# vearch/gamma

Hardware: AMD Instinct MI355X
Metric: queries/sec @ recall@10>=0.95, IVFPQ nlist=4096 nprobe=32 (higher is better)
Workload: dtype f32

## Files before the change

gamma_amd/_lib.py:

```python
import ctypes as C
import os

HERE = os.path.dirname(os.path.abspath(__file__))
LIB_PATH = os.path.join(HERE, "libgamma_hip.so")

f32p = C.POINTER(C.c_float)
i64p = C.POINTER(C.c_int64)
i32p = C.POINTER(C.c_int32)
u8p = C.POINTER(C.c_uint8)

NUM_STAGES = 6
STAGE_NAMES = ["coarse", "tables", "scan", "select", "rerank", "flat"]


class RangeFilter(C.Structure):
    _fields_ = [("bitmap", u8p), ("bitmap_bytes", C.c_int64), ("min_doc", C.c_int32),
                ("max_doc", C.c_int32), ("min_aligned", C.c_int32), ("b_not_in", C.c_int32)]


class FieldFilter(C.Structure):
    _fields_ = [("field_id", C.c_int32), ("include_lower", C.c_int32), ("include_upper", C.c_int32),
                ("reserved", C.c_int32), ("lower_i", C.c_int64), ("upper_i", C.c_int64),
                ("lower_f", C.c_double), ("upper_f", C.c_double)]


class TermFilter(C.Structure):
    _fields_ = [("field_id", C.c_int32), ("op", C.c_int32), ("n_items", C.c_int32), ("items", C.c_int32 * 16)]


class SearchParams(C.Structure):
    _fields_ = [("metric", C.c_int32), ("nprobe", C.c_int32), ("recall_num", C.c_int32),
                ("has_rank", C.c_int32), ("min_score", C.c_float), ("max_score", C.c_float),
                ("coarse_mode", C.c_int32), ("has_range", C.c_int32), ("n_range", C.c_int32),
                ("range", C.POINTER(RangeFilter)), ("n_field", C.c_int32), ("n_term", C.c_int32),
                ("field", C.POINTER(FieldFilter)), ("term", C.POINTER(TermFilter)), ("exact_ties", C.c_int32)]


SYMBOLS = {
    "gamma_hip_create": (C.c_int, [C.c_int, C.POINTER(C.c_void_p)]),
    "gamma_hip_destroy": (C.c_int, [C.c_void_p]),
    "gamma_hip_strerror": (C.c_char_p, [C.c_int]),
    "gamma_hip_last_error": (C.c_char_p, [C.c_void_p]),
    "gamma_hip_stream": (C.c_void_p, [C.c_void_p]),
    "gamma_hip_synchronize": (C.c_int, [C.c_void_p]),
    "gamma_hip_set_workspace_budget": (C.c_int, [C.c_void_p, C.c_int64]),
    "gamma_hip_debug_heap_stream": (C.c_int, [C.c_void_p, C.c_int, C.c_int, C.c_int, f32p, f32p, i32p, f32p, i32p]),
    "gamma_hip_set_scan_bound_feedback": (C.c_int, [C.c_void_p, C.c_int]),
    "gamma_hip_scan_bound_stats": (C.c_int, [C.c_void_p, i64p]),
    "gamma_hip_set_exact_ties": (C.c_int, [C.c_void_p, C.c_int]),
    "gamma_hip_field_append": (C.c_int, [C.c_void_p, C.c_int, C.c_int, C.c_int64, C.c_void_p]),
    "gamma_hip_field_update": (C.c_int, [C.c_void_p, C.c_int, C.c_int64, C.c_void_p]),
    "gamma_hip_field_count": (C.c_int64, [C.c_void_p, C.c_int]),
    "gamma_hip_term_append": (C.c_int, [C.c_void_p, C.c_int, C.c_int64, C.POINTER(C.c_int32), C.POINTER(C.c_int32)]),
    "gamma_hip_term_count": (C.c_int64, [C.c_void_p, C.c_int]),
    "gamma_hip_term_update": (C.c_int, [C.c_void_p, C.c_int, C.c_int64, C.c_int32, C.POINTER(C.c_int32)]),
    "gamma_hip_raw_init": (C.c_int, [C.c_void_p, C.c_int]),
    "gamma_hip_raw_append": (C.c_int, [C.c_void_p, C.c_int64, f32p]),
    "gamma_hip_raw_update": (C.c_int, [C.c_void_p, C.c_int64, f32p]),
    "gamma_hip_ivfpq_arena_stats": (C.c_int, [C.c_void_p, i64p]),
    "gamma_hip_ivfpq_arena_growth": (C.c_int, [C.c_void_p, i64p]),
    "gamma_hip_ivfpq_set_repack_threshold": (C.c_int, [C.c_void_p, C.c_int64]),
    "gamma_hip_set_small_path": (C.c_int, [C.c_void_p, C.c_int]),
    "gamma_hip_set_coarse_fused": (C.c_int, [C.c_void_p, C.c_int, C.c_int]),
    "gamma_hip_tie_stats": (C.c_int, [C.c_void_p, i64p, C.c_int]),
    "gamma_hip_ties_not_honoured": (C.c_int, [C.c_void_p, i64p, C.c_int]),
    "gamma_hip_blas_form_not_restated": (C.c_int, [C.c_void_p, i64p, C.c_int]),
    "gamma_hip_raw_write": (C.c_int, [C.c_void_p, C.c_int64, C.c_int64, f32p]),
    "gamma_hip_raw_gets": (C.c_int, [C.c_void_p, C.c_int64, i64p, f32p]),
    "gamma_hip_ivfpq_repack_verify_stats": (C.c_int, [C.c_void_p, i64p]),
    "gamma_hip_raw_count": (C.c_int64, [C.c_void_p]),
    "gamma_hip_raw_stats": (C.c_int, [C.c_void_p, i64p]),
    "gamma_hip_bitmap_upload": (C.c_int, [C.c_void_p, u8p, C.c_int64]),
    "gamma_hip_bitmap_set": (C.c_int, [C.c_void_p, i64p, C.c_int64, C.c_int]),
    "gamma_hip_ivfpq_init": (C.c_int, [C.c_void_p] + [C.c_int] * 7),
    "gamma_hip_ivfpq4_init": (C.c_int, [C.c_void_p] + [C.c_int] * 6),
    "gamma_hip_ivfpq_set_trained": (C.c_int, [C.c_void_p, f32p, f32p, f32p]),
    "gamma_hip_ivfpq_get_precomputed_table": (C.c_int, [C.c_void_p, f32p]),
    "gamma_hip_set_precomputed_table_max_bytes": (C.c_int, [C.c_int64]),
    "gamma_hip_get_precomputed_table_max_bytes": (C.c_int64, []),
    "gamma_hip_ivfpq_use_precomputed_table": (C.c_int, [C.c_void_p]),
    "gamma_hip_ivfpq_add_keys": (C.c_int, [C.c_void_p, C.c_int, C.c_int, i64p, u8p]),
    "gamma_hip_ivfpq_add_keys_batch": (C.c_int, [C.c_void_p, C.c_int, i32p, i32p, i64p, u8p]),
    "gamma_hip_ivfpq_update": (C.c_int, [C.c_void_p, C.c_int, C.c_int64, u8p]),
    "gamma_hip_vid2docid_append": (C.c_int, [C.c_void_p, C.c_int64, C.POINTER(C.c_int32)]),
    "gamma_hip_vid2docid_count": (C.c_int64, [C.c_void_p]),
    "gamma_hip_binivf_init": (C.c_int, [C.c_void_p, C.c_int, C.c_int, C.c_int, C.c_int]),
    "gamma_hip_binivf_train": (C.c_int, [C.c_void_p, C.c_int, C.c_int64, u8p, C.c_int, u8p]),
    "gamma_hip_binivf_set_trained": (C.c_int, [C.c_void_p, u8p]),
    "gamma_hip_binivf_assign": (C.c_int, [C.c_void_p, C.c_int64, u8p, C.c_int, i32p, i64p]),
    "gamma_hip_binivf_add": (C.c_int, [C.c_void_p, C.c_int64, u8p, C.c_int64]),
    "gamma_hip_binivf_search": (C.c_int, [C.c_void_p, C.POINTER(SearchParams), C.c_int, u8p, C.c_int, f32p, i64p]),
    "gamma_hip_binivf_search_device": (C.c_int, [C.c_void_p, C.POINTER(SearchParams), C.c_int, C.c_void_p, C.c_int,
                                                 C.c_void_p, C.c_void_p]),
    "gamma_hip_binivf_stats": (C.c_int, [C.c_void_p, i64p, C.c_int]),
    "gamma_hip_ivfflat_init": (C.c_int, [C.c_void_p, C.c_int, C.c_int, C.c_int, C.c_int, C.c_int]),
    "gamma_hip_ivfflat_set_trained": (C.c_int, [C.c_void_p, f32p]),
    "gamma_hip_ivfflat_search": (C.c_int, [C.c_void_p, C.POINTER(SearchParams), C.c_int, f32p, C.c_int, f32p, i64p]),
    "gamma_hip_ivfflat_search_device": (C.c_int, [C.c_void_p, C.POINTER(SearchParams), C.c_int, C.c_void_p, C.c_int,
                                                  C.c_void_p, C.c_void_p]),
    "gamma_hip_ivfpq_has_vid": (C.c_int, [C.c_void_p, i64p, C.c_int, u8p]),
    "gamma_hip_ivfpq_remove": (C.c_int, [C.c_void_p, C.c_int64]),
    "gamma_hip_ivfpq_delete": (C.c_int, [C.c_void_p, i64p, C.c_int]),
    "gamma_hip_ivfpq_compact_if_need": (C.c_int, [C.c_void_p]),
    "gamma_hip_ivfpq_list_size": (C.c_int64, [C.c_void_p, C.c_int]),
    "gamma_hip_ivfpq_list_capacity": (C.c_int64, [C.c_void_p, C.c_int]),
    "gamma_hip_ivfpq_get_list": (C.c_int, [C.c_void_p, C.c_int, i64p, u8p]),
    "gamma_hip_ivfpq_set_list_mask": (C.c_int, [C.c_void_p, u8p]),
    "gamma_hip_ivfpq_add": (C.c_int, [C.c_void_p, C.c_int64, f32p, C.c_int64]),
    "gamma_hip_ivfpq_encode": (C.c_int, [C.c_void_p, C.c_int64, f32p, i64p, u8p]),
    "gamma_hip_assign": (C.c_int, [C.c_void_p, C.c_int, C.c_int64, f32p, C.c_int, f32p, i32p, f32p]),
    "gamma_hip_kmeans": (C.c_int, [C.c_void_p, C.c_int, C.c_int64, f32p, C.c_int, C.c_int, C.c_int64, C.c_int, f32p,
                                   C.POINTER(C.c_float)]),
    "gamma_hip_rand_perm": (None, [i32p, C.c_int64, C.c_int64]),
    "gamma_hip_ivfpq_train": (C.c_int, [C.c_void_p, C.c_int, C.c_int64, f32p, C.c_int, C.c_int, f32p, f32p]),
    "gamma_hip_ivfpq_search": (C.c_int, [C.c_void_p, C.POINTER(SearchParams), C.c_int, f32p, C.c_int,
                                         f32p, i64p]),
    "gamma_hip_ivfpq_search_device": (C.c_int, [C.c_void_p, C.POINTER(SearchParams), C.c_int,
                                                C.c_void_p, C.c_int, C.c_void_p, C.c_void_p]),
    "gamma_hip_ivfpq_search_device_wait": (C.c_int, [C.c_void_p, C.POINTER(SearchParams), C.c_int,
                                                     C.c_void_p, C.c_int, C.c_void_p, C.c_void_p]),
    "gamma_hip_flat_search_device_wait": (C.c_int, [C.c_void_p, C.POINTER(SearchParams), C.c_int,
                                                    C.c_void_p, C.c_int, C.c_void_p, C.c_void_p]),
    "gamma_hip_ivfpq_last_stages": (C.c_int, [C.c_void_p, f32p, i64p, f32p, i64p]),
    "gamma_hip_ivfpq_search_shard": (C.c_int, [C.c_void_p, C.POINTER(SearchParams), C.c_int,
                                               C.c_void_p, C.c_int, C.c_void_p, C.c_void_p]),
    "gamma_hip_ivfpq_coarse_device": (C.c_int, [C.c_void_p, C.POINTER(SearchParams), C.c_int, C.c_void_p,
                                                C.c_void_p, C.c_void_p]),
    "gamma_hip_ivfpq_search_shard_preassigned": (C.c_int, [C.c_void_p, C.POINTER(SearchParams), C.c_int,
                                                           C.c_void_p, C.c_void_p, C.c_void_p, C.c_int,
                                                           C.c_void_p, C.c_void_p]),
    "gamma_hip_ivfpq_search_shard_bounded": (C.c_int, [C.c_void_p, C.POINTER(SearchParams), C.c_int,
                                                       C.c_void_p, C.c_void_p, C.c_void_p, C.c_int,
                                                       C.c_void_p, C.c_void_p, C.c_void_p, C.c_void_p, C.c_void_p]),
    "gamma_hip_raw_put": (C.c_int, [C.c_void_p, C.c_int64, i64p, f32p]),
    "gamma_hip_raw_drop": (C.c_int, [C.c_void_p, C.c_int64, i64p]),
    "gamma_hip_raw_clear": (C.c_int, [C.c_void_p]),
    "gamma_hip_raw_sparse_stats": (C.c_int, [C.c_void_p, i64p]),
    "gamma_hip_ivfpq_shard_exact": (C.c_int, [C.c_void_p, C.POINTER(SearchParams), C.c_int, C.c_void_p, C.c_void_p, C.c_int, C.c_void_p]),
    "gamma_hip_ivfpq_merge_rerank_exact": (C.c_int, [C.c_void_p, C.POINTER(SearchParams), C.c_int, C.c_int, C.c_void_p, C.c_int,
                                                     C.c_void_p, C.c_void_p, C.c_void_p, C.c_int, C.c_int, C.c_void_p, C.c_void_p]),
    "gamma_hip_ivfpq_shard_export_exact": (C.c_int, [C.c_void_p, C.POINTER(SearchParams), C.c_int, C.c_void_p, C.c_void_p, C.c_void_p,
                                                     C.c_void_p, C.c_int64, C.c_void_p, C.c_void_p]),
    "gamma_hip_ivfpq_merge_replay_exact": (C.c_int, [C.c_void_p, C.POINTER(SearchParams), C.c_int, C.c_int, C.c_void_p, C.c_int64,
                                                     C.c_void_p, C.c_void_p, C.c_void_p, C.c_void_p, C.c_int, C.c_void_p, C.c_void_p,
                                                     C.c_void_p]),
    "gamma_hip_bound_combine": (C.c_int, [C.c_void_p, C.c_void_p, C.c_void_p, C.c_int, C.c_int]),
    "gamma_hip_ivfpq_merge_rerank": (C.c_int, [C.c_void_p, C.POINTER(SearchParams), C.c_int, C.c_int,
                                               C.c_void_p, C.c_int, C.c_void_p, C.c_void_p, C.c_int,
                                               C.c_int, C.c_void_p, C.c_void_p]),
    "gamma_hip_flat_search": (C.c_int, [C.c_void_p, C.POINTER(SearchParams), C.c_int, f32p, C.c_int,
                                        f32p, i64p]),
    "gamma_hip_flat_search_device": (C.c_int, [C.c_void_p, C.POINTER(SearchParams), C.c_int,
                                               C.c_void_p, C.c_int, C.c_void_p, C.c_void_p]),
    "gamma_hip_raw_update_batch": (C.c_int, [C.c_void_p, C.c_int64, i64p, f32p]),
    "gamma_hip_ivfpq_dim": (C.c_int, [C.c_void_p]),
    "gamma_hip_ivfpq_nlist": (C.c_int, [C.c_void_p]),
    "gamma_hip_ivfpq_code_size": (C.c_int, [C.c_void_p]),
    "gamma_hip_ivfpq_update_batch": (C.c_int, [C.c_void_p, C.c_int, i64p, f32p]),
    "gamma_hip_ivfpq_encode_each": (C.c_int, [C.c_void_p, C.c_int64, f32p, i64p, u8p]),
    "gamma_hip_ivfpq_apply_updates": (C.c_int, [C.c_void_p, C.c_int, i32p, i64p, u8p, u8p]),
    "gamma_hip_group_create": (C.c_int, [C.POINTER(C.c_int), C.c_int, C.POINTER(C.c_void_p)]),
    "gamma_hip_group_destroy": (C.c_int, [C.c_void_p]),
    "gamma_hip_group_size": (C.c_int, [C.c_void_p]),
    "gamma_hip_group_member": (C.c_void_p, [C.c_void_p, C.c_int]),
    "gamma_hip_group_last_error": (C.c_char_p, [C.c_void_p]),
    "gamma_hip_group_set_owners": (C.c_int, [C.c_void_p, i64p]),
    "gamma_hip_group_owner": (C.c_int, [C.c_void_p, C.c_int]),
    "gamma_hip_ivfpq_shard_cut_flags": (C.c_int, [C.c_void_p, C.c_int, C.c_void_p]),
    "gamma_hip_ivfpq_merge_set_shard_flags": (C.c_int, [C.c_void_p, C.c_void_p]),
    "gamma_hip_ivfpq_merge_flagged": (C.c_int, [C.c_void_p, C.POINTER(C.c_int), C.POINTER(C.c_void_p)]),
    "gamma_hip_gather_rows": (C.c_int, [C.c_void_p, C.c_void_p, C.c_int, C.c_void_p, C.c_int, C.c_void_p]),
    "gamma_hip_ivfpq_max_list_len": (C.c_int, [C.c_void_p]),
    "gamma_hip_ivfpq_shard_export_rows": (C.c_int, [C.c_void_p, C.c_void_p, C.c_int, C.c_void_p, i64p]),
    "gamma_hip_ivfpq_shard_export": (C.c_int, [C.c_void_p, C.c_void_p, C.c_int, C.c_void_p, C.c_void_p, C.c_void_p, C.c_int64,
                                               C.c_void_p, C.c_void_p, C.c_void_p]),
    "gamma_hip_ivfpq_merge_replay": (C.c_int, [C.c_void_p, C.c_void_p, C.c_int, C.c_int, C.c_void_p, C.c_int64, C.c_void_p,
                                               C.c_void_p, C.c_void_p, C.c_int, C.c_void_p, C.c_void_p, C.c_void_p]),
    "gamma_hip_set_deferred_replay": (C.c_int, [C.c_void_p, C.c_int]),
    "gamma_hip_join": (C.c_int, [C.c_void_p]),
    "gamma_hip_group_set_placement": (C.c_int, [C.c_void_p, C.c_int]),
    "gamma_hip_group_placement": (C.c_int, [C.c_void_p]),
    "gamma_hip_group_ivfpq_add": (C.c_int, [C.c_void_p, C.c_int64, f32p, C.c_int64]),
    "gamma_hip_group_ivfpq_add_keys": (C.c_int, [C.c_void_p, C.c_int, C.c_int, i64p, u8p]),
    "gamma_hip_group_ivfpq_list_size": (C.c_int64, [C.c_void_p, C.c_int]),
    "gamma_hip_group_set_transport": (C.c_int, [C.c_void_p, C.c_int]),
    "gamma_hip_group_transport": (C.c_int, [C.c_void_p, i64p]),
    "gamma_hip_group_transport_note": (C.c_char_p, [C.c_void_p]),
    "gamma_hip_group_ivfpq_get_list": (C.c_int, [C.c_void_p, C.c_int, i64p, u8p]),
    "gamma_hip_group_ivfpq_update": (C.c_int, [C.c_void_p, C.c_int, i64p, f32p]),
    "gamma_hip_group_ivfpq_delete": (C.c_int, [C.c_void_p, i64p, C.c_int]),
    "gamma_hip_group_ivfpq_compact_if_need": (C.c_int, [C.c_void_p]),
    "gamma_hip_group_ivfpq_search": (C.c_int, [C.c_void_p, C.POINTER(SearchParams), C.c_int, f32p, C.c_int, f32p, i64p]),
    "gamma_hip_group_ivfpq_search_device": (C.c_int, [C.c_void_p, C.POINTER(SearchParams), C.c_int, C.c_void_p, C.c_int,
                                                      C.c_void_p, C.c_void_p]),
    "gamma_hip_group_total_mem_bytes": (C.c_int64, [C.c_void_p]),
    "gamma_hip_group_set_raw_placement": (C.c_int, [C.c_void_p, C.c_int]),
    "gamma_hip_group_raw_placement": (C.c_int, [C.c_void_p]),
    "gamma_hip_group_raw_put": (C.c_int, [C.c_void_p, C.c_int64, i64p, f32p, i64p]),
    "gamma_hip_total_mem_bytes": (C.c_int64, [C.c_void_p]),
    "gamma_hip_profile_enable": (C.c_int, [C.c_void_p, C.c_int]),
    "gamma_hip_profile_reset": (C.c_int, [C.c_void_p]),
    "gamma_hip_profile_get": (C.c_int, [C.c_void_p, C.c_int, C.POINTER(C.c_double),
                                        C.POINTER(C.c_int64)]),
    "gamma_hip_profile_scan_bytes": (C.c_int, [C.c_void_p, C.POINTER(C.c_int64),
                                               C.POINTER(C.c_int64)]),
}

_lib = None


BOUND_REDUCE_FN = C.CFUNCTYPE(C.c_int, C.c_void_p, C.c_void_p, C.c_int, C.c_int, C.c_void_p)


class GammaHipError(RuntimeError):
    pass

# ... 21 lines not shown
```

gamma_amd/api.py:

```python
import ctypes as C

import numpy as np

from . import _lib
from ._lib import GammaHipError, RangeFilter, SearchParams

METRIC_IP = 0
METRIC_L2 = 1

FLT_TINY = float(np.finfo(np.float32).tiny)
FLT_MAX = float(np.finfo(np.float32).max)


def _f32(a):
    return np.ascontiguousarray(a, dtype=np.float32)


def _p(a, t):
    return a.ctypes.data_as(t) if a is not None else None


def make_range_filter(docids, b_not_in=False):
    docids = np.asarray(sorted(set(int(x) for x in docids)), dtype=np.int64)
    mn, mx = (int(docids[0]), int(docids[-1])) if len(docids) else (0, 0)
# ... 361 lines not shown

    def binivf_search(self, x, k, args):
        x = np.ascontiguousarray(x, dtype=np.uint8)
        nq = x.shape[0]
        D = np.empty((nq, max(k, 0)), dtype=np.float32)
        I = np.empty((nq, max(k, 0)), dtype=np.int64)
        self._ck(self.L.gamma_hip_binivf_search(self.h, args.ref(), nq, _p(x, _lib.u8p), k, _p(D, _lib.f32p),
                                                _p(I, _lib.i64p)), "binivf_search")
        return D, I

    def binivf_search_device(self, d_x, nq, k, args, d_D, d_I):
        self._ck(self.L.gamma_hip_binivf_search_device(self.h, args.ref(), nq, d_x, k, d_D, d_I), "binivf_search_device")

    def binivf_stats(self, reset=False):
        out = np.zeros(2, dtype=np.int64)
        self._ck(self.L.gamma_hip_binivf_stats(self.h, _p(out, _lib.i64p), 1 if reset else 0), "binivf_stats")
        return int(out[0]), int(out[1])

    def last_stages(self, nq, nprobe, R):
        cd = np.empty((nq, nprobe), dtype=np.float32)
        ci = np.empty((nq, nprobe), dtype=np.int64)
        rd = np.empty((nq, R), dtype=np.float32)
        ri = np.empty((nq, R), dtype=np.int64)
        self._ck(self.L.gamma_hip_ivfpq_last_stages(self.h, _p(cd, _lib.f32p), _p(ci, _lib.i64p),
                                                    _p(rd, _lib.f32p), _p(ri, _lib.i64p)), "last_stages")
        return dict(coarse_dis=cd, coarse_idx=ci, recall_dis=rd, recall_ids=ri)

    def flat_search(self, x, k, args):
        x = _f32(x)
        nq = x.shape[0]
        D = np.empty((nq, max(k, 0)), dtype=np.float32)
        I = np.empty((nq, max(k, 0)), dtype=np.int64)
        self._ck(self.L.gamma_hip_flat_search(self.h, args.ref(), nq, _p(x, _lib.f32p), k,
                                              _p(D, _lib.f32p), _p(I, _lib.i64p)), "flat_search")
        return D, I

    def ivfpq_search_device(self, d_x, nq, k, args, d_D, d_I):
        self._ck(self.L.gamma_hip_ivfpq_search_device(self.h, args.ref(), nq, d_x, k, d_D, d_I),
                 "ivfpq_search_device")

    def ivfpq_search_device_wait(self, d_x, nq, k, args, d_D, d_I):
        self._ck(self.L.gamma_hip_ivfpq_search_device_wait(self.h, args.ref(), nq, d_x, k, d_D, d_I),
                 "ivfpq_search_device_wait")

    def flat_search_device_wait(self, d_x, nq, k, args, d_D, d_I):
        self._ck(self.L.gamma_hip_flat_search_device_wait(self.h, args.ref(), nq, d_x, k, d_D, d_I), "flat_search_device_wait")

    def flat_search_device(self, d_x, nq, k, args, d_D, d_I):
        self._ck(self.L.gamma_hip_flat_search_device(self.h, args.ref(), nq, d_x, k, d_D, d_I),
                 "flat_search_device")

    def ivfpq_search_shard(self, d_x, nq, k, args, d_rdis, d_rids):
        self._ck(self.L.gamma_hip_ivfpq_search_shard(self.h, args.ref(), nq, d_x, k, d_rdis, d_rids),
                 "ivfpq_search_shard")

    def ivfpq_coarse_device(self, d_x, nq, args, d_cdis, d_probe):
        self._ck(self.L.gamma_hip_ivfpq_coarse_device(self.h, args.ref(), nq, d_x, d_cdis, d_probe),
                 "ivfpq_coarse_device")

    def ivfpq_search_shard_preassigned(self, d_x, nq, d_cdis, d_probe, k, args, d_rdis, d_rids):
        self._ck(self.L.gamma_hip_ivfpq_search_shard_preassigned(self.h, args.ref(), nq, d_x, d_cdis,
                                                                  d_probe, k, d_rdis, d_rids),
                 "ivfpq_search_shard_preassigned")

    def ivfpq_search_shard_bounded(self, d_x, nq, d_cdis, d_probe, k, args, d_rdis, d_rids, d_bound, reduce=None):
        err = []

        def _cb(user, ptr, n, take_max, stream):
            try:
                reduce(n, bool(take_max))
                return 0
            except BaseException as e:
                err.append(e)
                return 1
        cb = _lib.BOUND_REDUCE_FN(_cb) if reduce is not None else None
        rc = self.L.gamma_hip_ivfpq_search_shard_bounded(self.h, args.ref(), nq, d_x, d_cdis, d_probe, k, d_rdis, d_rids,
                                                         d_bound, C.cast(cb, C.c_void_p) if cb is not None else None, None)
        if err:
            raise err[0]
        self._ck(rc, "ivfpq_search_shard_bounded")

    def ivfpq_merge_rerank(self, nshards, nq, d_x, k, args, d_all_dis, d_all_ids, q0, nq_local, d_D, d_I):
        self._ck(self.L.gamma_hip_ivfpq_merge_rerank(self.h, args.ref(), nshards, nq, d_x, k, d_all_dis,
                                                     d_all_ids, q0, nq_local, d_D, d_I), "merge_rerank")

    def ivfpq_shard_cut_flags(self, nq, d_flags):
        self._ck(self.L.gamma_hip_ivfpq_shard_cut_flags(self.h, nq, d_flags), "shard_cut_flags")

    def ivfpq_merge_set_shard_flags(self, d_flags):
        self._ck(self.L.gamma_hip_ivfpq_merge_set_shard_flags(self.h, d_flags), "merge_set_shard_flags")

    def ivfpq_merge_flagged(self):
        import ctypes as C
        n = C.c_int(0)
        ptr = C.c_void_p(0)
        self._ck(self.L.gamma_hip_ivfpq_merge_flagged(self.h, C.byref(n), C.byref(ptr)), "merge_flagged")
        return int(n.value), (ptr.value or 0)

    def gather_rows(self, d_src, row_words, d_list, n, d_dst):
        self._ck(self.L.gamma_hip_gather_rows(self.h, d_src, row_words, d_list, n, d_dst), "gather_rows")

    def max_list_len(self):
        return self.L.gamma_hip_ivfpq_max_list_len(self.h)

    def ivfpq_shard_export_rows(self, nf, d_probe_f, args):
        out = np.zeros(1, dtype=np.int64)
        self._ck(self.L.gamma_hip_ivfpq_shard_export_rows(self.h, args.ref(), nf, d_probe_f, _p(out, _lib.i64p)), "shard_export_rows")
        return int(out[0])

    def ivfpq_shard_export(self, nf, d_xf, d_cdis_f, d_probe_f, stride, args, d_vals, d_ids, d_off):
        self._ck(self.L.gamma_hip_ivfpq_shard_export(self.h, args.ref(), nf, d_xf, d_cdis_f, d_probe_f, stride, d_vals, d_ids,
                                                     d_off), "shard_export")

    def ivfpq_shard_exact(self, d_x, nq, d_ids, R, args, d_exact):
        self._ck(self.L.gamma_hip_ivfpq_shard_exact(self.h, args.ref(), nq, d_x, d_ids, R, d_exact), "shard_exact")

    def ivfpq_merge_rerank_exact(self, nshards, nq, d_x, k, args, d_all_dis, d_all_ids, d_all_exact, q0, nq_local, d_D, d_I):
        self._ck(self.L.gamma_hip_ivfpq_merge_rerank_exact(self.h, args.ref(), nshards, nq, d_x, k, d_all_dis, d_all_ids, d_all_exact,
                                                           q0, nq_local, d_D, d_I), "merge_rerank_exact")

    def ivfpq_shard_export_exact(self, nf, d_xf, d_vals, d_ids, d_off, stride, d_bound_f, args, d_ex):
        self._ck(self.L.gamma_hip_ivfpq_shard_export_exact(self.h, args.ref(), nf, d_xf, d_vals, d_ids, d_off, stride, d_bound_f, d_ex),
                 "shard_export_exact")

    def ivfpq_merge_replay_exact(self, nshards, nf, d_x_slice, stride, d_vals_all, d_ids_all, d_off_all, d_ex_all, k, args, d_list,
                                 d_D, d_I):
        self._ck(self.L.gamma_hip_ivfpq_merge_replay_exact(self.h, args.ref(), nshards, nf, d_x_slice, stride, d_vals_all, d_ids_all,
                                                           d_off_all, d_ex_all, k, d_list, d_D, d_I), "merge_replay_exact")

    def ivfpq_merge_replay(self, nshards, nf, d_x_slice, stride, d_vals_all, d_ids_all, d_off_all, k, args, d_list, d_D, d_I):
        self._ck(self.L.gamma_hip_ivfpq_merge_replay(self.h, args.ref(), nshards, nf, d_x_slice, stride, d_vals_all, d_ids_all,
                                                     d_off_all, k, d_list, d_D, d_I), "merge_replay")

    def debug_heap_stream(self, op, k, vals):
        vals = _f32(vals).ravel()
        av, ai = np.empty(k, np.float32), np.empty(k, np.int32)
        sv, si = np.empty(k, np.float32), np.empty(k, np.int32)
        self._ck(self.L.gamma_hip_debug_heap_stream(self.h, op, k, len(vals), _p(vals, _lib.f32p), _p(av, _lib.f32p),
                                                    _p(ai, _lib.i32p), _p(sv, _lib.f32p), _p(si, _lib.i32p)), "debug_heap_stream")
        return av, ai, sv, si

    def set_scan_bound_feedback(self, on):
        self._ck(self.L.gamma_hip_set_scan_bound_feedback(self.h, 1 if on else 0), "set_scan_bound_feedback")

    def scan_bound_stats(self):
        out = np.zeros(4, np.int64)
        self._ck(self.L.gamma_hip_scan_bound_stats(self.h, _p(out, _lib.i64p)), "scan_bound_stats")
        return dict(zip(["fell_through", "queries", "backoffs", "gave_up_waiting"], [int(v) for v in out]))

    def set_dist_budget(self, nbytes):
        self._ck(self.L.gamma_hip_set_workspace_budget(self.h, int(nbytes)), "set_workspace_budget")

    def set_coarse_fused(self, on=True, list_cap=128):
        self._ck(self.L.gamma_hip_set_coarse_fused(self.h, 1 if on else 0, list_cap), "set_coarse_fused")

    def set_small_path(self, on=True):
        self._ck(self.L.gamma_hip_set_small_path(self.h, int(on)), "set_small_path")

    def tie_stats(self, reset=False):
        out = np.zeros(3, np.int64)
        self._ck(self.L.gamma_hip_tie_stats(self.h, _p(out, _lib.i64p), 1 if reset else 0), "tie_stats")
        return dict(coarse_rows=int(out[0]), cut_ties=int(out[1]), replayed=int(out[2]))

    def ties_not_honoured(self, reset=False):
        out = np.zeros(1, dtype=np.int64)
        self._ck(self.L.gamma_hip_ties_not_honoured(self.h, _p(out, _lib.i64p), 1 if reset else 0), "ties_not_honoured")
        return int(out[0])

    def blas_form_not_restated(self, reset=False):
        out = np.zeros(1, dtype=np.int64)
        self._ck(self.L.gamma_hip_blas_form_not_restated(self.h, _p(out, _lib.i64p), 1 if reset else 0), "blas_form_not_restated")
        return int(out[0])

    def set_exact_ties(self, on=True):
        self._ck(self.L.gamma_hip_set_exact_ties(self.h, 1 if on else 0), "set_exact_ties")

    _FIELD_DTYPES = {np.dtype(np.int32): 0, np.dtype(np.int64): 1, np.dtype(np.float32): 2,
                     np.dtype(np.float64): 3}

    def field_append(self, field_id, values):
        values = np.ascontiguousarray(values)
        dt = self._FIELD_DTYPES[values.dtype]
        self._ck(self.L.gamma_hip_field_append(self.h, field_id, dt, values.size, values.ctypes.data),
                 "field_append")

    def field_update(self, field_id, docid, value):
        value = np.ascontiguousarray(value)
        self._ck(self.L.gamma_hip_field_update(self.h, field_id, docid, value.ctypes.data), "field_update")

    def term_append(self, field_id, docs_items):
        counts = np.ascontiguousarray([len(d) for d in docs_items], dtype=np.int32)
        flat = np.ascontiguousarray([t for d in docs_items for t in d], dtype=np.int32)
        self._ck(self.L.gamma_hip_term_append(self.h, field_id, len(counts), counts.ctypes.data_as(C.POINTER(C.c_int32)),
                                              flat.ctypes.data_as(C.POINTER(C.c_int32))), "term_append")

    def term_update(self, field_id, docid, items):
        it = np.ascontiguousarray(items, dtype=np.int32)
        self._ck(self.L.gamma_hip_term_update(self.h, field_id, docid, len(it), it.ctypes.data_as(C.POINTER(C.c_int32))),
                 "term_update")

    def term_count(self, field_id):
        return self.L.gamma_hip_term_count(self.h, field_id)

    def field_count(self, field_id):
        return self.L.gamma_hip_field_count(self.h, field_id)

    def stream(self):
        return self.L.gamma_hip_stream(self.h)

    def synchronize(self):
        self._ck(self.L.gamma_hip_synchronize(self.h), "synchronize")

    def total_mem_bytes(self):
        return self.L.gamma_hip_total_mem_bytes(self.h)

    def profile_enable(self, on=True):
        self._ck(self.L.gamma_hip_profile_enable(self.h, int(on)), "profile_enable")

    def profile_reset(self):
        self._ck(self.L.gamma_hip_profile_reset(self.h), "profile_reset")

    def profile(self):
        out = {}
        for i, name in enumerate(_lib.STAGE_NAMES):
            ms, n = C.c_double(), C.c_int64()
            self._ck(self.L.gamma_hip_profile_get(self.h, i, C.byref(ms), C.byref(n)), "profile_get")
            out[name] = (ms.value, n.value)
        b, pr = C.c_int64(), C.c_int64()
        self._ck(self.L.gamma_hip_profile_scan_bytes(self.h, C.byref(b), C.byref(pr)), "scan_bytes")
        out["scan_bytes"] = b.value
        out["scan_pairs"] = pr.value
        return out


class GammaHipGroup:

    def __init__(self, devices):
        self.L = _lib.load()
        devs = (C.c_int * len(devices))(*devices)
        g = C.c_void_p()
        rc = self.L.gamma_hip_group_create(devs, len(devices), C.byref(g))
        if rc != 0:
            raise GammaHipError("gamma_hip_group_create(%s): %s" % (list(devices), self.L.gamma_hip_strerror(rc).decode()))
        self.g = g
        self.members = []
        for i in range(len(devices)):
            m = GammaHip.__new__(GammaHip)
            m.L = self.L
            m.h = C.c_void_p(self.L.gamma_hip_group_member(g, i))
            m.d = m.M = None
            m.close = lambda: None
            self.members.append(m)

    def close(self):
        if getattr(self, "g", None):
            for m in self.members:
                m.h = None
            self.L.gamma_hip_group_destroy(self.g)
            self.g = None

    def __del__(self):
        try:
            self.close()
        except Exception:
            pass

    def _ck(self, rc, what):
        if rc != 0:
            raise GammaHipError("%s: %s (%s)" % (what, self.L.gamma_hip_strerror(rc).decode(),
                                                 self.L.gamma_hip_group_last_error(self.g).decode()))

    def each(self, fn):
        return [fn(m) for m in self.members]

    def set_owners(self, weights=None):
        w = None if weights is None else np.ascontiguousarray(weights, dtype=np.int64)
        self._ck(self.L.gamma_hip_group_set_owners(self.g, None if w is None else _p(w, _lib.i64p)), "group_set_owners")

    def owner(self, l):
        return self.L.gamma_hip_group_owner(self.g, l)

    def set_placement(self, replicate):
        self._ck(self.L.gamma_hip_group_set_placement(self.g, 1 if replicate else 0), "group_set_placement")

    def set_raw_placement(self, sharded):
        self._ck(self.L.gamma_hip_group_set_raw_placement(self.g, 1 if sharded else 0), "group_set_raw_placement")

    def raw_placement(self):
        return bool(self.L.gamma_hip_group_raw_placement(self.g))

    def raw_put(self, vids, vecs):
        vids = np.ascontiguousarray(vids, dtype=np.int64)
        vecs = _f32(vecs)
        skipped = np.zeros(1, dtype=np.int64)
        self._ck(self.L.gamma_hip_group_raw_put(self.g, len(vids), _p(vids, _lib.i64p), _p(vecs, _lib.f32p), _p(skipped, _lib.i64p)),
                 "group_raw_put")
        return int(skipped[0])

    def add(self, vecs, first_vid):
        vecs = _f32(vecs)
        self._ck(self.L.gamma_hip_group_ivfpq_add(self.g, vecs.shape[0], _p(vecs, _lib.f32p), first_vid), "group_add")

    def add_keys(self, l, vids, codes):
        vids = np.ascontiguousarray(vids, dtype=np.int64)
        codes = np.ascontiguousarray(codes, dtype=np.uint8)
        self._ck(self.L.gamma_hip_group_ivfpq_add_keys(self.g, l, len(vids), _p(vids, _lib.i64p), _p(codes, _lib.u8p)),
                 "group_add_keys")
# ... 68 lines not shown
```

gamma_amd/csrc/coarse.hip:

```cpp
#include <hip/hip_runtime.h>
#include <stdint.h>
#include <math.h>
#include <stdlib.h>

#include <algorithm>
#include <type_traits>

#include "device_math.h"
#include "heap_dev.h"
#include "kernels.h"

namespace gh {

namespace {
typedef float f32x16 __attribute__((ext_vector_type(16)));
typedef unsigned int u32x2 __attribute__((ext_vector_type(2)));

__device__ __forceinline__ int wave_incl_scan_i(int v) {
    const int lane = threadIdx.x & 63;
#pragma unroll
    for (int o = 1; o < 64; o <<= 1) {
        const int t = __shfl_up(v, o, 64);
        if (lane >= o) v += t;
    }
    return v;
}
}

template <int NCH, bool STORE = false>
__global__ __launch_bounds__(256, 2) void k_coarse_fused(const float* __restrict__ x, int nq,
                                                         const float* __restrict__ y, int ny, int col0,
                                                         const float* __restrict__ yn,
                                                         const float* __restrict__ tau,
                                                         int tiles_per_strip, int cap, int cap_stride,
                                                         unsigned long long* __restrict__ cand,
                                                         int* __restrict__ cand_cnt, int nseg,
                                                         const int* __restrict__ rowmap) {
    constexpr int D = 16 * NCH, LD = D + 1, SEGS = D / 32;
    extern __shared__ float s_co[];
    __shared__ float s_xn[128];
    __shared__ float2 s_xt[128];
    const int tid = threadIdx.x, lane = tid & 63, w = tid >> 6;
    const int seg = blockIdx.x, q_base = blockIdx.y * 128;
    int nrows = nq;
    if constexpr (STORE) {
        if (rowmap) {
            nrows = min(rowmap[0], nq);
            if (q_base >= nrows) return;
        }
    }
    const int ntiles = (ny - col0 + 63) >> 6;
    const int t0 = seg * tiles_per_strip, t1 = min(ntiles, t0 + tiles_per_strip);
    auto slot_r = [&](int it) { return (((w * NCH + it) / SEGS) << 3) + (lane >> 3); };
    auto slot_c = [&](int it) { return (((w * NCH + it) % SEGS) << 5) + ((lane & 7) << 2); };
    float4 vb[NCH];
    auto put = [&](float* base, int it) {
        float* p = base + slot_r(it) * LD + slot_c(it);
        p[0] = vb[it].x; p[1] = vb[it].y; p[2] = vb[it].z; p[3] = vb[it].w;
    };
#pragma unroll
    for (int half = 0; half < 2; half++) {
#pragma unroll
        for (int it = 0; it < NCH; it++) {
            int row = min(q_base + half * 64 + slot_r(it), nrows - 1);
            if constexpr (STORE) {
                if (rowmap) row = rowmap[1 + row];
            }
            vb[it] = *reinterpret_cast<const float4*>(x + (int64_t)row * D + slot_c(it));
        }
#pragma unroll
        for (int it = 0; it < NCH; it++) put(s_co + half * 64 * LD, it);
    }
    __syncthreads();
#pragma unroll
    for (int half = 0; half < 2; half++) {
        const float* row = s_co + (half * 64 + (tid >> 2)) * LD;
        const int l4 = tid & 3;
        float nacc = 0.f;
        for (int i = 0; i < D; i += 4) {
            const float xv = row[i + l4];
            nacc = __builtin_fmaf(xv, xv, nacc);
        }
        const float t01 = nacc + __shfl_down(nacc, 1, 4);
        const float nn = t01 + __shfl_down(t01, 2, 4);
        if (l4 == 0) s_xn[half * 64 + (tid >> 2)] = nn;
    }
    float a[8 * NCH];
    {
        const float* fa = s_co + (w * 32 + (lane & 31)) * LD + (lane >> 5);
#pragma unroll
        for (int u = 0; u < 8 * NCH; u++) a[u] = fa[2 * u];
    }
    __syncthreads();
    if (tid < 128) s_xt[tid] = make_float2(s_xn[tid], (!STORE && q_base + tid < nq) ? tau[q_base + tid] : -INFINITY);
    auto gload = [&](int t) {
#pragma unroll
        for (int it = 0; it < NCH; it++)
            vb[it] = *reinterpret_cast<const float4*>(y + (int64_t)min(col0 + t * 64 + slot_r(it), ny - 1) * D + slot_c(it));
    };
    if (t0 < t1) {
        gload(t0);
#pragma unroll
        for (int it = 0; it < NCH; it++) put(s_co, it);
    }
    __syncthreads();
    int cnt[16];
#pragma unroll
    for (int r = 0; r < 16; r++) cnt[r] = 0;
    const uint32_t lt_mask = (1u << (lane & 31)) - 1u;
    const unsigned row_stride = STORE ? (unsigned)cap_stride : (unsigned)nseg * (unsigned)cap_stride;
    const unsigned lane_row = STORE ? (unsigned)(q_base + w * 32 + 4 * (lane >> 5)) * (unsigned)cap_stride
                                    : ((unsigned)((q_base + w * 32 + 4 * (lane >> 5)) * nseg + seg)) * (unsigned)cap_stride;
    const __amdgpu_buffer_rsrc_t rsrc = __builtin_amdgcn_make_buffer_rsrc(
        cand, 0,
        (int)min(STORE ? (int64_t)nq * cap_stride * 4 : (int64_t)nq * nseg * cap_stride * 8, (int64_t)0x7fffffff),
        0x00020000);
    constexpr unsigned OOB = 0x80000000u;
    const int sh = lane & 32;
    int rs[16];
#pragma unroll
    for (int r = 0; r < 16; r++) rs[r] = ((r & 3) + 8 * (r >> 2)) * (int)row_stride * (STORE ? 4 : 8);
    const float2* xt_row = s_xt + w * 32 + 4 * (lane >> 5);
    auto epi = [&](const f32x16& o, int r, unsigned colv, float ync, int rsoff) {
        const float2 xt = xt_row[(r & 3) + 8 * (r >> 2)];
        if constexpr (STORE) {
            float dis = __builtin_fmaf(-2.f, o[r], xt.x + ync);
            if (dis < 0.f) dis = 0.f;
            __builtin_amdgcn_raw_buffer_store_b32(__float_as_uint(dis), rsrc,
                                                  (int)colv < ny ? (lane_row + (colv - (unsigned)col0)) * 4u : OOB, rsoff, 0);
            return;
        }
        const float dis = __builtin_fmaf(-2.f, o[r], xt.x + ync);
        const bool pass = dis <= xt.y;
        const unsigned long long mask = __ballot(pass);
        const uint32_t mh = (uint32_t)(mask >> sh);
        const unsigned slot = min((unsigned)cnt[r] + (unsigned)__popc(mh & lt_mask), (unsigned)cap);
        u32x2 item;
        item.x = colv;
        item.y = (uint32_t)max((int)__float_as_uint(dis), 0) | 0x80000000u;
        __builtin_amdgcn_raw_buffer_store_b64(item, rsrc, pass ? (lane_row + slot) * 8u : OOB, rsoff, 0);
        cnt[r] += __popc(mh);
    };
    auto step = [&](auto do_mfma, auto do_epi, f32x16& n, const float* fb, const f32x16& o, int colo) {
        constexpr bool MF = decltype(do_mfma)::value, EP = decltype(do_epi)::value;
        float ync = 0.f;
        const unsigned colv = (unsigned)(colo + (lane & 31));
        if constexpr (EP) ync = (int)colv < ny ? yn[min((int)colv, ny - 1)] : INFINITY;
        if constexpr (MF) {
#pragma unroll
            for (int i = 0; i < 16; i++) n[i] = 0.f;
            float f[4];
#pragma unroll
            for (int u = 0; u < 3; u++) f[u] = fb[2 * u];
            constexpr int KP = 8 * NCH, EVERY = KP / 16;
#pragma unroll
            for (int u = 0; u < KP; u++) {
                if (u + 3 < KP) f[(u + 3) & 3] = fb[2 * (u + 3)];
                n = __builtin_amdgcn_mfma_f32_32x32x2f32(a[u], f[u & 3], n, 0, 0, 0);
                if constexpr (EP) {
                    if (u % EVERY == 0) epi(o, u / EVERY, colv, ync, rs[u / EVERY]);
                }
                __builtin_amdgcn_sched_barrier(0);
            }
        } else if constexpr (EP) {
#pragma unroll
            for (int r = 0; r < 16; r++) epi(o, r, colv, ync, rs[r]);
        }
    };
    const std::true_type yes;
    const std::false_type no;
    f32x16 acc0, acc1;
    auto stage = [&](int t) {
#pragma unroll
        for (int it = 0; it < NCH; it++) put(s_co + ((t - t0) & 1) * 64 * LD, it);
    };
    for (int t = t0; t < t1; t++) {
        const float* fb0 = s_co + ((t - t0) & 1) * 64 * LD + (lane & 31) * LD + (lane >> 5);
        const int colb = col0 + t * 64;
        if (t > t0) step(yes, yes, acc0, fb0, acc1, colb - 32);
        else step(yes, no, acc0, fb0, acc1, 0);
        const bool more = t + 1 < t1;
        if (more) gload(t + 1);
        step(yes, yes, acc1, fb0 + 32 * LD, acc0, colb);
        if (more) stage(t + 1);
        __syncthreads();
    }
    if (t0 < t1) step(no, yes, acc0, s_co, acc1, col0 + (t1 - 1) * 64 + 32);
    if (!STORE && (lane & 31) == 0) {
#pragma unroll
        for (int r = 0; r < 16; r++) {
            const int row = q_base + w * 32 + (r & 3) + 8 * (r >> 2) + 4 * (lane >> 5);
            if (row < nq) cand_cnt[row * nseg + seg] = cnt[r];
        }
    }
}


__device__ __forceinline__ uint32_t wave_kth_smallest(uint32_t m, int K) {
    int lt = 0, le = 0;
#pragma unroll
    for (int l = 0; l < 64; l++) {
        const uint32_t o = (uint32_t)__builtin_amdgcn_readlane((int)m, l);
        lt += o < m ? 1 : 0;
        le += o <= m ? 1 : 0;
    }
    const unsigned long long who = __ballot(lt < K && K <= le);
    return (uint32_t)__shfl((int)m, (int)__ffsll((long long)who) - 1, 64);
}

__device__ __forceinline__ uint32_t wave_kth_smallest2(uint32_t m0, uint32_t m1, int K) {
    int lt0 = 0, le0 = 0, lt1 = 0, le1 = 0;
#pragma unroll
    for (int l = 0; l < 64; l++) {
        const uint32_t o0 = (uint32_t)__builtin_amdgcn_readlane((int)m0, l);
        const uint32_t o1 = (uint32_t)__builtin_amdgcn_readlane((int)m1, l);
        lt0 += (o0 < m0 ? 1 : 0) + (o1 < m0 ? 1 : 0);
        le0 += (o0 <= m0 ? 1 : 0) + (o1 <= m0 ? 1 : 0);
        lt1 += (o0 < m1 ? 1 : 0) + (o1 < m1 ? 1 : 0);
        le1 += (o0 <= m1 ? 1 : 0) + (o1 <= m1 ? 1 : 0);
    }
    const unsigned long long who0 = __ballot(lt0 < K && K <= le0), who1 = __ballot(lt1 < K && K <= le1);
    return who0 ? (uint32_t)__shfl((int)m0, (int)__ffsll((long long)who0) - 1, 64)
                : (uint32_t)__shfl((int)m1, (int)__ffsll((long long)who1) - 1, 64);
}

template <int NPL>
__global__ __launch_bounds__(256) void k_coarse_bound(const float* __restrict__ mat, int nq, int P, float* __restrict__ tau,
                                                      int* __restrict__ ovf) {
    if (blockIdx.x == 0 && threadIdx.x == 0) ovf[0] = 0;
    const int lane = threadIdx.x & 63, q = blockIdx.x * 4 + (threadIdx.x >> 6);
    if (q >= nq) return;
    const float* v = mat + (int64_t)q * (64 * NPL) + lane;
    uint32_t m0 = 0xffffffffu, m1 = 0xffffffffu;
#pragma unroll
    for (int j = 0; j < NPL; j++) {
        const uint32_t k = f2key(v[64 * j]);
        if (j & 1) m1 = k < m1 ? k : m1;
        else m0 = k < m0 ? k : m0;
    }
    const uint32_t kb = P <= 32 ? wave_kth_smallest(m0 < m1 ? m0 : m1, P) : wave_kth_smallest2(m0, m1, P);
    if (lane == 0) tau[q] = key2f(kb);
}

constexpr int CF_BUF = 256;
template <int SNPL, int MAXSEG>
__global__ __launch_bounds__(256) void k_coarse_final(const float* __restrict__ mat, const float* __restrict__ tau,
                                                      const unsigned long long* __restrict__ cand,
                                                      const int* __restrict__ cand_cnt, int nseg, int cap,
                                                      int cap_stride, int nq, int P, float* __restrict__ out_dis,
                                                      int* __restrict__ out_idx, int* __restrict__ ovf, int flag_ties) {
    constexpr int NPL = SNPL + 2 * MAXSEG;
    __shared__ unsigned long long s_buf[4][CF_BUF];
    const int lane = threadIdx.x & 63, w = threadIdx.x >> 6;
    const int q = blockIdx.x * 4 + w;
    if (q >= nq) return;
    unsigned long long* buf = s_buf[w];
    const int cnt = lane < nseg ? cand_cnt[q * nseg + lane] : 0;
    if (__ballot(cnt > cap)) {
        if (lane == 0) ovf[1 + atomicAdd(ovf, 1)] = q;
        return;
    }
    unsigned long long it[NPL];
    {
        const float t = tau[q];
        const float* v = mat + (int64_t)q * (64 * SNPL) + lane;
#pragma unroll
        for (int j = 0; j < SNPL; j++) {
            const float x = v[64 * j];
            it[j] = x <= t ? (((unsigned long long)f2key(x) << 32) | (unsigned)(64 * j + lane)) : ~0ull;
        }
    }
#pragma unroll
    for (int sg = 0; sg < MAXSEG; sg++) {
        const int c = __shfl(cnt, sg, 64);
        const unsigned long long* p = cand + ((int64_t)q * nseg + min(sg, nseg - 1)) * cap_stride;
        const int e0 = (lane - 4 * sg) & 63;
        it[SNPL + 2 * sg] = e0 < c ? p[e0] : ~0ull;
        it[SNPL + 2 * sg + 1] = e0 + 64 < c ? p[e0 + 64] : ~0ull;
    }
    uint32_t m0 = 0xffffffffu, m1 = 0xffffffffu;
#pragma unroll
    for (int j = 0; j < NPL; j++) {
        const uint32_t k = (uint32_t)(it[j] >> 32);
        const bool g1 = j < SNPL ? (j & 1) != 0 : ((j >> 1) & 1) != 0;
        if (g1) m1 = k < m1 ? k : m1;
        else m0 = k < m0 ? k : m0;
    }
    const uint32_t kb = P <= 32 ? wave_kth_smallest(m0 < m1 ? m0 : m1, P) : wave_kth_smallest2(m0, m1, P);
    int c = 0;
#pragma unroll
    for (int j = 0; j < NPL; j++) c += ((uint32_t)(it[j] >> 32) <= kb && it[j] != ~0ull) ? 1 : 0;
    const int incl = wave_incl_scan_i(c);
    const int tot = __shfl(incl, 63, 64);
    if (tot > CF_BUF) {
        if (lane == 0) ovf[1 + atomicAdd(ovf, 1)] = q;
        return;
    }
    int off = incl - c;
#pragma unroll
    for (int j = 0; j < NPL; j++)
        if ((uint32_t)(it[j] >> 32) <= kb && it[j] != ~0ull) buf[off++] = it[j];
    __builtin_amdgcn_wave_barrier();
    unsigned long long mine[CF_BUF / 64];
    int rr[CF_BUF / 64];
#pragma unroll
    for (int u = 0; u < CF_BUF / 64; u++) {
        mine[u] = lane + 64 * u < tot ? buf[lane + 64 * u] : ~0ull;
        rr[u] = 0;
    }
    if (tot <= 64) {
        for (int j = 0; j < tot; j++) rr[0] += buf[j] < mine[0] ? 1 : 0;
    } else {
        for (int j = 0; j < tot; j++) {
            const unsigned long long xj = buf[j];
#pragma unroll
            for (int u = 0; u < CF_BUF / 64; u++) rr[u] += xj < mine[u] ? 1 : 0;
        }
    }
#pragma unroll
    for (int u = 0; u < CF_BUF / 64; u++) {
        if (lane + 64 * u < tot && rr[u] < P) {
            out_dis[(int64_t)q * P + rr[u]] = key2f((uint32_t)(mine[u] >> 32));
            out_idx[(int64_t)q * P + rr[u]] = (int)(uint32_t)mine[u];
        }
    }
    for (int r = tot + lane; r < P; r += 64) {
        out_dis[(int64_t)q * P + r] = INFINITY;
        out_idx[(int64_t)q * P + r] = -1;
    }
    if (flag_ties) {
        __builtin_amdgcn_wave_barrier();
#pragma unroll
        for (int u = 0; u < CF_BUF / 64; u++)
            if (lane + 64 * u < tot) buf[rr[u]] = mine[u];
        __builtin_amdgcn_wave_barrier();
        const int have = min(tot, P + 1);
        bool eq = false;
        for (int i = lane; i + 1 < have; i += 64) eq |= (uint32_t)(buf[i] >> 32) == (uint32_t)(buf[i + 1] >> 32);
        if (__ballot(eq) && lane == 0) ovf[1 + atomicAdd(ovf, 1)] = q;
    }
}

__global__ __launch_bounds__(256) void k_coarse_repair(const float* __restrict__ x, int d, const float* __restrict__ y, int ny,
                                                       const float* __restrict__ yn, const int* __restrict__ ovf,
                                                       uint32_t* __restrict__ scratch, int P,
                                                       float* __restrict__ out_dis, int* __restrict__ out_idx) {
    extern __shared__ float s_x[];
    __shared__ float s_n;
    __shared__ unsigned long long s_red[4];
    const int tid = threadIdx.x, lane = tid & 63, w = tid >> 6;
    const int n = ovf[0];
    uint32_t* keys = scratch + (int64_t)blockIdx.x * ny;
    for (int i = blockIdx.x; i < n; i += gridDim.x) {
        const int q = ovf[1 + i];
        __syncthreads();
        for (int t = tid; t < d; t += 256) s_x[t] = x[(int64_t)q * d + t];
        __syncthreads();
        if (tid == 0) {
            float a4[4] = {0.f, 0.f, 0.f, 0.f};
            int t = 0;
            for (; t + 4 <= d; t += 4)
                for (int l = 0; l < 4; l++) a4[l] = __builtin_fmaf(s_x[t + l], s_x[t + l], a4[l]);
            for (int l = 0; t + l < d; l++) a4[l] = a4[l] + s_x[t + l] * s_x[t + l];
            s_n = (a4[0] + a4[1]) + (a4[2] + a4[3]);
        }
        __syncthreads();
        const float xn = s_n;
        for (int c = tid; c < ny; c += 256) {
            const float* yr = y + (int64_t)c * d;
            float ip = 0.f;
            for (int t = 0; t < d; t++) ip = __builtin_fmaf(s_x[t], yr[t], ip);
            float dis = (xn + yn[c]) - 2.f * ip;
            if (dis < 0.f) dis = 0.f;
            keys[c] = f2key(dis);
        }
        __syncthreads();
        unsigned long long last = 0;
        bool first = true;
        for (int r = 0; r < P; r++) {
            unsigned long long best = ~0ull;
            for (int c = tid; c < ny; c += 256) {
                const unsigned long long item = ((unsigned long long)keys[c] << 32) | (unsigned)c;
                if ((first || item > last) && item < best) best = item;
            }
#pragma unroll
            for (int o = 32; o > 0; o >>= 1) {
                const unsigned long long t = __shfl_xor(best, o, 64);
                best = t < best ? t : best;
            }
            if (lane == 0) s_red[w] = best;
            __syncthreads();
            best = s_red[0];
            for (int k = 1; k < 4; k++) best = s_red[k] < best ? s_red[k] : best;
            __syncthreads();
            if (tid == 0) {
                out_dis[(int64_t)q * P + r] = best == ~0ull ? INFINITY : key2f((uint32_t)(best >> 32));
                out_idx[(int64_t)q * P + r] = best == ~0ull ? -1 : (int)(uint32_t)best;
            }
            last = best;
            first = false;
            if (best == ~0ull) {
                for (int r2 = r + 1 + tid; r2 < P; r2 += 256) {
                    out_dis[(int64_t)q * P + r2] = INFINITY;
                    out_idx[(int64_t)q * P + r2] = -1;
                }
                break;
            }
        }
    }
}

static bool coarse_fused_shape(int nlist, int P, int* sample, int* nseg) {
    if (P < 1 || P > 64) return false;
    for (int sm = P <= 32 ? 512 : 1024; sm <= 2048; sm *= 2) {
        if (nlist < 4 * sm) break;
        const double F = P <= 32 ? 1.0 - pow(1.0 - P / 64.0, 64.0 / sm) : 1.0 - pow(1.0 - P / 128.0, 128.0 / sm);
        for (int sg = 8; sg <= 16; sg *= 2) {
            if (F * (nlist - sm) / sg <= 48.0) {
                *sample = sm;
                *nseg = sg;
                return true;
            }
        }
    }
    return false;
}

bool coarse_fused_supported(int nq, int d, int nlist, int P, bool exact_ties) {
    int sm, sg;
    if (!(nq >= 4096 && (d == 32 || d == 64 || d == 96 || d == 128) && coarse_fused_shape(nlist, P, &sm, &sg))) return false;
    if (exact_ties && (int64_t)nq * nlist * 4 >= 0x7fffffffLL) return false;
    return (int64_t)nq * sg * kCoarseCap * 8 < 0x7fffffffLL && (int64_t)nq * sm * 4 < 0x7fffffffLL;
}

CoarseFusedPlan coarse_fused_plan(int nq, int nlist, int P, int cap, bool exact_ties) {
    CoarseFusedPlan pl;
    if (!coarse_fused_shape(nlist, P, &pl.sample, &pl.nseg)) {
        launch_refused("coarse_fused_plan: shape outside the matrix-free coarse path (coarse_fused_supported)");
        pl.sample = 512;
        pl.nseg = 1;
    }
    const int ntiles = (nlist - pl.sample + 63) / 64;
    pl.tiles_per_strip = (ntiles + pl.nseg - 1) / pl.nseg;
    pl.nseg = (ntiles + pl.tiles_per_strip - 1) / pl.tiles_per_strip;
    pl.cap_stride = kCoarseCap;
    pl.cap = std::max(1, std::min(kCoarseCap - 1, cap));
    size_t o = 0;
    auto take = [&](size_t bytes) {
        const size_t at = o;
        o += (bytes + 255) & ~(size_t)255;
        return at;
    };
    pl.off_mat = take((size_t)nq * pl.sample * sizeof(float));
    pl.off_tau = take((size_t)nq * sizeof(float));
    pl.off_cand = take((size_t)nq * pl.nseg * pl.cap_stride * sizeof(unsigned long long));
    pl.off_cnt = take((size_t)nq * pl.nseg * sizeof(int));
    pl.off_ovf = take((size_t)(nq + 1) * sizeof(int));
    pl.off_scratch = take((size_t)kCoarseRepairGrid * nlist * sizeof(uint32_t));
    pl.off_full = exact_ties ? take((size_t)nq * nlist * sizeof(float)) : 0;
    pl.bytes = o;
    return pl;
}

void launch_coarse_fused(hipStream_t s, const CoarseFusedPlan& pl, void* ws, const float* x, int nq, int d,
                         const float* y, int nlist, const float* yn, int P, float* out_dis, int* out_idx, bool exact_ties,
                         unsigned long long* tie_stats, hipStream_t side, hipEvent_t fork, hipEvent_t join) {
    char* b = static_cast<char*>(ws);
    float* mat = reinterpret_cast<float*>(b + pl.off_mat);
    float* tau = reinterpret_cast<float*>(b + pl.off_tau);
    unsigned long long* cand = reinterpret_cast<unsigned long long*>(b + pl.off_cand);
    int* cnt = reinterpret_cast<int*>(b + pl.off_cnt);
    int* ovf = reinterpret_cast<int*>(b + pl.off_ovf);
    uint32_t* scratch = reinterpret_cast<uint32_t*>(b + pl.off_scratch);
    const size_t lds = (size_t)2 * 64 * (d + 1) * sizeof(float);
    {
        const int stiles = pl.sample / 64, sstrips = 4, tps = (stiles + sstrips - 1) / sstrips;
        dim3 sgrid((unsigned)sstrips, (unsigned)((nq + 127) / 128));
#define GH_CS(NCH)                                                                                                      \
    do {                                                                                                                \
        static std::atomic<uint64_t> attr{0};                                                           \
        if (first_call_on_device(attr)) {                                                                               \
            (void)hipFuncSetAttribute(reinterpret_cast<const void*>(k_coarse_fused<NCH, true>),                         \
                                      hipFuncAttributeMaxDynamicSharedMemorySize, 2 * 64 * (16 * NCH + 1) * 4);         \
        }                                                                                                               \
        hipLaunchKernelGGL((k_coarse_fused<NCH, true>), sgrid, dim3(256), lds, s, x, nq, y, pl.sample, 0, yn, nullptr, \
                           tps, 0, pl.sample, reinterpret_cast<unsigned long long*>(mat), nullptr, sstrips, nullptr);  \
    } while (0)
        switch (d) {
            case 32: GH_CS(2); break;
            case 64: GH_CS(4); break;
            case 96: GH_CS(6); break;
            default: GH_CS(8); break;
        }
#undef GH_CS
    }
    if (pl.sample == 512) hipLaunchKernelGGL(k_coarse_bound<8>, dim3((nq + 3) / 4), dim3(256), 0, s, mat, nq, P, tau, ovf);
    else if (pl.sample == 1024) hipLaunchKernelGGL(k_coarse_bound<16>, dim3((nq + 3) / 4), dim3(256), 0, s, mat, nq, P, tau, ovf);
    else hipLaunchKernelGGL(k_coarse_bound<32>, dim3((nq + 3) / 4), dim3(256), 0, s, mat, nq, P, tau, ovf);
    dim3 grid((unsigned)pl.nseg, (unsigned)((nq + 127) / 128));
#define GH_CF(NCH)                                                                                                      \
    do {                                                                                                                \
        static std::atomic<uint64_t> attr{0};                                                           \
        if (first_call_on_device(attr)) {                                                                               \
            (void)hipFuncSetAttribute(reinterpret_cast<const void*>(k_coarse_fused<NCH>),                               \
                                      hipFuncAttributeMaxDynamicSharedMemorySize, 2 * 64 * (16 * NCH + 1) * 4);         \
        }                                                                                                               \
        hipLaunchKernelGGL((k_coarse_fused<NCH>), grid, dim3(256), lds, s, x, nq, y, nlist, pl.sample, yn, tau,         \
                           pl.tiles_per_strip, pl.cap, pl.cap_stride, cand, cnt, pl.nseg, nullptr);                          \
    } while (0)
    switch (d) {
        case 32: GH_CF(2); break;
        case 64: GH_CF(4); break;
        case 96: GH_CF(6); break;
        default: GH_CF(8); break;
    }
#undef GH_CF
#define GH_FIN(SN, MS)                                                                                                  \
    hipLaunchKernelGGL((k_coarse_final<SN, MS>), dim3((nq + 3) / 4), dim3(256), 0, s, mat, tau, cand, cnt, pl.nseg, pl.cap, \
                       pl.cap_stride, nq, P, out_dis, out_idx, ovf, exact_ties ? 1 : 0)
    if (pl.sample == 512) {
        if (pl.nseg <= 4) GH_FIN(8, 4);
        else if (pl.nseg <= 8) GH_FIN(8, 8);
        else GH_FIN(8, 16);
    } else if (pl.sample == 1024) {
        if (pl.nseg <= 8) GH_FIN(16, 8);
        else GH_FIN(16, 16);
    } else {
        if (pl.nseg <= 8) GH_FIN(32, 8);
        else GH_FIN(32, 16);
    }
#undef GH_FIN
    if (!exact_ties) {
        hipLaunchKernelGGL(k_coarse_repair, dim3(kCoarseRepairGrid), dim3(256), (size_t)d * sizeof(float), s, x, d, y, nlist, yn,
                           ovf, scratch, P, out_dis, out_idx);
        return;
    }
    hipStream_t rs = s;
    const bool forked = side && fork && join;
    float* full = reinterpret_cast<float*>(b + pl.off_full);
    {
        const int ntiles = (nlist + 63) / 64, fstrips = std::min(ntiles, 64), tps = (ntiles + fstrips - 1) / fstrips;
        dim3 fgrid((unsigned)fstrips, (unsigned)((nq + 127) / 128));
#define GH_CR(NCH)                                                                                                      \
    hipLaunchKernelGGL((k_coarse_fused<NCH, true>), fgrid, dim3(256), lds, rs, x, nq, y, nlist, 0, yn, nullptr, tps, 0,  \
                       nlist, reinterpret_cast<unsigned long long*>(full), nullptr, fstrips, ovf)
        switch (d) {
            case 32: GH_CR(2); break;
            case 64: GH_CR(4); break;
            case 96: GH_CR(6); break;
            default: GH_CR(8); break;
        }
#undef GH_CR
    }
    if (forked) {
        (void)hipEventRecord(fork, s);
        (void)hipStreamWaitEvent(side, fork, 0);
        rs = side;
    }
    launch_coarse_heap_rows(rs, full, nlist, nq, P, ovf, out_dis, out_idx, tie_stats);
    if (rs != s) (void)hipEventRecord(join, rs);
}

}
```

gamma_amd/csrc/flat_mfma.hip:

```cpp
#include <hip/hip_runtime.h>
#include <stdint.h>

#include <algorithm>
#include <atomic>
#include <cstdlib>

#include "device_math.h"
#include "filter_dev.h"
#include "block_utils.h"
#include "kernels.h"
#include "rerank_dev.h"

namespace gh {

typedef __attribute__((__vector_size__(8 * sizeof(__bf16)))) __bf16 bf16x8;
typedef float ff32x16 __attribute__((ext_vector_type(16)));

constexpr float FM_C = 1.220703125e-4f;
constexpr int FM_QT = 64;
constexpr int FM_ROWS = 128;
constexpr int FM_NT = 256;

__device__ __forceinline__ uint32_t cvt_pk_bf16(float lo, float hi) {
    uint32_t r;
    asm("v_cvt_pk_bf16_f32 %0, %1, %2" : "=v"(r) : "v"(lo), "v"(hi));
    return r;
}
__device__ __forceinline__ void split_bf16x8(const float* f, uint4& hi, uint4& lo) {
    uint32_t h[4], l[4];
#pragma unroll
    for (int i = 0; i < 4; i++) {
        h[i] = cvt_pk_bf16(f[2 * i], f[2 * i + 1]);
        const float h0 = __uint_as_float(h[i] << 16), h1 = __uint_as_float(h[i] & 0xffff0000u);
        l[i] = cvt_pk_bf16(f[2 * i] - h0, f[2 * i + 1] - h1);
    }
    hi = make_uint4(h[0], h[1], h[2], h[3]);
    lo = make_uint4(l[0], l[1], l[2], l[3]);
}

__host__ __device__ constexpr int fm_mt_bytes(int D) { return 2 * (D / 16) * 2 * 32 * 16; }

template <int D>
__global__ __launch_bounds__(256) void k_flat_prep_queries(const float* __restrict__ x, int nq, int nq_pad,
                                                           char* __restrict__ out) {
    constexpr int KK = D / 16;
    const int idx = blockIdx.x * 256 + threadIdx.x;
    if (idx >= nq_pad * (D / 8)) return;
    const int q = idx / (D / 8), kg = idx % (D / 8);
    float f[8];
#pragma unroll
    for (int t = 0; t < 8; t++) f[t] = q < nq ? x[(int64_t)q * D + kg * 8 + t] : 0.f;
    uint4 hi, lo;
    split_bf16x8(f, hi, lo);
    const int mt = q >> 5, i = q & 31, kh = kg / KK, kk = kg % KK;
    char* base = out + (int64_t)mt * fm_mt_bytes(D);
    *reinterpret_cast<uint4*>(base + ((((0 * KK + kk) * 2 + kh) * 32 + i) * 16)) = hi;
    *reinterpret_cast<uint4*>(base + ((((1 * KK + kk) * 2 + kh) * 32 + i) * 16)) = lo;
}

template <bool L2>
__global__ __launch_bounds__(256) void k_flat_bounds(const float* __restrict__ xn, const uint32_t* __restrict__ tau, int nq,
                                                     int nq_pad, float* __restrict__ bnd, float cm) {
    const int q = blockIdx.x * 256 + threadIdx.x;
    if (q >= nq_pad) return;
    float av = INFINITY, gv = 0.f;
    if (q < nq) {
        const uint32_t t = tau[q];
        const float tq = t >= 0xff800000u ? (L2 ? 3.402823466e+38f : -3.402823466e+38f) : key2f(L2 ? t : ~t);
        const float x2 = xn[q];
        if (L2) {
            av = 0.5f * ((1.f - cm) * x2 - tq);
        } else {
            av = tq;
            gv = -cm * __builtin_sqrtf(x2);
        }
    }
    bnd[q] = av;
    bnd[nq_pad + q] = gv;
}

struct FlatFilterArgs {
    const char* qimg;
    const float* bnd;
    int nq, nq_pad;
    const float* y;
    int64_t ny;
    int64_t row_base;
    uint2* pairs;
    int* npairs;
    int cap;
};
constexpr int FM_WLIST = 256;
constexpr int FM_NSUB = 32;
constexpr int FM_CTR_STRIDE = 32;

template <bool L2, int D>
__global__ __launch_bounds__(FM_NT) void k_flat_filter(FlatFilterArgs a) {
    constexpr int KK = D / 16;
    constexpr int TILE = 2 * fm_mt_bytes(D);
    constexpr int LPT = TILE / (FM_NT * 16);
    static_assert(TILE % (FM_NT * 16) == 0, "tile staged by whole rounds of the workgroup");
    extern __shared__ __attribute__((aligned(16))) char s_fm[];
    char* s_tile = s_fm;
    float* s_a = reinterpret_cast<float*>(s_fm + 2 * TILE);
    float* s_g = s_a + 2 * FM_QT;
    uint2* s_list = reinterpret_cast<uint2*>(s_g + 2 * FM_QT);
    const int tid = threadIdx.x, lane = tid & 63, w = tid >> 6;
    const int rg = w >> 1, mh = w & 1, kh = lane >> 5, j = lane & 31;
    const int64_t r0 = (int64_t)blockIdx.x * FM_ROWS + rg * 64;
    bf16x8 bh[2][KK], bl[2][KK];
    float hrow[2];
#pragma unroll
    for (int nt = 0; nt < 2; nt++) {
        const int64_t r = r0 + nt * 32 + j;
        const bool live = r < a.ny;
        const float* yp = a.y + (live ? r : 0) * D + (D / 2) * kh;
        float ss = 0.f;
#pragma unroll
        for (int kk = 0; kk < KK; kk++) {
            const float4 v0 = *reinterpret_cast<const float4*>(yp + 8 * kk);
            const float4 v1 = *reinterpret_cast<const float4*>(yp + 8 * kk + 4);
            const float f[8] = {v0.x, v0.y, v0.z, v0.w, v1.x, v1.y, v1.z, v1.w};
#pragma unroll
            for (int t = 0; t < 8; t++) ss = __builtin_fmaf(f[t], f[t], ss);
            uint4 hi, lo;
            split_bf16x8(f, hi, lo);
            bh[nt][kk] = __builtin_bit_cast(bf16x8, hi);
            bl[nt][kk] = __builtin_bit_cast(bf16x8, lo);
        }
        const float yn = ss + __shfl_xor(ss, 32, 64);
        hrow[nt] = !live ? (L2 ? INFINITY : -INFINITY) : (L2 ? 0.5f * (1.f - FM_C) * yn : __builtin_sqrtf(yn));
    }
    const int nit = a.nq_pad / FM_QT;
    auto stage = [&](int it, int b) {
        const char* src = a.qimg + (int64_t)it * TILE + (w * LPT) * 1024 + lane * 16;
        char* dst = s_tile + b * TILE + (w * LPT) * 1024;
#pragma unroll
        for (int u = 0; u < LPT; u++)
            __builtin_amdgcn_global_load_lds((const __attribute__((address_space(1))) void*)(src + u * 1024),
                                             (__attribute__((address_space(3))) void*)(dst + u * 1024), 16, 0, 0);
        if (w == 0) {
            __builtin_amdgcn_global_load_lds((const __attribute__((address_space(1))) void*)(a.bnd + it * FM_QT + lane),
                                             (__attribute__((address_space(3))) void*)(s_a + b * FM_QT), 4, 0, 0);
            if (!L2)
                __builtin_amdgcn_global_load_lds((const __attribute__((address_space(1))) void*)(a.bnd + a.nq_pad + it * FM_QT + lane),
                                                 (__attribute__((address_space(3))) void*)(s_g + b * FM_QT), 4, 0, 0);
        }
    };
    uint2* wl = s_list + w * FM_WLIST;
    int wcnt = 0;
    const int sub = (int)(blockIdx.x & (FM_NSUB - 1));
    int* seg_ctr = a.npairs + sub * FM_CTR_STRIDE;
    uint2* seg = a.pairs + (int64_t)sub * a.cap;
    auto flush = [&]() {
        int base = 0;
        if (lane == 0) base = atomicAdd(seg_ctr, wcnt);
        base = __builtin_amdgcn_readfirstlane(base);
        __builtin_amdgcn_wave_barrier();
        for (int i = lane; i < wcnt; i += 64)
            if (base + i < a.cap) seg[base + i] = wl[i];
        __builtin_amdgcn_wave_barrier();
        wcnt = 0;
    };
    stage(0, 0);
    __syncthreads();
    for (int it = 0; it < nit; it++) {
        const int b = it & 1;
        const float* pa = s_a + b * FM_QT + mh * 32 + 4 * kh;
        const float* pg = s_g + b * FM_QT + mh * 32 + 4 * kh;
        float4 av4[4], gv4[4];
#pragma unroll
        for (int g4 = 0; g4 < 4; g4++) {
            av4[g4] = *reinterpret_cast<const float4*>(pa + 8 * g4);
            gv4[g4] = L2 ? make_float4(1.f, 1.f, 1.f, 1.f) : *reinterpret_cast<const float4*>(pg + 8 * g4);
        }
        if (it + 1 < nit) stage(it + 1, b ^ 1);
        ff32x16 acc[2];
#pragma unroll
        for (int nt = 0; nt < 2; nt++)
#pragma unroll
            for (int r = 0; r < 16; r++) acc[nt][r] = 0.f;
        const char* tb = s_tile + b * TILE + mh * fm_mt_bytes(D) + (kh * 32 + j) * 16;
#pragma unroll
        for (int kk = 0; kk < KK; kk++) {
            const bf16x8 ah = *reinterpret_cast<const bf16x8*>(tb + ((0 * KK + kk) * 2) * 512);
            const bf16x8 al = *reinterpret_cast<const bf16x8*>(tb + ((1 * KK + kk) * 2) * 512);
#pragma unroll
            for (int nt = 0; nt < 2; nt++) {
                acc[nt] = __builtin_amdgcn_mfma_f32_32x32x16_bf16(al, bh[nt][kk], acc[nt], 0, 0, 0);
                acc[nt] = __builtin_amdgcn_mfma_f32_32x32x16_bf16(ah, bl[nt][kk], acc[nt], 0, 0, 0);
                acc[nt] = __builtin_amdgcn_mfma_f32_32x32x16_bf16(ah, bh[nt][kk], acc[nt], 0, 0, 0);
// ... 365 lines not shown
```

gamma_amd/csrc/gamma_hip.cpp:

```cpp
#include "gamma_hip_internal.h"

using namespace ghi;

extern "C" {

const char* gamma_hip_strerror(int code) {
    switch (code) {
        case GAMMA_HIP_OK: return "ok";
        case GAMMA_HIP_EINVAL: return "invalid argument";
        case GAMMA_HIP_ENOTTRAINED: return "index not trained";
        case GAMMA_HIP_EDEVICE: return "HIP runtime error";
        case GAMMA_HIP_ENOMEM: return "out of memory";
        case GAMMA_HIP_EFULL: return "inverted list full";
        case GAMMA_HIP_EUNSUPPORTED: return "exact ties requested beyond the replay's range";
        default: return "unknown error";
    }
}

int gamma_hip_create(int device, gamma_hip_index** out) {
    if (!out) return GAMMA_HIP_EINVAL;
    *out = nullptr;
    int ndev = 0;
    if (hipGetDeviceCount(&ndev) != hipSuccess || ndev <= 0) return GAMMA_HIP_EDEVICE;
    if (device < 0 || device >= ndev) return GAMMA_HIP_EINVAL;
    if (hipSetDevice(device) != hipSuccess) return GAMMA_HIP_EDEVICE;
    H* h = new (std::nothrow) H();
    if (!h) return GAMMA_HIP_ENOMEM;
    h->device = device;
    if (hipStreamCreateWithFlags(&h->stream, hipStreamNonBlocking) != hipSuccess ||
        hipStreamCreateWithFlags(&h->wstream, hipStreamNonBlocking) != hipSuccess ||
        hipStreamCreateWithFlags(&h->side, hipStreamNonBlocking) != hipSuccess ||
        hipStreamCreateWithFlags(&h->side2, hipStreamNonBlocking) != hipSuccess ||
        hipEventCreateWithFlags(&h->ev_fork, hipEventDisableTiming) != hipSuccess ||
        hipEventCreateWithFlags(&h->ev_join, hipEventDisableTiming) != hipSuccess ||
        hipEventCreateWithFlags(&h->ev_rfork, hipEventDisableTiming) != hipSuccess ||
        hipEventCreateWithFlags(&h->ev_rdone, hipEventDisableTiming) != hipSuccess) {
        delete h;
        return GAMMA_HIP_EDEVICE;
    }
    for (int v = 0; v < H::NVER; v++)
        if (hipEventCreateWithFlags(&h->ver_ev[v], hipEventDisableTiming) != hipSuccess ||
            hipEventCreateWithFlags(&h->rd_ev[v], hipEventDisableTiming) != hipSuccess) {
            delete h;
            return GAMMA_HIP_EDEVICE;
        }
    if (hipMalloc((void**)&h->d_scan_codes, sizeof(unsigned long long)) != hipSuccess ||
        hipMemset(h->d_scan_codes, 0, sizeof(unsigned long long)) != hipSuccess ||
        hipMalloc((void**)&h->d_tie_stats, 3 * sizeof(unsigned long long)) != hipSuccess ||
        hipMemset(h->d_tie_stats, 0, 3 * sizeof(unsigned long long)) != hipSuccess ||
        hipMalloc((void**)&h->d_bound_stat, 5 * sizeof(unsigned long long)) != hipSuccess ||
        hipMemset(h->d_bound_stat, 0, 5 * sizeof(unsigned long long)) != hipSuccess ||
        hipHostMalloc((void**)&h->pin_bound_stat, 4 * sizeof(unsigned long long), hipHostMallocDefault) != hipSuccess) {
        (void)hipStreamDestroy(h->stream);
        delete h;
        return GAMMA_HIP_EDEVICE;
    }
    memset(h->pin_bound_stat, 0, 4 * sizeof(unsigned long long));
    size_t free_b = 0, total_b = 0;
    if (hipMemGetInfo(&free_b, &total_b) == hipSuccess && total_b > 0)
        h->dist_budget_bytes = std::min<size_t>((size_t)32 << 30, std::max<size_t>((size_t)1 << 30, total_b / 8));
    *out = h;
    return GAMMA_HIP_OK;
}

int gamma_hip_destroy(gamma_hip_index* h) {
    if (!h) return GAMMA_HIP_OK;
    {
        std::unique_lock<std::mutex> lk(h->comb_mu);
        h->comb_stop = true;
        h->comb_wcv.notify_all();
    }
    if (h->comb_thread.joinable()) h->comb_thread.join();
    (void)hipSetDevice(h->device);
    (void)hipStreamSynchronize(h->stream);
    (void)hipStreamSynchronize(h->wstream);
    if (h->side) (void)hipStreamSynchronize(h->side);
    if (h->ev_fork) (void)hipEventDestroy(h->ev_fork);
    if (h->ev_join) (void)hipEventDestroy(h->ev_join);
    for (hipEvent_t& e : h->ev_call)
        if (e) (void)hipEventDestroy(e);
    for (auto& sl : h->hslot) {
        sl.x.release();
        sl.D.release();
        sl.I.release();
        if (sl.pin) (void)hipHostFree(sl.pin);
        if (sl.ev_up) (void)hipEventDestroy(sl.ev_up);
        if (sl.ev_done) (void)hipEventDestroy(sl.ev_done);
    }
    if (h->up_stream) (void)hipStreamDestroy(h->up_stream);
    for (auto& b : h->fbank) b.release();
    for (hipEvent_t& e : h->ev_bank)
        if (e) (void)hipEventDestroy(e);
    if (h->ev_rfork) (void)hipEventDestroy(h->ev_rfork);
    if (h->ev_rdone) (void)hipEventDestroy(h->ev_rdone);
    for (int v = 0; v < H::NVER; v++) {
        if (h->ver_ev[v]) (void)hipEventDestroy(h->ver_ev[v]);
        if (h->rd_ev[v]) (void)hipEventDestroy(h->rd_ev[v]);
        if (h->d_ver_off[v]) (void)hipFree(h->d_ver_off[v]);
        if (h->d_ver_len[v]) (void)hipFree(h->d_ver_len[v]);
        if (h->pin_ver[v]) (void)hipHostFree(h->pin_ver[v]);
    }
    for (auto& e : h->events) {
        (void)hipEventDestroy(e.a);
        (void)hipEventDestroy(e.b);
    }
    if (h->raw_vmm) {
        h->raw_vm.release();
        h->d_raw = nullptr;
    }
    h->vm_codes.release();
    h->vm_ids.release();
    h->vm_sums.release();
    h->alt_codes.release();
    h->alt_ids.release();
    h->alt_sums.release();
    for (auto& r : h->vm_retired) r.release();
    if (h->arena_vmm) {
        h->d_codes = nullptr;
        h->d_ids = nullptr;
        h->d_sums = nullptr;
    }
    if (h->d_raw_slot) (void)hipFree(h->d_raw_slot);
    void* ptrs[] = {h->d_list_rank, h->d_raw, h->d_bitmap, h->d_cc, h->d_cc_norms, h->d_pqc, h->d_T2, h->d_codes,
                    h->d_ids, h->d_list_mask, h->d_scan_codes, h->d_tie_stats, h->d_v2d, h->d_sums, h->d_t2max, h->d_bound_stat,
                    h->d_bin_cc, h->d_bin_stats};
    for (void* p : ptrs)
        if (p) (void)hipFree(p);
    for (auto& kv : h->fields)
        if (kv.second.d) (void)hipFree(kv.second.d);
    for (auto& kv : h->terms) {
        if (kv.second.d_off) (void)hipFree(kv.second.d_off);
        if (kv.second.d_tok) (void)hipFree(kv.second.d_tok);
    }
    for (hipEvent_t e : h->event_pool) (void)hipEventDestroy(e);
    for (void* pp : h->comb_pin)
        if (pp) (void)hipHostFree(pp);
    if (h->dir_pin) (void)hipHostFree(h->dir_pin);
    if (h->bound_copy_ev) (void)hipEventDestroy(h->bound_copy_ev);
    if (h->pin_bound_stat) (void)hipHostFree(h->pin_bound_stat);
    if (h->pin_flat_over) (void)hipHostFree(h->pin_flat_over);
    DevBuf* bufs[] = {&h->w_mat, &h->w_coarse_dis, &h->w_probe, &h->w_xn, &h->w_st2, &h->w_pair_off,
                      &h->w_qtotal, &h->w_dist, &h->w_cand_dis, &h->w_cand_pos, &h->w_cand_ids,
                      &h->w_exact, &h->w_selv, &h->w_selp, &h->w_x, &h->w_outd, &h->w_outl, &h->w_stage, &h->w_shard_cut,
                      &h->w_filter, &h->w_m_dis, &h->w_m_ids, &h->w_part_v, &h->w_part_i, &h->w_assign,
                      &h->w_codes_tmp, &h->w_qperm, &h->w_qbins, &h->w_scnt, &h->w_sflag, &h->w_surv, &h->w_pair_base,
                      &h->w_pair_ip, &h->w_flat_cand, &h->w_flat_meta, &h->w_full_cdis,
                      &h->w_full_probe, &h->w_ftab, &h->w_qfil, &h->w_tieflag, &h->w_tcut, &h->w_tlist, &h->w_lm_units, &h->w_lm_cnt, &h->w_fbits, &h->w_cmp_codes, &h->w_cmp_ids, &h->w_cmp_len, &h->w_cmp_sums, &h->w_fD, &h->w_fI, &h->w_fx, &h->w_fslab, &h->w_flog, &h->w_mr_vals, &h->w_mr_ids, &h->w_mr_meta,
                      &h->we_mat, &h->we_cdis, &h->we_x, &h->we_assign, &h->we_codes, &h->we_stage};
    for (DevBuf* b : bufs) b->release();
    (void)hipStreamDestroy(h->stream);
    (void)hipStreamDestroy(h->wstream);
    if (h->side) (void)hipStreamDestroy(h->side);
    if (h->side2) (void)hipStreamDestroy(h->side2);
    delete h;
    return GAMMA_HIP_OK;
}

const char* gamma_hip_last_error(gamma_hip_index* h) { return h ? h->err.c_str() : "null handle"; }
void* gamma_hip_stream(gamma_hip_index* h) { return h ? (void*)h->stream : nullptr; }

int gamma_hip_synchronize(gamma_hip_index* h) {
    if (!h) return GAMMA_HIP_EINVAL;
    SearchLock lk(h);
    GH_CHECK(h, hipSetDevice(h->device));
    GH_CHECK(h, hipStreamSynchronize(h->stream));
    GH_CHECK(h, hipStreamSynchronize(h->wstream));
    if (h->side) GH_CHECK(h, hipStreamSynchronize(h->side));
    if (h->side2) GH_CHECK(h, hipStreamSynchronize(h->side2));
    h->replay_pending = false;
    return GAMMA_HIP_OK;
}

int gamma_hip_set_deferred_replay(gamma_hip_index* h, int on) {
    if (!h) return GAMMA_HIP_EINVAL;
    SearchLock lk(h);
    if (!on && h->replay_pending) {
        GH_CHECK(h, hipSetDevice(h->device));
        GH_CHECK(h, hipStreamWaitEvent(h->stream, h->ev_rdone, 0));
        h->replay_pending = false;
    }
    h->defer_replay = on != 0;
    return GAMMA_HIP_OK;
}

int gamma_hip_join(gamma_hip_index* h) {
    if (!h) return GAMMA_HIP_EINVAL;
    SearchLock lk(h);
    if (h->replay_pending) {
        GH_CHECK(h, hipSetDevice(h->device));
        GH_CHECK(h, hipStreamWaitEvent(h->stream, h->ev_rdone, 0));
        h->replay_pending = false;
    }
    return GAMMA_HIP_OK;
}

int gamma_hip_ivfpq_dim(gamma_hip_index* h) { return (h && h->ivf_init) ? h->d : 0; }
int gamma_hip_ivfpq_nlist(gamma_hip_index* h) { return (h && h->ivf_init) ? h->nlist : 0; }
int gamma_hip_ivfpq_code_size(gamma_hip_index* h) { return (h && h->ivf_init) ? h->code_size : 0; }

int gamma_hip_set_exact_ties(gamma_hip_index* h, int on) {
    if (!h) return GAMMA_HIP_EINVAL;
    SearchLock lk(h);
    h->exact_ties = on != 0;
    return GAMMA_HIP_OK;
}

int gamma_hip_set_coarse_fused(gamma_hip_index* h, int on, int list_cap) {
    if (!h || list_cap < 1 || list_cap > gh::kCoarseCap) return GAMMA_HIP_EINVAL;
    SearchLock lk(h);
    h->coarse_fused = on != 0;
    h->coarse_cap = list_cap;
    return GAMMA_HIP_OK;
}

int gamma_hip_set_small_path(gamma_hip_index* h, int on) {
    if (!h) return GAMMA_HIP_EINVAL;
    SearchLock lk(h);
    h->small_path = on != 0;
    h->small_presel = on >= 2 ? on : 0;
    return GAMMA_HIP_OK;
}

int gamma_hip_tie_stats(gamma_hip_index* h, int64_t* out3, int reset) {
    if (!h || !out3) return GAMMA_HIP_EINVAL;
    SearchLock lk(h);
    GH_CHECK(h, hipSetDevice(h->device));
    if (h->side) GH_CHECK(h, hipStreamSynchronize(h->side));
    if (h->side2) GH_CHECK(h, hipStreamSynchronize(h->side2));
    unsigned long long v[3];
    GH_CHECK(h, hipMemcpyAsync(v, h->d_tie_stats, sizeof(v), hipMemcpyDeviceToHost, h->stream));
    if (reset) GH_CHECK(h, hipMemsetAsync(h->d_tie_stats, 0, sizeof(v), h->stream));
    GH_CHECK(h, hipStreamSynchronize(h->stream));
    for (int i = 0; i < 3; i++) out3[i] = (int64_t)v[i];
    return GAMMA_HIP_OK;
}

int gamma_hip_ties_not_honoured(gamma_hip_index* h, int64_t* out_calls, int reset) {
    if (!h || !out_calls) return GAMMA_HIP_EINVAL;
    *out_calls = reset ? h->ties_unhonoured.exchange(0) : h->ties_unhonoured.load();
    return GAMMA_HIP_OK;
}

int gamma_hip_blas_form_not_restated(gamma_hip_index* h, int64_t* out_calls, int reset) {
    if (!h || !out_calls) return GAMMA_HIP_EINVAL;
    *out_calls = reset ? h->blas_unrestated.exchange(0) : h->blas_unrestated.load();
    return GAMMA_HIP_OK;
}

int gamma_hip_set_scan_bound_feedback(gamma_hip_index* h, int on) {
    if (!h) return GAMMA_HIP_EINVAL;
    SearchLock lk(h);
    h->bound_feedback_off = on == 0;
    h->bound_off_calls = 0;
    return GAMMA_HIP_OK;
}

int gamma_hip_scan_bound_stats(gamma_hip_index* h, int64_t* out4) {
    if (!h || !out4) return GAMMA_HIP_EINVAL;
    SearchLock lk(h);
    GH_CHECK(h, hipSetDevice(h->device));
    GH_CHECK(h, hipStreamSynchronize(h->stream));
    unsigned long long v[5] = {0, 0, 0, 0, 0};
    GH_CHECK(h, hipMemcpy(v, h->d_bound_stat, sizeof(v), hipMemcpyDeviceToHost));
    const int slot = h->bound_epoch & 1;
    out4[0] = (int64_t)v[2 * slot];
    out4[1] = (int64_t)v[2 * slot + 1];
    out4[2] = h->bound_backoffs;
    out4[3] = (int64_t)v[4];
    return GAMMA_HIP_OK;
}

int gamma_hip_set_workspace_budget(gamma_hip_index* h, int64_t bytes) {
    if (!h || bytes <= 0) return GAMMA_HIP_EINVAL;
    SearchLock lk(h);
    h->dist_budget_bytes = (size_t)bytes;
    return GAMMA_HIP_OK;
}

int64_t gamma_hip_total_mem_bytes(gamma_hip_index* h) {
    if (!h) return -1;
    std::lock_guard<std::mutex> g(h->mu);
    int64_t b = 0;
    b += h->raw_cap * h->raw_d * (int64_t)sizeof(float) + h->raw_slot_cap * (int64_t)sizeof(int32_t);
    b += (int64_t)h->bitmap_cap_bytes;
    for (auto& kv : h->fields) b += kv.second.cap * (int64_t)field_elem_size(kv.second.dtype);
    for (auto& kv : h->terms) b += kv.second.cap_docs * 8 + kv.second.cap_tok * 4;
    if (h->ivf_init) {
        b += (int64_t)h->nlist * h->d * 4 + (int64_t)h->nlist * 4 + (int64_t)h->M * 256 * h->dsub * 4;
        if (h->d_T2) b += h->ivfflat ? 256 : (int64_t)h->nlist * h->M * 256 * 4;
        b += h->arena_cap * (h->code_size + (int64_t)sizeof(int64_t));
        if (h->d_sums) b += h->arena_cap * (int64_t)sizeof(float) + (int64_t)h->nlist * 4;
        b += (int64_t)h->nlist * 12;
        b += (int64_t)(h->w_cmp_codes.cap + h->w_cmp_ids.cap + h->w_cmp_len.cap);
    }
    return b;
}

int gamma_hip_profile_enable(gamma_hip_index* h, int on) {
    if (!h) return GAMMA_HIP_EINVAL;
    SearchLock lk(h);
    h->profile = on == 2 ? 2 : (on != 0 ? 1 : 0);
    return GAMMA_HIP_OK;
}

int gamma_hip_profile_reset(gamma_hip_index* h) {
    if (!h) return GAMMA_HIP_EINVAL;
    SearchLock lk(h);
    GH_CHECK(h, hipSetDevice(h->device));
    GH_TRY(drain_events(h));
    for (int i = 0; i < GAMMA_HIP_NUM_STAGES; i++) {
        h->stage_ms[i] = 0;
        h->stage_n[i] = 0;
    }
    h->scan_pairs = 0;
    GH_CHECK(h, hipMemsetAsync(h->d_scan_codes, 0, sizeof(unsigned long long), h->stream));
    GH_CHECK(h, hipStreamSynchronize(h->stream));
    return GAMMA_HIP_OK;
}

int gamma_hip_profile_get(gamma_hip_index* h, int stage, double* total_ms, int64_t* launches) {
    if (!h || stage < 0 || stage >= GAMMA_HIP_NUM_STAGES) return GAMMA_HIP_EINVAL;
    SearchLock lk(h);
    GH_CHECK(h, hipSetDevice(h->device));
    GH_TRY(drain_events(h));
    if (total_ms) *total_ms = h->stage_ms[stage];
    if (launches) *launches = h->stage_n[stage];
    return GAMMA_HIP_OK;
}

int gamma_hip_profile_scan_bytes(gamma_hip_index* h, int64_t* bytes, int64_t* pairs) {
    if (!h) return GAMMA_HIP_EINVAL;
    SearchLock lk(h);
    GH_CHECK(h, hipSetDevice(h->device));
    GH_CHECK(h, hipStreamSynchronize(h->stream));
    unsigned long long codes = 0;
    GH_CHECK(h, hipMemcpy(&codes, h->d_scan_codes, sizeof(codes), hipMemcpyDeviceToHost));
    if (bytes) *bytes = (int64_t)codes * h->code_size;
    if (pairs) *pairs = h->scan_pairs;
    return GAMMA_HIP_OK;
}

}
```

gamma_amd/csrc/gamma_hip_internal.h:

```cpp
#pragma once
#include "../../include/gamma_hip.h"

#include <hip/hip_runtime.h>
#include <math.h>
#include <stdlib.h>
#include <string.h>

#include <algorithm>
#include <atomic>
#include <map>
#include <chrono>
#include <condition_variable>
#include <cstring>
#include <deque>
#include <functional>
#include <mutex>
#include <string>
#include <thread>
#include <unordered_map>
#include <vector>

#include "kernels.h"

namespace ghi {
// ... 63 lines not shown
    const int64_t rx = nx % 4096, ry = ny % 1024;
    if ((rx >= 1 && rx <= 7) || (ry >= 1 && ry <= 7)) return true;
    return d == 384 && ry >= 9 && ry <= 512;
}

struct gamma_hip_index {
    int device = 0;
    hipStream_t stream = nullptr, wstream = nullptr;
    hipStream_t side = nullptr;
    hipStream_t side2 = nullptr;
    hipEvent_t ev_fork = nullptr, ev_join = nullptr;
    bool coarse_join_pending = false;
    hipEvent_t ev_rfork = nullptr, ev_rdone = nullptr;
    bool defer_replay = false, defer_now = false, replay_pending = false;
    hipEvent_t ev_call[4] = {nullptr, nullptr, nullptr, nullptr};
    unsigned call_seq = 0;
    struct HostSlot {
        DevBuf x, D, I;
        void* pin = nullptr;
        size_t pin_bytes = 0;
        hipEvent_t ev_up = nullptr, ev_done = nullptr;
        bool busy = false;
    };
    HostSlot hslot[2];
    std::mutex hs_mu;
    std::condition_variable hs_cv;
    hipStream_t up_stream = nullptr;
    DevBuf fbank[5];
    int flat_bank = 0;
    hipEvent_t ev_bank[2] = {nullptr, nullptr};
    bool bank_used[2] = {false, false};
    bool replay_is_flat = false;
    int* pin_flat_over = nullptr;
    int* flat_over_dst = nullptr;
    bool flat_no_bound = false;
    std::atomic<int> big_calls_in_flight{0};
    std::atomic<int64_t> big_calls_overlap_seen_ns{INT64_MIN / 2};
    uint64_t write_gen = 1, cmp_gen = 0;
    bool cmp_has_sums = false, cmp_sums_built = false;
    bool cmp_by_clause = false;
    bool merge_flags = false;
    int shard_cut_nq = 0;
    bool shard_cut_chunked = false;
    const uint8_t* merge_shard_flags = nullptr;
    int merge_nql = 0;
    std::mutex mu, search_mu, writer_mu;
    WriteLock* wl = nullptr;
    static constexpr int NVER = 4;
    int64_t* d_ver_off[NVER] = {nullptr, nullptr, nullptr, nullptr};
    int* d_ver_len[NVER] = {nullptr, nullptr, nullptr, nullptr};
    void* pin_ver[NVER] = {nullptr, nullptr, nullptr, nullptr};
    hipEvent_t ver_ev[NVER] = {nullptr, nullptr, nullptr, nullptr};
    hipEvent_t rd_ev[NVER] = {nullptr, nullptr, nullptr, nullptr};
    bool rd_set[NVER] = {false, false, false, false};
    int cur_ver = 0;
    std::string err;

    int raw_d = 0;
    float* d_raw = nullptr;
    int64_t nraw = 0, raw_cap = 0;
    bool raw_sparse = false;
    std::vector<int32_t> h_raw_slot;
    int32_t* d_raw_slot = nullptr;
    int64_t raw_slot_cap = 0;
    int64_t raw_live = 0;
    std::vector<int32_t> raw_free;
    bool raw_vmm = false;
    VmRange raw_vm;
    int64_t raw_regrows = 0;

    struct Column {
        int dtype = 0;
        uint8_t* d = nullptr;
        int64_t n = 0, cap = 0;
    };
    std::map<int, Column> fields;
    struct TermColumn {
        int64_t* d_off = nullptr;
        int32_t* d_tok = nullptr;
        int64_t ndocs = 0, cap_docs = 0, ntok = 0, cap_tok = 0;
        std::vector<int64_t> h_rows;
    };
    std::map<int, TermColumn> terms;

    uint8_t* d_bitmap = nullptr;
    int64_t bitmap_bits = 0;
    size_t bitmap_cap_bytes = 0;
    std::vector<uint8_t> h_bitmap;
    bool bitmap_any = false;
    int64_t n_moved = 0;

    bool ivf_init = false, trained = false;
    int d = 0, nlist = 0, M = 0, ksub = 256, dsub = 0, code_size = 0, metric = GAMMA_HIP_METRIC_L2;
    int bucket_init = 1000, bucket_max = 1280000;
    float *d_cc = nullptr, *d_cc_norms = nullptr, *d_pqc = nullptr, *d_T2 = nullptr;
    int* d_list_rank = nullptr;
    bool sort_queries = getenv("GAMMA_HIP_NO_QUERY_SORT") == nullptr;
    bool scan_bound = getenv("GAMMA_HIP_NO_SCAN_BOUND") == nullptr;
    unsigned long long* d_bound_stat = nullptr;
    unsigned long long* pin_bound_stat = nullptr;
    unsigned long long bound_seen[2] = {0, 0};
    hipEvent_t bound_copy_ev = nullptr;
    bool bound_copy_pending = false;
    uint64_t bound_sig = 0;
    int bound_epoch = 0;
    bool bound_feedback_off = false;
    int bound_calls = 0, bound_off_calls = 0;
    int64_t bound_backoffs = 0;

    uint8_t* d_codes = nullptr;
    int64_t* d_ids = nullptr;
    float* d_sums = nullptr;
    float* d_t2max = nullptr;
    float t2max_all = 0.f;
    int table_mode = 1;
    const float* scan_st2(bool l2) const { return (l2 && table_mode == 0) ? d_pqc : w_st2.as<float>(); }
    bool keep_sums = false;
    int64_t q_stride_cap = 0;
    int64_t arena_cap = 0, arena_used = 0, arena_waste = 0;
    bool arena_vmm = false;
    VmRange vm_codes, vm_ids, vm_sums;
    VmRange alt_codes, alt_ids, alt_sums;
    std::vector<VmRange> vm_retired;
    int64_t arena_regrows = 0;
    int64_t repack_min_entries = 1 << 16;
    int64_t n_repacks = 0;
    int64_t repack_verified = 0, repack_verify_failures = 0;
    std::vector<int64_t> h_list_off;
    std::vector<int> h_list_len, h_list_cap, h_deleted;
    std::vector<uint8_t> h_extend_time;
    int64_t* d_list_off = nullptr;
    int* d_list_len = nullptr;
    uint8_t* d_list_mask = nullptr;
    std::vector<uint8_t> h_list_mask;
    std::vector<int64_t> vid_pos;
    int max_list_len = 0;
    int64_t ntotal = 0;

    DevBuf w_mat, w_coarse_dis, w_probe, w_xn, w_st2, w_pair_off, w_qtotal, w_dist, w_cand_dis,
            w_cand_pos, w_cand_ids, w_exact, w_selv, w_selp, w_x, w_outd, w_outl, w_stage, w_shard_cut, w_filter,
            w_m_dis, w_m_ids, w_part_v, w_part_i, w_assign, w_codes_tmp, w_qperm, w_qbins, w_scnt, w_sflag, w_surv, w_pair_base, w_q8, w_q8meta, w_q8cand, w_q8int,
            w_pair_ip, w_flat_cand, w_flat_meta, w_full_cdis, w_full_probe, w_ftab, w_qfil, w_tieflag, w_tcut, w_tlist, w_textra, w_fq, w_fraw, w_frcnt, w_lm_units, w_lm_cnt, w_fbits, w_cmp_codes, w_cmp_ids, w_cmp_len, w_cmp_sums, w_fD, w_fI, w_fx, w_fslab, w_flog, w_mr_vals, w_mr_ids, w_mr_meta,
            we_mat, we_cdis, we_x, we_assign, we_codes, we_stage, we_chk;
    unsigned long long* d_scan_codes = nullptr;
    size_t dist_budget_bytes = (size_t)8 << 30;

    gh::FilterDesc ftab_shadow;
    bool ftab_valid = false;

    bool exact_ties = true;
    std::atomic<int64_t> ties_unhonoured{0};
    int scan_dbg_now = 0;
    std::atomic<int64_t> blas_unrestated{0};
    bool coarse_fused = true;
    bool small_path = true;
    int small_presel = 0;
    std::vector<int32_t> h_v2d;
    int32_t* d_v2d = nullptr;
    int64_t v2d_cap = 0;
    int64_t doc_of(int64_t v) const { return (v >= 0 && (size_t)v < h_v2d.size()) ? (int64_t)h_v2d[v] : v; }
    bool doc_deleted(int64_t v) const {
        const int64_t dd = doc_of(v);
        return dd >= 0 && dd < bitmap_bits && !h_bitmap.empty() && ((h_bitmap[dd >> 3] >> (dd & 7)) & 1);
    }
    bool ivfflat = false;
    bool binivf = false;
    uint8_t* d_bin_cc = nullptr;
    unsigned long long* d_bin_stats = nullptr;
    int coarse_cap = gh::kCoarseCap;
    unsigned long long* d_tie_stats = nullptr;
    struct TieCtx {
        bool on = false, bounded = false;
        int G = 0, nsl = 0, cap = 0;
        int64_t q_stride = 0;
    } tie;

    int last_nq = 0, last_P = 0, last_R = 0;
    const int* last_qperm = nullptr;

    struct Waiter {
        const gamma_hip_search_params* p;
        int nq, k, mode;
        int kind = 0;
        const float* x;
        float* D;
        int64_t* I;
        int rc = 0;
        static constexpr int FAN = 4;
        bool done = false;
        std::mutex wm;
        std::condition_variable cv;
        Waiter* child[FAN] = {nullptr, nullptr, nullptr, nullptr};
    };
    std::mutex comb_mu;
    std::condition_variable comb_wcv;
    std::deque<Waiter*> comb_q;
    bool prefiltered = false;
    bool comb_busy = false;
    bool comb_stop = false;
    std::thread comb_thread;
    bool combine = getenv("GAMMA_HIP_NO_COMBINE") == nullptr;
    static constexpr int NSET = 4;
    void* comb_pin[NSET] = {nullptr, nullptr, nullptr, nullptr};
    void* comb_pin_dev[NSET] = {nullptr, nullptr, nullptr, nullptr};
    size_t comb_pin_bytes[NSET] = {0, 0, 0, 0};
    void* dir_pin = nullptr;
    void* dir_pin_dev = nullptr;
    size_t dir_pin_bytes = 0;

    int profile = 0;
    std::vector<StageEvent> events;
    std::vector<hipEvent_t> event_pool;
    double stage_ms[GAMMA_HIP_NUM_STAGES] = {0};
    int64_t stage_n[GAMMA_HIP_NUM_STAGES] = {0};
    int64_t scan_pairs = 0;
};

struct WriteLock {
    gamma_hip_index* h;
    std::unique_lock<std::mutex> w, s, m;
    explicit WriteLock(gamma_hip_index* h_) : h(h_), w(h_->writer_mu), s(h_->search_mu, std::defer_lock), m(h_->mu) {
        h->wl = this;
        h->write_gen++;
    }
    ~WriteLock() { h->wl = nullptr; }
    hipError_t exclusive() {
        if (!s.owns_lock()) {
            m.unlock();
            s.lock();
            m.lock();
        }
        hipError_t e = hipStreamSynchronize(h->stream);
        if (e == hipSuccess) e = hipStreamSynchronize(h->wstream);
        if (e == hipSuccess && h->side) e = hipStreamSynchronize(h->side);
        if (e == hipSuccess && h->side2) e = hipStreamSynchronize(h->side2);
        return e;
    }
    void shared() {
        if (s.owns_lock()) s.unlock();
    }
};

namespace ghi {

using H = gamma_hip_index;

struct SearchLock {
    std::unique_lock<std::mutex> s, m;
    explicit SearchLock(H* h) : s(h->search_mu), m(h->mu) {}
    void enqueued() {
        if (m.owns_lock()) m.unlock();
    }
};

#define GH_CHECK(h, expr)                                                                  \
    do {                                                                                   \
        hipError_t e_ = (expr);                                                            \
        if (e_ != hipSuccess) {                                                            \
            (h)->err = std::string(#expr) + ": " + hipGetErrorString(e_);                  \
            return e_ == hipErrorOutOfMemory ? GAMMA_HIP_ENOMEM : GAMMA_HIP_EDEVICE;       \
        }                                                                                  \
        if (const char* r_ = gh::launch_refused_take()) {    \
            (h)->err = std::string("internal: ") + r_;                                     \
            return GAMMA_HIP_EDEVICE;                                                      \
        }                                                                                  \
    } while (0)

#define GH_TRY(expr)                   \
    do {                               \
        int rc_ = (expr);              \
        if (rc_ != GAMMA_HIP_OK) return rc_; \
    } while (0)

inline int fail(H* h, int code, const char* msg) {
    h->err = msg;
    return code;
}

struct StageScope {
    H* h;
    int stage;
    bool count;
    hipEvent_t a = nullptr, b = nullptr;
    StageScope(H* h_, int st, bool count_ = true) : h(h_), stage(st), count(count_) {
        if (h->profile == 1 || (h->profile == 2 && st == GAMMA_HIP_STAGE_SCAN && count_)) {
            auto take = [&]() -> hipEvent_t {
                if (!h->event_pool.empty()) {
                    hipEvent_t e = h->event_pool.back();
                    h->event_pool.pop_back();
                    return e;
                }
                hipEvent_t e = nullptr;
                return hipEventCreate(&e) == hipSuccess ? e : nullptr;
            };
            a = take();
            b = take();
            if (!a || !b) {
                a = b = nullptr;
                return;
            }
            (void)hipEventRecord(a, h->stream);
        }
    }
    ~StageScope() {
        if (a && b) {
            (void)hipEventRecord(b, h->stream);
            h->events.push_back({stage, a, b, count});
// ... 47 lines not shown
```

gamma_amd/csrc/gamma_hip_search.cpp:

```cpp
#include "gamma_hip_internal.h"
#include "gamma_hip_search.h"
#include "pq4.h"

namespace ghi {


int build_filter(H* h, const gamma_hip_search_params* p, gh::FilterDesc* f, size_t* off_io, int64_t est_codes) {
    memset(f, 0, sizeof(*f));
    f->del_bitmap = h->d_bitmap;
    f->del_bits = h->d_bitmap ? h->bitmap_bits : 0;
    f->vid2doc = h->h_v2d.empty() ? nullptr : h->d_v2d;
    f->n_vid2doc = (int64_t)h->h_v2d.size();
    f->has_range = p->has_range ? 1 : 0;
    f->n_range = p->has_range ? p->n_range : 0;
    if (f->n_range > gh::kMaxRange) return fail(h, GAMMA_HIP_EINVAL, "too many range filters");
    if (f->n_range > 0) {
        size_t tot = 0;
        for (int i = 0; i < f->n_range; i++) tot += ((size_t)p->range[i].bitmap_bytes + 15) & ~(size_t)15;
        if (!off_io) GH_CHECK(h, h->w_filter.ensure(tot));
        size_t off = off_io ? *off_io : 0;
        for (int i = 0; i < f->n_range; i++) {
            const gamma_hip_range_filter& r = p->range[i];
            uint8_t* dst = h->w_filter.as<uint8_t>() + off;
            GH_CHECK(h, hipMemcpyAsync(dst, r.bitmap, (size_t)r.bitmap_bytes, hipMemcpyHostToDevice,
                                       h->stream));
            f->range[i].bitmap = dst;
            f->range[i].min_doc = r.min_doc;
            f->range[i].max_doc = r.max_doc;
            f->range[i].min_aligned = r.min_aligned;
            f->range[i].b_not_in = r.b_not_in;
            off += ((size_t)r.bitmap_bytes + 15) & ~(size_t)15;
        }
        if (off_io) *off_io = off;
    }
    f->n_field = p->n_field;
    if (p->n_field < 0 || p->n_field > gh::kMaxField || (p->n_field > 0 && !p->field))
        return fail(h, GAMMA_HIP_EINVAL, "bad field filters");
    for (int i = 0; i < p->n_field; i++) {
        const gamma_hip_field_filter& ff = p->field[i];
        auto it = h->fields.find(ff.field_id);
        if (it == h->fields.end()) return fail(h, GAMMA_HIP_EINVAL, "field filter on an unknown column");
        gh::FieldDesc& fd = f->field[i];
        fd.col = it->second.d;
        fd.n = it->second.n;
        fd.dtype = it->second.dtype;
        fd.incl = (ff.include_lower ? 1 : 0) | (ff.include_upper ? 2 : 0);
        fd.lo_i = ff.lower_i;
        fd.hi_i = ff.upper_i;
        fd.lo_f = ff.lower_f;
        fd.hi_f = ff.upper_f;
    }
    f->n_term = p->n_term;
    if (p->n_term < 0 || p->n_term > gh::kMaxTerm || (p->n_term > 0 && !p->term))
        return fail(h, GAMMA_HIP_EINVAL, "bad term filters");
    for (int i = 0; i < p->n_term; i++) {
        const gamma_hip_term_filter& tf = p->term[i];
        auto it = h->terms.find(tf.field_id);
        if (it == h->terms.end()) return fail(h, GAMMA_HIP_EINVAL, "term filter on an unknown column");
        if (tf.n_items < 0 || tf.n_items > gh::kMaxTermItems || tf.op < 0 || tf.op > 2)
            return fail(h, GAMMA_HIP_EINVAL, "bad term filter");
        gh::TermDesc& td = f->term[i];
        td.off = it->second.d_off;
        td.tok = it->second.d_tok;
        td.n = it->second.ndocs;
        td.op = tf.op;
        td.n_items = tf.n_items;
        for (int k = 0; k < tf.n_items; k++) td.items[k] = tf.items[k];
    }
    if (!off_io && est_codes > 0 && f->n_field + f->n_term > 0 && f->n_range < gh::kMaxRange) {
        int64_t nbits = 0;
        for (int i = 0; i < f->n_field; i++) nbits = std::max<int64_t>(nbits, f->field[i].n);
        for (int i = 0; i < f->n_term; i++) nbits = std::max<int64_t>(nbits, f->term[i].n);
        const char* env = getenv("GAMMA_HIP_FILTER_BITMAP");
        const bool want = env ? atoi(env) != 0 : est_codes >= 4 * nbits;
        if (want && nbits > 0 && nbits < ((int64_t)1 << 31)) {
            gh::FilterDesc g = *f;
            g.has_range = 0;
            g.n_range = 0;
            g.del_bitmap = nullptr;
            g.del_bits = 0;
            g.vid2doc = nullptr;
            g.n_vid2doc = 0;
            GH_CHECK(h, h->w_fbits.ensure((size_t)((nbits + 63) / 64) * 8));
            gh::launch_filter_bitmap(h->stream, g, nbits, h->w_fbits.as<uint8_t>());
            gh::RangeDesc& r = f->range[f->n_range++];
            r.bitmap = h->w_fbits.as<uint8_t>();
            r.min_doc = 0;
            r.max_doc = (int32_t)(nbits - 1);
            r.min_aligned = 0;
            r.b_not_in = 0;
            f->has_range = 1;
            f->n_field = 0;
            f->n_term = 0;
        }
    }
    return GAMMA_HIP_OK;
}

int filt_ctx_single(H* h, const gh::FilterDesc& f, FiltCtx* c) {
    GH_CHECK(h, h->w_ftab.ensure(sizeof(gh::FilterDesc)));
    if (!h->ftab_valid || memcmp(&h->ftab_shadow, &f, sizeof(f)) != 0) {
        h->ftab_shadow = f;
        h->ftab_valid = true;
        GH_CHECK(h, hipMemcpyAsync(h->w_ftab.p, &h->ftab_shadow, sizeof(f), hipMemcpyHostToDevice, h->stream));
    }
    c->d_tab = h->w_ftab.as<gh::FilterDesc>();
    c->d_qf = nullptr;
    c->any_clause = f.has_range || f.n_field > 0 || f.n_term > 0;
    return GAMMA_HIP_OK;
}

int check_params(H* h, const gamma_hip_search_params* p, int nq, int k) {
    if (!p) return fail(h, GAMMA_HIP_EINVAL, "null params");
    if (nq < 0) return fail(h, GAMMA_HIP_EINVAL, "nq < 0");
    if (p->metric != GAMMA_HIP_METRIC_IP && p->metric != GAMMA_HIP_METRIC_L2)
        return fail(h, GAMMA_HIP_EINVAL, "bad metric");
    if (k > 4096) return fail(h, GAMMA_HIP_EINVAL, "k > 4096 unsupported");
    return GAMMA_HIP_OK;
}

static inline bool tie_on(const gamma_hip_search_params* p) { return p->exact_ties > 0; }
int resolve_ties(H* h, const gamma_hip_search_params* p, gamma_hip_search_params* pp, bool in_range, const char* what) {
    *pp = *p;
    bool want = p->exact_ties != 0 ? p->exact_ties > 0 : h->exact_ties;
    if (want && !in_range) {
        if (p->exact_ties > 0) return fail(h, GAMMA_HIP_EUNSUPPORTED, what);
        h->ties_unhonoured.fetch_add(1, std::memory_order_relaxed);
        want = false;
    }
    pp->exact_ties = want ? 1 : -1;
    return GAMMA_HIP_OK;
}

int coarse_join(H* h) {
    if (h->coarse_join_pending) {
        GH_CHECK(h, hipStreamWaitEvent(h->stream, h->ev_join, 0));
        h->coarse_join_pending = false;
    }
    return GAMMA_HIP_OK;
}

int ivfpq_coarse(H* h, const gamma_hip_search_params* p, int nq, const float* d_x, float* out_dis = nullptr,
                 int* out_probe = nullptr, bool defer_join = false) {
    const int P = p->nprobe, d = h->d, nlist = h->nlist;
    hipStream_t s = h->stream;
    int mode = p->coarse_mode;
    if (mode < 0) mode = nq < 20 ? 0 : 1;
    const bool fused = mode == 1 && h->coarse_fused && gh::coarse_fused_supported(nq, d, nlist, P, tie_on(p));
    gh::CoarseFusedPlan plan;
    if (fused) {
        plan = gh::coarse_fused_plan(nq, nlist, P, h->coarse_cap, tie_on(p));
        GH_CHECK(h, h->w_mat.ensure(plan.bytes));
    } else {
        GH_CHECK(h, h->w_mat.ensure((size_t)nq * nlist * sizeof(float)));
    }
    if (!out_dis || !out_probe) {
        GH_CHECK(h, h->w_coarse_dis.ensure((size_t)nq * P * sizeof(float)));
        GH_CHECK(h, h->w_probe.ensure((size_t)nq * P * sizeof(int)));
        out_dis = h->w_coarse_dis.as<float>();
        out_probe = h->w_probe.as<int>();
    }
    StageScope t(h, GAMMA_HIP_STAGE_COARSE);
    if (fused) {
        static const bool no_side = getenv("GAMMA_HIP_NO_SIDE_STREAM") != nullptr;
        const bool side = tie_on(p) && defer_join && !no_side;
        gh::launch_coarse_fused(s, plan, h->w_mat.p, d_x, nq, d, h->d_cc, nlist, h->d_cc_norms, P, out_dis, out_probe,
                                tie_on(p), h->d_tie_stats, side ? h->side : nullptr, h->ev_fork, h->ev_join);
        h->coarse_join_pending = side;
        static const bool dbg = getenv("GAMMA_HIP_COARSE_DBG") != nullptr;
        if (dbg) {
            int n_ovf = 0;
            GH_CHECK(h, hipStreamSynchronize(s));
            GH_CHECK(h, hipMemcpy(&n_ovf, static_cast<char*>(h->w_mat.p) + plan.off_ovf, sizeof(int), hipMemcpyDeviceToHost));
            fprintf(stderr, "coarse fused: nlist %d nprobe %d sample %d strips %d: %d of %d queries repaired\n", nlist, P,
                    plan.sample, plan.nseg, n_ovf, nq);
        }
        return GAMMA_HIP_OK;
    }
    if (mode == 0) {
        gh::launch_pairwise(s, true, d_x, nq, d, h->d_cc, nlist, h->w_mat.as<float>(), nlist);
    } else {
        const float* xn = nullptr;
        if (d > 128) {
            GH_CHECK(h, h->w_xn.ensure((size_t)nq * sizeof(float)));
            gh::launch_row_norms(s, d_x, nq, d, h->w_xn.as<float>());
            xn = h->w_xn.as<float>();
        }
        gh::launch_l2_gemmform(s, d_x, nq, d, h->d_cc, nlist, xn, h->d_cc_norms,
                               h->w_mat.as<float>(), nlist, true);
    }
    if (tie_on(p)) GH_CHECK(h, h->w_tieflag.ensure((size_t)nq));
    static const bool no_side = getenv("GAMMA_HIP_NO_SIDE_STREAM") != nullptr;
    const bool side = tie_on(p) && defer_join && !no_side;
    h->coarse_join_pending = gh::launch_coarse_select(s, h->w_mat.as<float>(), nlist, nq, P, out_dis, out_probe,
                                                      tie_on(p) ? h->w_tieflag.as<uint8_t>() : nullptr, h->d_tie_stats,
                                                      side ? h->side : nullptr, h->ev_fork, h->ev_join);
    return GAMMA_HIP_OK;
}

struct BoundXchg {
    float* d_bound = nullptr;
    gamma_hip_bound_reduce_fn fn = nullptr;
    void* user = nullptr;
    bool called = false;
    bool two_phase = false;
    int P_in = 0;
    int G1 = 2;
    int reduce(H* h, int nq, bool l2) {
        called = true;
        const int rc = fn ? fn(user, d_bound, nq, l2 ? 0 : 1, (void*)h->stream) : 0;
        return rc ? fail(h, GAMMA_HIP_EDEVICE, "bound reduction callback failed") : GAMMA_HIP_OK;
    }
};

static int pq4_refuse(H* h, const char* what) {
    h->err = std::string("4-bit handle: ") + what + " is 8-bit only";
    return GAMMA_HIP_EUNSUPPORTED;
}
#define GH_NO_PQ4(h, what)                                                \
    do {                                                                  \
        if ((h)->ksub == gh::kPq4Ksub) return pq4_refuse((h), (what));    \
    } while (0)

int ivfpq_stage_a(H* h, const gamma_hip_search_params* p, const FiltCtx& fc, int nq,
                  const float* d_x, int R, const float* pre_dis = nullptr, const int* pre_probe = nullptr,
                  bool shard = false, float* out_dis = nullptr, int64_t* out_ids = nullptr, BoundXchg* bx = nullptr) {
    const int P = p->nprobe, d = h->d, M = h->M, nlist = h->nlist;
    const bool two = bx && bx->two_phase;
    const bool l2 = p->metric == GAMMA_HIP_METRIC_L2;
    const bool pq4 = h->ksub == gh::kPq4Ksub;
    if (pq4 && (shard || bx)) return pq4_refuse(h, "a list-shard search");
    hipStream_t s = h->stream;
    const int ver = h->cur_ver;
    GH_CHECK(h, hipStreamWaitEvent(s, h->ver_ev[ver], 0));
    GH_CHECK(h, h->w_coarse_dis.ensure((size_t)nq * P * sizeof(float)));
    GH_CHECK(h, h->w_probe.ensure((size_t)nq * P * sizeof(int)));
    GH_CHECK(h, h->w_pair_off.ensure((size_t)nq * (P + 1) * sizeof(int)));
    GH_CHECK(h, h->w_pair_base.ensure((size_t)nq * P * sizeof(int64_t)));
    GH_CHECK(h, h->w_qtotal.ensure((size_t)nq * sizeof(int)));
    GH_CHECK(h, h->w_cand_pos.ensure((size_t)nq * R * sizeof(int)));
    if (!out_dis) {
        GH_CHECK(h, h->w_cand_dis.ensure((size_t)nq * R * sizeof(float)));
        out_dis = h->w_cand_dis.as<float>();
    }
    if (!out_ids) {
        GH_CHECK(h, h->w_cand_ids.ensure((size_t)nq * R * sizeof(int64_t)));
        out_ids = h->w_cand_ids.as<int64_t>();
    }
    if (pre_dis && pre_probe) {
        if (shard) {
            gh::launch_compact_probes(s, pre_probe, pre_dis, nq, two ? bx->P_in : P, h->d_list_len, h->d_list_mask, nlist,
                                      h->w_probe.as<int>(), h->w_coarse_dis.as<float>(), P);
        } else {
            GH_CHECK(h, hipMemcpyAsync(h->w_coarse_dis.p, pre_dis, (size_t)nq * P * sizeof(float),
                                       hipMemcpyDeviceToDevice, s));
            GH_CHECK(h, hipMemcpyAsync(h->w_probe.p, pre_probe, (size_t)nq * P * sizeof(int),
                                       hipMemcpyDeviceToDevice, s));
        }
    } else {
        GH_TRY(ivfpq_coarse(h, p, nq, d_x, nullptr, nullptr, true));
    }
    h->scan_pairs += (int64_t)nq * P;
    const int need_ids =
            (!h->prefiltered && (fc.any_clause || (h->d_bitmap && h->bitmap_any) || h->n_moved > 0)) ? 1 : 0;
    const int* qperm = nullptr;
    double mean_len = (double)h->ntotal / std::max(1, nlist);
    int64_t owned = nlist;
    if (shard && !h->h_list_mask.empty()) {
        int64_t tot = 0;
        owned = 0;
        for (int l = 0; l < nlist; l++)
            if (h->h_list_len[l] > 0 && h->h_list_mask[l]) {
                owned++;
                tot += h->h_list_len[l];
            }
        mean_len = owned ? (double)tot / (double)owned : 0.0;
    }
    int G0 = (mean_len <= 700.0 && P <= 64) ? 8 : 4;
    static const bool no_c8 = getenv("GAMMA_HIP_NO_C8") != nullptr;
    constexpr int cf_maxr = 512;
    const bool c8_shape = !pq4 && !no_c8 && l2 && M == 16 && R <= cf_maxr && h->d_sums && h->d_t2max;
    if (G0 == 8 && c8_shape && P > 8) G0 = 5;
    int64_t t2_bytes = (int64_t)nlist * M * h->ksub * sizeof(float);
    const bool compacted = shard && pre_dis && pre_probe;
    if (two) {
        G0 = std::max(1, std::min(bx->G1, P));
        t2_bytes = owned * M * 256 * (int64_t)sizeof(float);
    } else if (compacted && h->scan_bound && R <= 256) {
        if (h->h_list_mask.empty()) {
            owned = 0;
            for (int l = 0; l < nlist; l++) owned += h->h_list_len[l] > 0;
        }
        t2_bytes = owned * M * 256 * (int64_t)sizeof(float);
        const double exp_probes = (double)P * (double)owned / std::max(1, nlist);
        const double exp_cand = exp_probes * mean_len;
        if (exp_cand <= 16384.0) {
            G0 = 1;
            while (G0 < P) G0 <<= 1;
        }
    }
    const int G = gh::scan_group_size(nq, P, G0), PGN = (P + G - 1) / G;
    h->tie = H::TieCtx();
    h->tie.on = tie_on(p);
    h->shard_cut_nq = (shard && h->tie.on) ? nq : 0;
    h->shard_cut_chunked = false;
    constexpr int scan_gmin = 4, bound_maxr = 1024;
    bool bounded = !pq4 && (!shard || compacted) && h->scan_bound && R <= bound_maxr && P <= 128 && G >= (two ? 1 : scan_gmin);
    if (bounded) {
        static const bool no_fb = getenv("GAMMA_HIP_NO_BOUND_FEEDBACK") != nullptr;
        const uint64_t sig = ((uint64_t)P << 40) ^ ((uint64_t)R << 20) ^ ((uint64_t)(l2 ? 1 : 0) << 1) ^ (fc.any_clause ? 1u : 0u) ^
                             ((uint64_t)(shard ? 1 : 0) << 2) ^ (1ull << 63);
        if (sig != h->bound_sig) {
            h->bound_sig = sig;
            h->bound_epoch++;
            h->bound_off_calls = 0;
            h->bound_calls = 0;
            h->bound_seen[0] = h->bound_seen[1] = 0;
            const int slot = h->bound_epoch & 1;
            if (h->bound_copy_pending) {
                (void)hipEventSynchronize(h->bound_copy_ev);
                h->bound_copy_pending = false;
// ... 1966 lines not shown
```

gamma_amd/csrc/gamma_hip_store.cpp:

```cpp
#include "binivf.h"
#include "gamma_hip_internal.h"
#include "pq4.h"

namespace ghi {


}
bool VmRange::reserve(int device_, size_t chunk_min) {
    hipMemAllocationProp prop = {};
    prop.type = hipMemAllocationTypePinned;
    prop.location.type = hipMemLocationTypeDevice;
    prop.location.id = device_;
    size_t g = 0, free_b = 0, total_b = 0;
    void* va = nullptr;
    if (hipMemGetAllocationGranularity(&g, &prop, hipMemAllocationGranularityRecommended) != hipSuccess || g == 0 ||
        hipMemGetInfo(&free_b, &total_b) != hipSuccess || total_b == 0) {
        (void)hipGetLastError();
        return false;
    }
    const size_t chunk = std::max<size_t>(std::max<size_t>(g, chunk_min), (size_t)2 << 20) / g * g;
    const size_t want = (total_b + chunk - 1) / chunk * chunk;
    if (hipMemAddressReserve(&va, want, 0, nullptr, 0) != hipSuccess || !va) {
        (void)hipGetLastError();
        return false;
// ... 940 lines not shown
    GH_CHECK(h, hipMalloc((void**)&np, ncap));
    GH_CHECK(h, hipMemsetAsync(np, 0, ncap, h->wstream));
    if (h->d_bitmap)
        GH_CHECK(h, hipMemcpyAsync(np, h->d_bitmap, h->bitmap_cap_bytes, hipMemcpyDeviceToDevice, h->wstream));
    GH_CHECK(h, hipStreamSynchronize(h->wstream));
    if (h->d_bitmap) GH_CHECK(h, hipFree(h->d_bitmap));
    h->d_bitmap = np;
    h->bitmap_cap_bytes = ncap;
    h->h_bitmap.resize(ncap, 0);
    return GAMMA_HIP_OK;
}

int gamma_hip_bitmap_upload(gamma_hip_index* h, const uint8_t* bitmap, int64_t nbits) {
    if (!h || nbits < 0 || (nbits > 0 && !bitmap)) return GAMMA_HIP_EINVAL;
    WriteLock lk(h);
    GH_CHECK(h, hipSetDevice(h->device));
    GH_TRY(bitmap_reserve(h, nbits));
    size_t bytes = ((size_t)nbits >> 3) + 1;
    GH_CHECK(h, hipMemsetAsync(h->d_bitmap, 0, h->bitmap_cap_bytes, h->wstream));
    GH_CHECK(h, hipMemcpyAsync(h->d_bitmap, bitmap, bytes, hipMemcpyHostToDevice, h->wstream));
    GH_CHECK(h, hipStreamSynchronize(h->wstream));
    std::fill(h->h_bitmap.begin(), h->h_bitmap.end(), 0);
    memcpy(h->h_bitmap.data(), bitmap, bytes);
    h->bitmap_bits = nbits;
    h->bitmap_any = false;
    for (size_t i = 0; i < bytes && !h->bitmap_any; i++) h->bitmap_any = bitmap[i] != 0;
    return GAMMA_HIP_OK;
}

int gamma_hip_bitmap_set(gamma_hip_index* h, const int64_t* docids, int64_t n, int value) {
    if (!h || n < 0 || (n > 0 && !docids)) return GAMMA_HIP_EINVAL;
    WriteLock lk(h);
    if (n == 0) return GAMMA_HIP_OK;
    GH_CHECK(h, hipSetDevice(h->device));
    int64_t mx = 0;
    for (int64_t i = 0; i < n; i++) mx = std::max(mx, docids[i]);
    if (mx >= h->bitmap_bits) {
        GH_TRY(bitmap_reserve(h, mx + 1));
        h->bitmap_bits = std::max<int64_t>(h->bitmap_bits, mx + 1);
    }
    GH_CHECK(h, h->we_stage.ensure((size_t)n * sizeof(int64_t)));
    GH_CHECK(h, hipMemcpyAsync(h->we_stage.p, docids, (size_t)n * sizeof(int64_t), hipMemcpyHostToDevice, h->wstream));
    gh::launch_bitmap_set(h->wstream, h->d_bitmap, h->we_stage.as<int64_t>(), n, h->bitmap_bits, value);
    GH_CHECK(h, hipStreamSynchronize(h->wstream));
    for (int64_t i = 0; i < n; i++) {
        int64_t id = docids[i];
        if (id < 0) continue;
        if (value) h->bitmap_any = true;
        if (value) h->h_bitmap[id >> 3] |= (uint8_t)(1u << (id & 7));
        else h->h_bitmap[id >> 3] &= (uint8_t)~(1u << (id & 7));
    }
    return GAMMA_HIP_OK;
}

static int ivf_init_locked(gamma_hip_index* h, int d, int nlist, int M, int metric, int bucket_init_size,
                           int bucket_max_size, bool flat, bool binary = false);
int gamma_hip_ivfpq_init(gamma_hip_index* h, int d, int nlist, int M, int nbits, int metric,
                         int bucket_init_size, int bucket_max_size) {
    if (!h) return GAMMA_HIP_EINVAL;
    WriteLock lk(h);
    if (h->ivf_init) return fail(h, GAMMA_HIP_EINVAL, "already initialised");
    if (d <= 0 || nlist <= 0 || M <= 0) return fail(h, GAMMA_HIP_EINVAL, "bad d/nlist/M");
    if (nbits != 8) return fail(h, GAMMA_HIP_EINVAL, "only nbits_per_idx == 8 is supported on device");
    if (d % M != 0) return fail(h, GAMMA_HIP_EINVAL, "d must be divisible by nsubvector");
    if (d / M > 64) return fail(h, GAMMA_HIP_EINVAL, "dsub > 64 unsupported");
    if (M > 64) return fail(h, GAMMA_HIP_EINVAL, "nsubvector > 64 unsupported (LUT must fit 64 KiB LDS)");
    return ivf_init_locked(h, d, nlist, M, metric, bucket_init_size, bucket_max_size, false);
}

static std::atomic<int64_t> g_table_max_bytes{(int64_t)1 << 31};
int gamma_hip_set_precomputed_table_max_bytes(int64_t bytes) {
    if (bytes < 0) return GAMMA_HIP_EINVAL;
    g_table_max_bytes.store(bytes);
    return GAMMA_HIP_OK;
}
int64_t gamma_hip_get_precomputed_table_max_bytes(void) { return g_table_max_bytes.load(); }
int gamma_hip_ivfpq_use_precomputed_table(gamma_hip_index* h) {
    if (!h || !h->ivf_init || h->ivfflat) return GAMMA_HIP_EINVAL;
    return h->table_mode;
}

int gamma_hip_ivfpq4_init(gamma_hip_index* h, int d, int nlist, int M, int metric, int bucket_init_size,
                          int bucket_max_size) {
    if (!h) return GAMMA_HIP_EINVAL;
    WriteLock lk(h);
    if (h->ivf_init) return fail(h, GAMMA_HIP_EINVAL, "already initialised");
    if (d <= 0 || nlist <= 0 || M <= 0) return fail(h, GAMMA_HIP_EINVAL, "bad d/nlist/M");
    if (d % M != 0) return fail(h, GAMMA_HIP_EINVAL, "d must be divisible by nsubvector");
    if (d / M > 64) return fail(h, GAMMA_HIP_EINVAL, "dsub > 64 unsupported");
    if (gh::pq4_code_size(M) > gh::kPq4MaxCodeSize)
        return fail(h, GAMMA_HIP_EINVAL, "4-bit codes: code_size = (4 * nsubvector + 7) / 8 > 64 unsupported");
    if ((int64_t)nlist * M * gh::kPq4Ksub * (int64_t)sizeof(float) > g_table_max_bytes.load())
        return fail(h, GAMMA_HIP_EUNSUPPORTED, "4-bit codes: the precomputed table would exceed precomputed_table_max_bytes (table mode 0 is 8-bit only)");
    h->ksub = gh::kPq4Ksub;
    const int rc = ivf_init_locked(h, d, nlist, M, metric, bucket_init_size, bucket_max_size, false);
    if (rc != GAMMA_HIP_OK) h->ksub = 256;
    return rc;
}

static int ivf_init_locked(gamma_hip_index* h, int d, int nlist, int M, int metric, int bucket_init_size,
                           int bucket_max_size, bool flat, bool binary) {
    if (metric != GAMMA_HIP_METRIC_IP && metric != GAMMA_HIP_METRIC_L2) return fail(h, GAMMA_HIP_EINVAL, "bad metric");
    GH_CHECK(h, hipSetDevice(h->device));
    h->ivfflat = flat;
    const int ksub = h->ksub;
    h->table_mode = (!flat && (int64_t)nlist * M * ksub * (int64_t)sizeof(float) > g_table_max_bytes.load()) ? 0 : 1;
    h->keep_sums = !flat && ksub == 256 && h->table_mode == 1 && getenv("GAMMA_HIP_NO_CODE_SUMS") == nullptr;
    h->d = d;
    h->nlist = nlist;
    h->M = M;
    h->dsub = d / M;
    h->code_size = ksub == gh::kPq4Ksub ? gh::pq4_code_size(M) : M;
    h->metric = metric;
    h->bucket_init = bucket_init_size > 0 ? bucket_init_size : 1000;
    h->bucket_max = bucket_max_size > 0 ? bucket_max_size : 1280000;
    if (!binary) {
        GH_CHECK(h, hipMalloc((void**)&h->d_cc, (size_t)nlist * d * sizeof(float)));
        GH_CHECK(h, hipMalloc((void**)&h->d_cc_norms, (size_t)nlist * sizeof(float)));
        GH_CHECK(h, hipMalloc((void**)&h->d_pqc, flat ? 256 : (size_t)M * ksub * h->dsub * sizeof(float)));
        if (flat || h->table_mode == 1)
            GH_CHECK(h, hipMalloc((void**)&h->d_T2, flat ? 256 : (size_t)nlist * M * ksub * sizeof(float)));
    }
    for (int v = 0; v < H::NVER; v++) {
        GH_CHECK(h, hipMalloc((void**)&h->d_ver_off[v], (size_t)nlist * sizeof(int64_t)));
        GH_CHECK(h, hipMalloc((void**)&h->d_ver_len[v], (size_t)nlist * sizeof(int)));
        GH_CHECK(h, hipHostMalloc(&h->pin_ver[v], (size_t)nlist * (sizeof(int64_t) + sizeof(int)), hipHostMallocDefault));
    }
    h->d_list_off = h->d_ver_off[0];
    h->d_list_len = h->d_ver_len[0];
    h->h_list_off.resize(nlist);
    h->h_list_len.assign(nlist, 0);
    h->h_list_cap.assign(nlist, h->bucket_init);
    h->h_deleted.assign(nlist, 0);
    h->h_extend_time.assign(nlist, 0);
    for (int l = 0; l < nlist; l++) h->h_list_off[l] = (int64_t)l * h->bucket_init;
    h->arena_used = 0;
    GH_TRY(arena_reserve(h, (int64_t)nlist * h->bucket_init));
    h->arena_used = (int64_t)nlist * h->bucket_init;
    GH_TRY(publish_meta(h));
    GH_CHECK(h, hipStreamSynchronize(h->wstream));
    h->vid_pos.assign((size_t)nlist * h->bucket_init, -1);
    h->ivf_init = true;
    return GAMMA_HIP_OK;
}

int gamma_hip_ivfflat_init(gamma_hip_index* h, int d, int nlist, int metric, int bucket_init_size, int bucket_max_size) {
    if (!h) return GAMMA_HIP_EINVAL;
    WriteLock lk(h);
    if (h->ivf_init) return fail(h, GAMMA_HIP_EINVAL, "already initialised");
    if (d <= 0 || nlist <= 0) return fail(h, GAMMA_HIP_EINVAL, "bad d/nlist");
    return ivf_init_locked(h, d, nlist, 1, metric, bucket_init_size, bucket_max_size, true);
}

int gamma_hip_ivfflat_set_trained(gamma_hip_index* h, const float* cc) {
    if (!h || !cc) return GAMMA_HIP_EINVAL;
    WriteLock lk(h);
    if (!h->ivf_init || !h->ivfflat || h->binivf) return fail(h, GAMMA_HIP_EINVAL, "ivfflat not initialised");
    GH_CHECK(h, hipSetDevice(h->device));
    GH_CHECK(h, hipMemcpyAsync(h->d_cc, cc, (size_t)h->nlist * h->d * sizeof(float), hipMemcpyHostToDevice, h->wstream));
    gh::launch_row_norms(h->wstream, h->d_cc, h->nlist, h->d, h->d_cc_norms);
    GH_CHECK(h, hipGetLastError());
    GH_CHECK(h, hipStreamSynchronize(h->wstream));
    h->trained = true;
    return GAMMA_HIP_OK;
}

int gamma_hip_binivf_init(gamma_hip_index* h, int nbits, int nlist, int bucket_init_size, int bucket_max_size) {
    if (!h) return GAMMA_HIP_EINVAL;
    WriteLock lk(h);
    if (h->ivf_init) return fail(h, GAMMA_HIP_EINVAL, "already initialised");
    if (nbits <= 0 || nbits % 8 != 0 || nbits / 8 > gh::kBinMaxCodeSize || nlist <= 0)
        return fail(h, GAMMA_HIP_EINVAL, "bad nbits / nlist (nbits % 8 == 0, at most 2048 bits)");
    GH_TRY(ivf_init_locked(h, nbits, nlist, nbits / 8, GAMMA_HIP_METRIC_L2, bucket_init_size, bucket_max_size, true, true));
    h->binivf = true;
    GH_CHECK(h, hipMalloc((void**)&h->d_bin_cc, (size_t)nlist * h->code_size));
    GH_CHECK(h, hipMalloc((void**)&h->d_bin_stats, 2 * sizeof(unsigned long long)));
    GH_CHECK(h, hipMemset(h->d_bin_stats, 0, 2 * sizeof(unsigned long long)));
    return GAMMA_HIP_OK;
}

int gamma_hip_binivf_set_trained(gamma_hip_index* h, const uint8_t* centroid_codes) {
    if (!h || !centroid_codes) return GAMMA_HIP_EINVAL;
    WriteLock lk(h);
    if (!h->ivf_init || !h->binivf) return fail(h, GAMMA_HIP_EINVAL, "binivf not initialised");
    GH_CHECK(h, hipSetDevice(h->device));
    GH_CHECK(h, hipMemcpyAsync(h->d_bin_cc, centroid_codes, (size_t)h->nlist * h->code_size, hipMemcpyHostToDevice,
                               h->wstream));
    GH_CHECK(h, hipStreamSynchronize(h->wstream));
    h->trained = true;
    return GAMMA_HIP_OK;
}

int gamma_hip_ivfpq_set_trained(gamma_hip_index* h, const float* cc, const float* pqc, const float* table) {
    if (!h || !cc || !pqc) return GAMMA_HIP_EINVAL;
    WriteLock lk(h);
    if (!h->ivf_init || h->ivfflat) return fail(h, GAMMA_HIP_EINVAL, "ivfpq not initialised");
    GH_CHECK(h, hipSetDevice(h->device));
    const size_t ncc = (size_t)h->nlist * h->d, npq = (size_t)h->M * h->ksub * h->dsub;
    const size_t nt = (size_t)h->nlist * h->M * h->ksub;
    GH_CHECK(h, hipMemcpyAsync(h->d_cc, cc, ncc * sizeof(float), hipMemcpyHostToDevice, h->wstream));
    GH_CHECK(h, hipMemcpyAsync(h->d_pqc, pqc, npq * sizeof(float), hipMemcpyHostToDevice, h->wstream));
    gh::launch_row_norms(h->wstream, h->d_cc, h->nlist, h->d, h->d_cc_norms);
    if (h->table_mode == 0) {
    } else if (table)
        GH_CHECK(h, hipMemcpyAsync(h->d_T2, table, nt * sizeof(float), hipMemcpyHostToDevice, h->wstream));
    else if (h->ksub == gh::kPq4Ksub)
        gh::launch_pq4_precompute_table(h->wstream, h->d_cc, h->nlist, h->d, h->M, h->d_pqc, h->d_T2);
    else
        gh::launch_precompute_table(h->wstream, h->d_cc, h->nlist, h->d, h->M, h->d_pqc, h->d_T2);
    {
        std::vector<int> rank = centroid_rank(cc, h->nlist, h->d);
        if (!h->d_list_rank) GH_CHECK(h, hipMalloc((void**)&h->d_list_rank, (size_t)h->nlist * sizeof(int)));
        GH_CHECK(h, hipMemcpyAsync(h->d_list_rank, rank.data(), (size_t)h->nlist * sizeof(int),
                                   hipMemcpyHostToDevice, h->wstream));
        GH_CHECK(h, hipStreamSynchronize(h->wstream));
    }
    if (h->keep_sums) {
        if (!h->d_t2max) GH_CHECK(h, hipMalloc((void**)&h->d_t2max, (size_t)h->nlist * sizeof(float)));
        gh::launch_t2_rowmax(h->wstream, h->d_T2, h->nlist, h->M, h->d_t2max);
    }
    GH_CHECK(h, hipGetLastError());
    GH_CHECK(h, hipStreamSynchronize(h->wstream));
    h->t2max_all = 0.f;
    if (h->keep_sums && h->d_t2max) {
        std::vector<float> tm((size_t)h->nlist);
        GH_CHECK(h, hipMemcpy(tm.data(), h->d_t2max, tm.size() * sizeof(float), hipMemcpyDeviceToHost));
        for (float v : tm) h->t2max_all = std::max(h->t2max_all, v);
    }
    h->trained = true;
    if (h->ntotal > 0) {
        GH_TRY(sums_all_lists(h));
        GH_CHECK(h, hipStreamSynchronize(h->wstream));
    }
    return GAMMA_HIP_OK;
}

int gamma_hip_ivfpq_get_precomputed_table(gamma_hip_index* h, float* out) {
    if (!h || !out) return GAMMA_HIP_EINVAL;
    WriteLock lk(h);
    if (!h->trained) return fail(h, GAMMA_HIP_ENOTTRAINED, "not trained");
    if (h->table_mode == 0) return fail(h, GAMMA_HIP_EUNSUPPORTED, "table mode 0: no precomputed table (it would exceed precomputed_table_max_bytes)");
    GH_CHECK(h, hipSetDevice(h->device));
    GH_CHECK(h, hipMemcpyAsync(out, h->d_T2, (size_t)h->nlist * h->M * h->ksub * sizeof(float),
                               hipMemcpyDeviceToHost, h->wstream));
    GH_CHECK(h, hipStreamSynchronize(h->wstream));
    return GAMMA_HIP_OK;
}

int gamma_hip_ivfpq_add_keys(gamma_hip_index* h, int list_no, int n, const int64_t* vids, const uint8_t* codes) {
    if (!h || (n > 0 && (!vids || !codes))) return GAMMA_HIP_EINVAL;
    WriteLock lk(h);
    if (!h->ivf_init) return fail(h, GAMMA_HIP_EINVAL, "ivfpq not initialised");
    GH_CHECK(h, hipSetDevice(h->device));
    return add_keys_locked(h, list_no, n, vids, codes);
}

int gamma_hip_ivfpq_add_keys_batch(gamma_hip_index* h, int nlists, const int32_t* list_nos,
                                   const int32_t* counts, const int64_t* vids, const uint8_t* codes) {
    if (!h || nlists < 0 || (nlists > 0 && (!list_nos || !counts || !vids || !codes))) return GAMMA_HIP_EINVAL;
    WriteLock lk(h);
    if (!h->ivf_init) return fail(h, GAMMA_HIP_EINVAL, "ivfpq not initialised");
    GH_CHECK(h, hipSetDevice(h->device));
    int64_t off = 0;
    {
        std::map<int, int64_t> per_list;
        for (int i = 0; i < nlists; i++) {
            if (list_nos[i] < 0 || list_nos[i] >= h->nlist || counts[i] < 0) return fail(h, GAMMA_HIP_EINVAL, "bad list_no");
            per_list[list_nos[i]] += counts[i];
        }
        for (auto& kv : per_list) {
            if (kv.second > h->bucket_max) return fail(h, GAMMA_HIP_EFULL, "exceed the max bucket keys");
            GH_TRY(list_ensure(h, kv.first, (int)kv.second));
        }
    }
    std::vector<int> r_list, r_n;
    std::vector<int64_t> r_pos;
    int r_max = 0;
    for (int i = 0; i < nlists; i++) {
        const int l = list_nos[i], n = counts[i];
        if (n == 0) continue;
        const int64_t pos = h->h_list_off[l] + h->h_list_len[l];
        r_list.push_back(l);
        r_n.push_back(n);
        r_pos.push_back(pos);
        r_max = std::max(r_max, n);
        GH_CHECK(h, hipMemcpyAsync(h->d_ids + pos, vids + off, (size_t)n * sizeof(int64_t), hipMemcpyHostToDevice, h->wstream));
        GH_CHECK(h, hipMemcpyAsync(h->d_codes + pos * h->code_size, codes + off * h->code_size,
                                   (size_t)n * h->code_size, hipMemcpyHostToDevice, h->wstream));
        for (int j = 0; j < n; j++) {
            const int64_t v = vids[off + j];
            if (v < 0) {
                h->h_deleted[l]++;
                h->n_moved++;
                continue;
            }
            if ((size_t)v >= h->vid_pos.size()) h->vid_pos.resize(std::max<size_t>(h->vid_pos.size() * 2, v + 1), -1);
            h->vid_pos[v] = ((int64_t)l << 32) | (int64_t)(h->h_list_len[l] + j);
            if (h->doc_deleted(v)) h->h_deleted[l]++;
        }
        h->h_list_len[l] += n;
        h->ntotal += n;
        if (h->h_list_len[l] > h->max_list_len) h->max_list_len = h->h_list_len[l];
        off += n;
    }
    if (h->d_sums && h->trained && !r_list.empty()) {
        const size_t nr = r_list.size(), o_n = nr * sizeof(int), o_pos = (2 * nr * sizeof(int) + 7) & ~(size_t)7;
        GH_CHECK(h, h->we_stage.ensure(o_pos + nr * sizeof(int64_t)));
        char* b = h->we_stage.as<char>();
        GH_CHECK(h, hipMemcpyAsync(b, r_list.data(), nr * sizeof(int), hipMemcpyHostToDevice, h->wstream));
        GH_CHECK(h, hipMemcpyAsync(b + o_n, r_n.data(), nr * sizeof(int), hipMemcpyHostToDevice, h->wstream));
        GH_CHECK(h, hipMemcpyAsync(b + o_pos, r_pos.data(), nr * sizeof(int64_t), hipMemcpyHostToDevice, h->wstream));
        gh::launch_code_sums_ranges(h->wstream, h->d_T2, h->d_codes, h->code_size, reinterpret_cast<int*>(b),
                                    reinterpret_cast<int64_t*>(b + o_pos), reinterpret_cast<int*>(b + o_n), (int)nr, r_max,
                                    h->d_sums);
    }
    GH_TRY(publish_meta(h));
    GH_CHECK(h, hipStreamSynchronize(h->wstream));
    return arena_repack_if_need(h);
}

int gamma_hip_ivfpq_update(gamma_hip_index* h, int list_no, int64_t vid, const uint8_t* code) {
    if (!h || !code) return GAMMA_HIP_EINVAL;
    WriteLock lk(h);
    if (!h->ivf_init || list_no < 0 || list_no >= h->nlist) return fail(h, GAMMA_HIP_EINVAL, "bad list_no");
    if (vid < 0 || (size_t)vid >= h->vid_pos.size()) return GAMMA_HIP_OK;
    const int64_t bp = h->vid_pos[vid];
    if (bp == -1) return GAMMA_HIP_OK;
    GH_CHECK(h, hipSetDevice(h->device));
    const int ob = (int)(bp >> 32), op = (int)(bp & 0xffffffff);
    if (ob == list_no) {
        GH_CHECK(h, hipMemcpyAsync(h->d_codes + (h->h_list_off[ob] + op) * h->code_size, code, h->code_size,
                                   hipMemcpyHostToDevice, h->wstream));
        GH_TRY(sums_range(h, ob, h->h_list_off[ob] + op, 1));
        GH_CHECK(h, hipStreamSynchronize(h->wstream));
        return GAMMA_HIP_OK;
    }
    GH_TRY(list_ensure(h, list_no, 1));
    gh::launch_mark_moved(h->wstream, h->d_ids, h->h_list_off[ob] + op);
    h->h_deleted[ob]++;
    h->n_moved++;
    h->ntotal -= 1;
    return add_keys_locked(h, list_no, 1, &vid, code);
}

int gamma_hip_ivfpq_apply_updates(gamma_hip_index* h, int n, const int32_t* list_nos, const int64_t* vids,
                                  const uint8_t* codes, const uint8_t* ops) {
    if (!h || n < 0 || (n > 0 && (!list_nos || !vids || !codes))) return GAMMA_HIP_EINVAL;
    if (n == 0) return GAMMA_HIP_OK;
    WriteLock lk(h);
    if (!h->ivf_init) return fail(h, GAMMA_HIP_EINVAL, "ivfpq not initialised");
    GH_CHECK(h, hipSetDevice(h->device));
    const int cs = h->code_size;
    {
        std::map<int, int64_t> per_list;
        for (int i = 0; i < n; i++) {
// ... 377 lines not shown
```

gamma_amd/csrc/kernels.h:

```cpp
#pragma once
#include <atomic>
#include <hip/hip_runtime.h>
#include <stdint.h>

namespace gh {

void launch_refused(const char* what);
const char* launch_refused_take();


inline bool first_call_on_device(std::atomic<uint64_t>& done) {
    int dev = 0;
    (void)hipGetDevice(&dev);
    const uint64_t bit = 1ull << (dev & 63);
    return (done.fetch_or(bit) & bit) == 0;
}

constexpr int kMaxRange = 8;

struct RangeDesc {
    const uint8_t* bitmap;
    int32_t min_doc, max_doc, min_aligned, b_not_in;
};

// ... 36 lines not shown
void launch_pairwise_filtered(hipStream_t s, bool l2, const float* x, int nq, int d,
                              const float* y, int64_t ny, float* out, int64_t ld_out,
                              const FilterDesc& filt, float min_score, float max_score,
                              int64_t row_base);
struct FlatEmit {
    const uint32_t* tau;
    unsigned long long* cand;
    int* cnt;
    int cap;
    int cstride = 1;
};
bool pairwise_can_emit(int nq, int d, int64_t ny);
int flat_list_cap();
void launch_pairwise_emit(hipStream_t s, bool l2, const float* x, int nq, int d, const float* y, int64_t ny,
                          const FilterDesc& filt, float min_score, float max_score, int64_t row_base,
                          const FlatEmit& em);
void launch_flat_init(hipStream_t s, bool l2, const float* vals, const int* pos, int nq, int k, int64_t r0,
                      const FlatEmit& em, uint32_t* tau, int* kept = nullptr);
struct FlatLog {
    unsigned long long* items = nullptr;
    int* cnt = nullptr;
    int* kept = nullptr;
    int nsl = 0, pass = 0;
    unsigned long long* dbg = nullptr;
};
void launch_flat_compact(hipStream_t s, int nq, int k, const FlatEmit& em, uint32_t* tau, int* overflow,
                         const FlatLog* log = nullptr);
void launch_flat_final(hipStream_t s, bool l2, int nq, int k, const FlatEmit& em, float neutral, float* distances,
                       int64_t* labels);
void launch_row_norms(hipStream_t s, const float* y, int64_t n, int d, float* out);
bool flat_filter_supported(int nq, int d, int64_t ny);
int64_t flat_filter_pair_cap(int nq);
int flat_filter_counter_bytes();
size_t flat_filter_query_image_bytes(int nq, int d);
void launch_flat_prep_queries(hipStream_t s, const float* x, int nq, int d, void* image);
size_t flat_filter_bounds_bytes(int nq);
void launch_flat_filter(hipStream_t s, bool l2, int d, const void* qimage, const float* xn, const uint32_t* tau, float* bounds,
                        int nq, const float* y, int64_t ny, int64_t row_base, void* pairs, int* npairs, int64_t cap);
void launch_flat_exact(hipStream_t s, bool l2, const void* pairs, const int* npairs, int64_t cap, const float* x, int nq, int d,
                       const float* store, const FilterDesc& filt, float min_score, float max_score, const FlatEmit& em,
                       int* overflow);
inline int gemm_k_split(int d) { return (d > 384 && d <= 768 && d % 8 == 0) ? d / 2 : 0; }
void launch_l2_gemmform(hipStream_t s, const float* x, int nq, int d, const float* y, int64_t ny,
                        const float* xn, const float* yn, float* out, int64_t ld_out,
                        bool use_mfma);
void launch_pq_ip_table(hipStream_t s, const float* x, int nq, int d, int M, const float* pqc,
                        float* out);
void launch_precompute_table(hipStream_t s, const float* cc, int nlist, int d, int M,
                             const float* pqc, float* out);
struct PairZero {
    uint8_t* bytes = nullptr;
    unsigned long long* words = nullptr;
    int* count_a = nullptr;
    int* count_b = nullptr;
    const int* qo_rank = nullptr;
    int* qo_key = nullptr;
    int* qo_bins = nullptr;
};
void launch_pair_offsets(hipStream_t s, const int* probe_list, int nq, int P, const int* list_len,
                         const uint8_t* list_mask, int nlist, int* pair_off, int* q_total,
                         unsigned long long* scan_codes, const int64_t* list_off = nullptr,
                         int64_t* pair_base = nullptr, const PairZero* zero = nullptr);
void launch_compact_probes(hipStream_t s, const int* probe_in, const float* cdis_in, int nq, int P,
                           const int* list_len, const uint8_t* list_mask, int nlist, int* probe_out,
                           float* cdis_out, int P_out = 0);
void launch_bound_export(hipStream_t s, bool l2, const unsigned long long* ready, int nq, float* out);
void launch_bound_import(hipStream_t s, bool l2, const float* in, int nq, unsigned long long* ready);
void launch_fill_f32(hipStream_t s, float* p, int n, float v);
void launch_bound_combine(hipStream_t s, float* acc, const float* in, int n, int take_max);
void launch_pair_ip(hipStream_t s, const float* x, const float* cc, const int* probe_list, int nq, int P, int d,
                    int nlist, float* out);
struct ScanBound {
    unsigned long long* ready;
    unsigned long long* surv;
    int* gcnt;
    int K;
    int cnt_stride;
    int store_all;
    int* rq_list;
    int* rq_count;
    const float* sums;
    const float* t2max;
    int cf_span;
    unsigned long long* timeouts;
    int slice_cap;
    int part;
    int dbg_part;
    int c8;
    const int64_t* pair_base;
    float t2max_all;
};
struct Q8Args {
    int nq, P, G, M, nlist;
    double mean_len;
    const int* probe_list;
    const float* coarse_dis;
    const float* st2;
    const float* pqc = nullptr;
    int d = 0;
    const float* xd = nullptr;
    const float* T2;
    const float* t2max;
    const float* sums;
    const uint8_t* codes;
    const int64_t* ids;
    const int64_t* list_off;
    const int* list_len;
    const uint8_t* list_mask;
    const int* pair_off;
    const unsigned long long* ready;
    const FilterDesc* ftab;
    int need_ids;
    unsigned long long* surv;
    int* gcnt;
    int cnt_stride, slice_cap;
    int* rq_list;
    int* rq_count;
    uint8_t* q8;
    float4* meta;
    uint32_t* cand;
    int* iwork;
};
bool q8_supported(int M, int P, int G, int64_t q_stride);
int q8_cand_cap(int nq);
size_t q8_int_words(int nq, int P, int G, int nlist);
void launch_q8_consumers(hipStream_t s, const Q8Args& a);
int scan_slice_cap(int K);
bool scan_cf_applies(bool l2, int M, int P, int G, bool have_sums, bool store_all);
int scan_group_size(int nq, int P, int G0 = 8);
void launch_ivfpq_scan_pair(hipStream_t s, bool l2, const float* x, int nq, int d, int M, int P,
                            const int* probe_list, const float* coarse_dis, const float* cc,
                            const float* st2, const float* T2, const int64_t* list_off,
                            const int* list_len, const uint8_t* list_mask, int nlist,
                            const uint8_t* codes, const int64_t* ids, const int* pair_off,
                            int64_t q_stride, float* out, const FilterDesc* ftab , const int* qfil ,
                            int need_ids,
                            const int* qperm, int G, int pg_lo, int pg_cnt, int sparse, const ScanBound* bound,
                            const float* pqc_fused = nullptr,
                            const int* rq_list = nullptr, const int* rq_count = nullptr,
                            int chunk_len = 0, int max_units = 0);
int query_order_bins();
bool query_order_grid(int nq);
void launch_query_order(hipStream_t s, const int* probe_list, int nq, int P, const int* list_rank,
                        int nlist, int* qkey, int* qperm, int* bins = nullptr, bool hist_done = false);
void launch_sum_totals(hipStream_t s, const int* q_total, int nq, unsigned long long* acc);
void launch_max_local_total(hipStream_t s, const int* probe_list, int nq, int P, const int* list_len,
                            const uint8_t* list_mask, int nlist, int* out_max);
int select_kpad(int K);
constexpr int kCoarseCap = 128, kCoarseRepairGrid = 256;
struct CoarseFusedPlan {
    int sample, nseg, tiles_per_strip, cap, cap_stride;
    size_t off_mat, off_tau, off_cand, off_cnt, off_ovf, off_scratch, off_full, bytes;
};
bool coarse_fused_supported(int nq, int d, int nlist, int P, bool exact_ties = false);
CoarseFusedPlan coarse_fused_plan(int nq, int nlist, int P, int cap, bool exact_ties = false);
void launch_coarse_heap_rows(hipStream_t s, const float* mat, int nlist, int nq, int K, const int* rows, float* out_vals,
                             int* out_pos, unsigned long long* tie_stats);
void launch_coarse_fused(hipStream_t s, const CoarseFusedPlan& pl, void* ws, const float* x, int nq, int d,
                         const float* y, int nlist, const float* yn, int P, float* out_dis, int* out_idx,
                         bool exact_ties = false, unsigned long long* tie_stats = nullptr,
                         hipStream_t side = nullptr, hipEvent_t fork = nullptr, hipEvent_t join = nullptr);
bool launch_small_coarse_ip(hipStream_t s, const float* x, int nq, int d, const float* cc, int nlist, float* mat, int M,
                            const float* pqc, float* st2, int* zero_me = nullptr);
void launch_small_coarse_select(hipStream_t s, const float* mat, int nlist, int nq, int P, float* out_vals, int* out_pos,
                                const int* list_len, const uint8_t* list_mask, const int64_t* list_off, int* pair_off,
                                int* q_total, int64_t* pair_base, const float* x = nullptr, const float* cc = nullptr,
                                int d = 0, float* pair_ip = nullptr, uint32_t* units = nullptr, int* unit_count = nullptr,
                                int chunk_len = 0, int exact_ties = 0, unsigned long long* tie_stats = nullptr);
struct TieReplayArgs;
void launch_small_tail(hipStream_t s, bool l2, const float* slab, int64_t q_stride, const int* q_total, int nq, int R, int P,
                       const int* probe_list, const int* pair_off, const int64_t* list_off, const int64_t* ids,
                       float* cand_dis, int* cand_pos, int64_t* cand_ids, int has_rank, const float* x, int d,
                       const float* raw, int64_t nraw, int k, float min_score, float max_score, float neutral,
                       float* distances, int64_t* labels, int smax = 0, float* pre_val = nullptr, int* pre_pos = nullptr,
                       int fixed_n = 0,
                       const TieReplayArgs* tr = nullptr,
                       unsigned long long* tie_stats = nullptr);
void launch_ivfflat_scan(hipStream_t s, bool l2, const float* x, int nq, int d, int P, const int* pair_off,
                         const int64_t* pair_base, const int64_t* ids, const float* raw, int64_t nraw, int64_t q_stride,
                         float* out, const FilterDesc* ftab, int need_filter, float min_score, float max_score);
bool ivfflat_lm_supported(int d);
size_t ivfflat_lm_scratch_bytes(int nq, int P, int nlist);
void launch_ivfflat_lm(hipStream_t s, bool l2, const float* x, int nq, int d, int P, const int* probe, const int* pair_off,
                       const int64_t* list_off, const int* list_len, int nlist, const int64_t* ids, const float* raw,
                       int64_t nraw, int64_t q_stride, float* out, const FilterDesc* ftab, int need_filter, float min_score,
                       float max_score, void* scratch);
bool launch_coarse_select(hipStream_t s, const float* mat, int nlist, int nq, int K, float* out_vals, int* out_pos,
                          uint8_t* tie_flag, unsigned long long* tie_stats = nullptr, hipStream_t side = nullptr,
                          hipEvent_t fork = nullptr, hipEvent_t join = nullptr);
void launch_select_topk(hipStream_t s, bool smallest, const float* vals, int64_t seg_stride,
                        const int* seg_len, int fixed_len, int max_len, int nseg, int K,
                        float* out_vals, int* out_pos, const uint8_t* only = nullptr);
void launch_select_final(hipStream_t s, bool smallest, const unsigned long long* surv, const int* gcnt,
                         int nslices, int slice_cap, const unsigned long long* ready, const int* pair_off, int P,
                         int nq, int K, const int64_t* pair_base, const int64_t* ids, uint8_t* flag, float* out_vals,
                         int* out_pos, int64_t* out_ids, uint8_t* cut_tie = nullptr,
                         unsigned long long* tie_stats = nullptr, int* rq_list = nullptr, int* rq_count = nullptr, unsigned long long* bound_stat = nullptr);
void launch_map_candidates(hipStream_t s, const int* pos, int nq, int R, int P,
                           const int* probe_list, const int* pair_off, const int64_t* list_off,
                           const int64_t* ids, int64_t* cand_ids, const uint8_t* only = nullptr);
void launch_rerank_dist(hipStream_t s, bool l2, const float* x, int nq, int d, const float* raw,
                        int64_t nraw, const int64_t* cand_ids, int R, float min_score,
                        float max_score, float* out, const int32_t* slot = nullptr, int64_t nslot = 0);
void launch_export_exact(hipStream_t s, bool l2, const float* xf, int nf, int d, const float* raw, const int32_t* slot, int64_t nslot,
                         const float* vals, const int64_t* ids, int64_t stride, const int32_t* off, int P, const float* bound, float* ex);
void launch_lookup_exact(hipStream_t s, bool l2, const float* all_dis, const int64_t* all_ids, const float* all_exact, int W, int nq, int R,
                         int q0, int nql, const float* cand_dis, const int64_t* cand_ids, float* cand_exact);
struct TieFlags {
    const uint8_t* cut = nullptr;
    int* list = nullptr;
    int* count = nullptr;
    unsigned long long* stats = nullptr;
};
void launch_rerank_topk(hipStream_t s, bool l2, const float* x, int nq, int d, const float* raw,
                        int64_t nraw, const int64_t* cand_ids, int R, int k, float min_score,
                        float max_score, float neutral, float* distances, int64_t* labels,
                        const int* qperm = nullptr,
                        const TieFlags* ties = nullptr);
struct TieReplayArgs {
    const int* list;
    const int* count;
    int nq;
    const float* slab;
    int64_t q_stride;
    const int* pair_off;
    const int64_t* pair_base;
    const int64_t* ids;
    int P, G;
    const unsigned long long* ready;
    const unsigned long long* surv;
    const int* gcnt;
    int nsl, slice_cap;
    const float* x;
    int d;
    const float* raw;
    int64_t nraw;
    const float* ex_slab = nullptr;
    int* ex_missing = nullptr;
    int R, k, has_rank;
    float min_score, max_score, neutral;
    float* cand_dis;
    int64_t* cand_ids;
    float* distances;
    int64_t* labels;
    unsigned long long* dbg = nullptr;
    int pop_push = 0;
    int fixed_n = 0;
    int compact_rows = 0;
    int always_sliced = 0;
};
int tie_replay_max_k();
int tie_small_max_k();
void launch_tie_list(hipStream_t s, const uint8_t* cut, const uint8_t* extra, int nq, int* list, int* count,
                     unsigned long long* tie_stats);
void launch_debug_heap_stream(hipStream_t s, int op, int k, int n, const float* vals, uint2* out_arr, uint2* out_sorted);
int tie_replay_max_probes();
void launch_tie_replay(hipStream_t s, bool l2, const TieReplayArgs& a);
void launch_flag_cut_ties(hipStream_t s, const float* slab, int64_t q_stride, const int* q_total, int nq, int K,
                          const float* sel_vals, const int* sel_pos, const uint8_t* only, uint8_t* tflag,
                          int fixed_n = 0, int inside = 0);
int coarse_heap_max_k();
size_t tie_replay_lds_bytes(int R, int k, int P);
void launch_flat_take_flag(hipStream_t s, const float* D1, const int64_t* I1, int nq, int k, float* distances, int64_t* labels,
                           int* list, int* count, unsigned long long* tie_stats);
void launch_flag_merge_cut(hipStream_t s, const float* all_dis, int W, int nq, int R, int q0, int nql, const float* merged,
                           const int64_t* merged_ids, uint8_t* tcut, const uint8_t* shard_flags = nullptr);
void launch_shard_export(hipStream_t s, const int32_t* probe, int nf, int P, const int* list_len, const int64_t* list_off,
                         const uint8_t* list_mask, int nlist, const int64_t* ids, const float* slab, int64_t q_stride,
                         int64_t stride, float* vals, int64_t* out_ids, int32_t* off);
void launch_shard_export_rows(hipStream_t s, const int32_t* probe, int nf, int P, const int* list_len, const uint8_t* list_mask,
                              int nlist, int* max_entries);
void launch_merge_streams(hipStream_t s, int W, int nf, int P, int64_t stride, int64_t mstride, const float* vals, const int64_t* ids,
                          const int32_t* off, float* m_vals, int64_t* m_ids, int32_t* m_off, int64_t* m_base, float sentinel);
void launch_gather_words(hipStream_t s, const void* src, const int* list, int n, int words, void* out);
void launch_gather_rows(hipStream_t s, const float* x, const int* list, int n, int d, float* out);
void launch_finalize_topk(hipStream_t s, const float* sel_vals, const int* sel_pos, int nq, int k,
                          const int64_t* src_ids, int64_t src_stride, int64_t id_base,
                          float neutral, float* distances, int64_t* labels);
void launch_finalize_norank(hipStream_t s, const float* cand_dis, const int64_t* cand_ids, int nq,
                            int R, int k, float min_score, float max_score, float neutral,
                            float* distances, int64_t* labels, const TieFlags* ties = nullptr);
void launch_gather_shards(hipStream_t s, const float* all_dis, const int64_t* all_ids, int nshards,
                          int nq, int R, float* dis, int64_t* ids, float sentinel);
bool launch_merge_shards(hipStream_t s, bool smallest, const float* all_dis, const int64_t* all_ids, int W,
                         int nq, int R, int q0, int nql, float* out_dis, int64_t* out_ids);
void launch_take_ids(hipStream_t s, const int* pos, const int64_t* src_ids, int64_t src_stride,
                     int nq, int R, int64_t* out);
void launch_bitmap_set(hipStream_t s, uint8_t* bm, const int64_t* docids, int64_t n, int64_t nbits,
                       int value);
void launch_mark_moved(hipStream_t s, int64_t* ids, int64_t pos);
void launch_raw_slot_scatter(hipStream_t s, const int32_t* pairs, int64_t n, int32_t* tab, int64_t ntab);
void launch_raw_rows_scatter(hipStream_t s, const float* stage, const int32_t* pairs, int64_t n, int d, float* raw, int64_t cap);
void launch_list_checksum(hipStream_t s, const uint8_t* codes, const int64_t* ids, const int64_t* off, const int* len, int nlist,
                          int M, int max_len, unsigned long long* out);
void launch_repack_lists(hipStream_t s, const uint8_t* oc, const int64_t* oi, uint8_t* nc, int64_t* ni,
                         const int64_t* old_off, const int64_t* new_off, const int* len, int nlist, int M,
                         int max_len);
void launch_code_sums_ranges(hipStream_t s, const float* T2, const uint8_t* codes, int M, const int* list_no, const int64_t* pos,
                             const int* n, int nranges, int max_n, float* sums);
void launch_code_sums_one(hipStream_t s, const float* T2, const uint8_t* codes, int M, int list_no, int64_t pos, int n,
                          float* sums);
void launch_code_sums_lists(hipStream_t s, const float* T2, const uint8_t* codes, int M, const int64_t* list_off,
                            const int* list_len, int nlist, int max_len, float* sums);
void launch_t2_rowmax(hipStream_t s, const float* T2, int nlist, int M, float* t2max);
void launch_centroid_update(hipStream_t s, const float* x, int d, const int* order, const int* seg, int k, float* centroids,
                            float* hassign);
void launch_pq_encode(hipStream_t s, const float* x, int64_t n, int d, int M, const int* assign,
                      const float* cc, const float* pqc, uint8_t* codes);

}
```

include/gamma_hip.h:

```cpp
#ifndef GAMMA_HIP_H_
#define GAMMA_HIP_H_

#include <stddef.h>
#include <stdint.h>

#ifdef __cplusplus
extern "C" {
#endif

#define GAMMA_HIP_METRIC_IP 0
#define GAMMA_HIP_METRIC_L2 1

#define GAMMA_HIP_OK 0
#define GAMMA_HIP_EINVAL (-1)
#define GAMMA_HIP_ENOTTRAINED (-2)
#define GAMMA_HIP_EDEVICE (-3)
#define GAMMA_HIP_ENOMEM (-4)
#define GAMMA_HIP_EFULL (-5)
#define GAMMA_HIP_EUNSUPPORTED (-6)

typedef struct gamma_hip_index gamma_hip_index;

typedef struct {
    const uint8_t* bitmap;
    int64_t bitmap_bytes;
    int32_t min_doc, max_doc, min_aligned;
    int32_t b_not_in;
} gamma_hip_range_filter;

#define GAMMA_HIP_FIELD_INT 0
#define GAMMA_HIP_FIELD_LONG 1
#define GAMMA_HIP_FIELD_FLOAT 2
#define GAMMA_HIP_FIELD_DOUBLE 3
#define GAMMA_HIP_MAX_FIELD_FILTERS 8
typedef struct {
    int32_t field_id;
    int32_t include_lower, include_upper;
    int32_t reserved;
    int64_t lower_i, upper_i;
    double lower_f, upper_f;
} gamma_hip_field_filter;

#define GAMMA_HIP_MAX_TERM_FILTERS 8
#define GAMMA_HIP_MAX_TERM_ITEMS 16
#define GAMMA_HIP_TERM_AND 0
#define GAMMA_HIP_TERM_OR 1
#define GAMMA_HIP_TERM_NOT 2
typedef struct {
    int32_t field_id;
    int32_t op;
    int32_t n_items;
    int32_t items[GAMMA_HIP_MAX_TERM_ITEMS];
} gamma_hip_term_filter;

typedef struct {
    int32_t metric;
    int32_t nprobe;
    int32_t recall_num;
    int32_t has_rank;
    float min_score;
    float max_score;
    int32_t coarse_mode;
    int32_t has_range;
    int32_t n_range;
    const gamma_hip_range_filter* range;
    int32_t n_field;
    int32_t n_term;
    const gamma_hip_field_filter* field;
    const gamma_hip_term_filter* term;
    int32_t exact_ties;
} gamma_hip_search_params;

int gamma_hip_create(int device, gamma_hip_index** out);
int gamma_hip_destroy(gamma_hip_index* h);
const char* gamma_hip_strerror(int code);
const char* gamma_hip_last_error(gamma_hip_index* h);
void* gamma_hip_stream(gamma_hip_index* h);
int gamma_hip_synchronize(gamma_hip_index* h);

int gamma_hip_set_scan_bound_feedback(gamma_hip_index* h, int on);
int gamma_hip_scan_bound_stats(gamma_hip_index* h, int64_t* out4);
int gamma_hip_set_workspace_budget(gamma_hip_index* h, int64_t bytes);
int gamma_hip_set_exact_ties(gamma_hip_index* h, int on);
int gamma_hip_set_coarse_fused(gamma_hip_index* h, int on, int list_cap);
int gamma_hip_set_small_path(gamma_hip_index* h, int on);
int gamma_hip_tie_stats(gamma_hip_index* h, int64_t* out3, int reset);
int gamma_hip_ties_not_honoured(gamma_hip_index* h, int64_t* out_calls, int reset);
int gamma_hip_blas_form_not_restated(gamma_hip_index* h, int64_t* out_calls, int reset);

int gamma_hip_field_append(gamma_hip_index* h, int field_id, int dtype, int64_t n, const void* values);
int gamma_hip_field_update(gamma_hip_index* h, int field_id, int64_t docid, const void* value);
int64_t gamma_hip_field_count(gamma_hip_index* h, int field_id);
int gamma_hip_term_append(gamma_hip_index* h, int field_id, int64_t n_docs, const int32_t* counts,
                          const int32_t* items);
int64_t gamma_hip_term_count(gamma_hip_index* h, int field_id);
int gamma_hip_term_update(gamma_hip_index* h, int field_id, int64_t docid, int32_t count, const int32_t* items);

int gamma_hip_raw_init(gamma_hip_index* h, int d);
int gamma_hip_raw_append(gamma_hip_index* h, int64_t n, const float* vecs);
int gamma_hip_raw_update(gamma_hip_index* h, int64_t vid, const float* vec);
int gamma_hip_raw_update_batch(gamma_hip_index* h, int64_t n, const int64_t* vids, const float* vecs);
int gamma_hip_raw_write(gamma_hip_index* h, int64_t first_vid, int64_t n, const float* vecs);
int gamma_hip_raw_gets(gamma_hip_index* h, int64_t n, const int64_t* vids, float* out);
int gamma_hip_raw_put(gamma_hip_index* h, int64_t n, const int64_t* vids, const float* vecs);
int gamma_hip_raw_drop(gamma_hip_index* h, int64_t n, const int64_t* vids);
int gamma_hip_raw_clear(gamma_hip_index* h);
int gamma_hip_raw_sparse_stats(gamma_hip_index* h, int64_t* out3);
int64_t gamma_hip_raw_count(gamma_hip_index* h);
int gamma_hip_raw_stats(gamma_hip_index* h, int64_t* out4);

int gamma_hip_bitmap_upload(gamma_hip_index* h, const uint8_t* bitmap, int64_t nbits);
int gamma_hip_bitmap_set(gamma_hip_index* h, const int64_t* docids, int64_t n, int value);

int gamma_hip_ivfpq_init(gamma_hip_index* h, int d, int nlist, int M, int nbits, int metric,
                         int bucket_init_size, int bucket_max_size);
int gamma_hip_ivfpq4_init(gamma_hip_index* h, int d, int nlist, int M, int metric, int bucket_init_size,
                          int bucket_max_size);
int gamma_hip_ivfpq_set_trained(gamma_hip_index* h, const float* coarse_centroids,
                                const float* pq_centroids, const float* precomputed_table);
int gamma_hip_ivfpq_get_precomputed_table(gamma_hip_index* h, float* out);
int gamma_hip_set_precomputed_table_max_bytes(int64_t bytes);
int64_t gamma_hip_get_precomputed_table_max_bytes(void);
int gamma_hip_ivfpq_use_precomputed_table(gamma_hip_index* h);
int gamma_hip_ivfpq_dim(gamma_hip_index* h);
int gamma_hip_ivfpq_nlist(gamma_hip_index* h);
int gamma_hip_ivfpq_code_size(gamma_hip_index* h);

int gamma_hip_ivfpq_add_keys(gamma_hip_index* h, int list_no, int n, const int64_t* vids,
                             const uint8_t* codes);
int gamma_hip_ivfpq_add_keys_batch(gamma_hip_index* h, int nlists, const int32_t* list_nos,
                                   const int32_t* counts, const int64_t* vids,
                                   const uint8_t* codes);
int gamma_hip_ivfpq_update(gamma_hip_index* h, int list_no, int64_t vid, const uint8_t* code);
int gamma_hip_ivfpq_has_vid(gamma_hip_index* h, const int64_t* vids, int n, uint8_t* out);
int gamma_hip_ivfpq_update_batch(gamma_hip_index* h, int n, const int64_t* vids, const float* vecs);
int gamma_hip_ivfpq_encode_each(gamma_hip_index* h, int64_t n, const float* vecs, int64_t* list_nos, uint8_t* codes);
int gamma_hip_ivfpq_apply_updates(gamma_hip_index* h, int n, const int32_t* list_nos, const int64_t* vids,
                                  const uint8_t* codes, const uint8_t* ops);
int gamma_hip_ivfpq_remove(gamma_hip_index* h, int64_t vid);
int gamma_hip_ivfpq_delete(gamma_hip_index* h, const int64_t* vids, int n);
int gamma_hip_ivfpq_compact_if_need(gamma_hip_index* h);
int gamma_hip_ivfpq_arena_stats(gamma_hip_index* h, int64_t* out4);
int gamma_hip_ivfpq_set_repack_threshold(gamma_hip_index* h, int64_t min_waste_entries);
int gamma_hip_ivfpq_repack_verify_stats(gamma_hip_index* h, int64_t* out2);
int gamma_hip_ivfpq_arena_growth(gamma_hip_index* h, int64_t* out2);
int64_t gamma_hip_ivfpq_list_size(gamma_hip_index* h, int list_no);
int64_t gamma_hip_ivfpq_list_capacity(gamma_hip_index* h, int list_no);
int gamma_hip_ivfpq_get_list(gamma_hip_index* h, int list_no, int64_t* vids, uint8_t* codes);
int gamma_hip_ivfpq_set_list_mask(gamma_hip_index* h, const uint8_t* owned);

int gamma_hip_ivfpq_add(gamma_hip_index* h, int64_t n, const float* vecs, int64_t first_vid);
int gamma_hip_ivfpq_encode(gamma_hip_index* h, int64_t n, const float* vecs, int64_t* list_nos,
                           uint8_t* codes);

int gamma_hip_assign(gamma_hip_index* h, int d, int64_t n, const float* x, int k,
                     const float* centroids, int32_t* assign, float* dis);

int gamma_hip_kmeans(gamma_hip_index* h, int d, int64_t n, const float* x, int k, int niter, int64_t seed,
                     int max_points_per_centroid, float* centroids, float* objective);
int gamma_hip_ivfpq_train(gamma_hip_index* h, int d, int64_t n, const float* x, int nlist, int M, float* coarse, float* pq);
void gamma_hip_rand_perm(int32_t* perm, int64_t n, int64_t seed);

int gamma_hip_vid2docid_append(gamma_hip_index* h, int64_t n, const int32_t* docids);
int64_t gamma_hip_vid2docid_count(gamma_hip_index* h);

int gamma_hip_ivfflat_init(gamma_hip_index* h, int d, int nlist, int metric, int bucket_init_size,
                           int bucket_max_size);
int gamma_hip_ivfflat_set_trained(gamma_hip_index* h, const float* coarse_centroids);
int gamma_hip_ivfflat_search(gamma_hip_index* h, const gamma_hip_search_params* p, int nq, const float* x, int k,
                             float* distances, int64_t* labels);
int gamma_hip_ivfflat_search_device(gamma_hip_index* h, const gamma_hip_search_params* p, int nq, const float* d_x,
                                    int k, float* d_distances, int64_t* d_labels);

int gamma_hip_binivf_init(gamma_hip_index* h, int nbits, int nlist, int bucket_init_size, int bucket_max_size);
int gamma_hip_binivf_train(gamma_hip_index* h, int nbits, int64_t n, const uint8_t* codes, int nlist, uint8_t* centroid_codes);
int gamma_hip_binivf_set_trained(gamma_hip_index* h, const uint8_t* centroid_codes);
int gamma_hip_binivf_assign(gamma_hip_index* h, int64_t n, const uint8_t* codes, int k, int32_t* distances, int64_t* labels);
int gamma_hip_binivf_add(gamma_hip_index* h, int64_t n, const uint8_t* codes, int64_t first_vid);
int gamma_hip_binivf_search(gamma_hip_index* h, const gamma_hip_search_params* p, int nq, const uint8_t* x, int k,
                            float* distances, int64_t* labels);
int gamma_hip_binivf_search_device(gamma_hip_index* h, const gamma_hip_search_params* p, int nq, const uint8_t* d_x, int k,
                                   float* d_distances, int64_t* d_labels);
int gamma_hip_binivf_stats(gamma_hip_index* h, int64_t* out2, int reset);

int gamma_hip_ivfpq_search(gamma_hip_index* h, const gamma_hip_search_params* p, int nq,
                           const float* x, int k, float* distances, int64_t* labels);
int gamma_hip_ivfpq_search_device(gamma_hip_index* h, const gamma_hip_search_params* p, int nq,
                                  const float* d_x, int k, float* d_distances, int64_t* d_labels);
int gamma_hip_set_deferred_replay(gamma_hip_index* h, int on);
int gamma_hip_ivfpq_search_device_wait(gamma_hip_index* h, const gamma_hip_search_params* p, int nq,
                                       const float* d_x, int k, float* d_distances, int64_t* d_labels);
int gamma_hip_flat_search_device_wait(gamma_hip_index* h, const gamma_hip_search_params* p, int nq,
                                      const float* d_x, int k, float* d_distances, int64_t* d_labels);
int gamma_hip_join(gamma_hip_index* h);
int gamma_hip_ivfpq_last_stages(gamma_hip_index* h, float* coarse_dis, int64_t* coarse_idx,
                                float* recall_dis, int64_t* recall_ids);
int gamma_hip_ivfpq_search_shard(gamma_hip_index* h, const gamma_hip_search_params* p, int nq,
                                 const float* d_x, int k, float* d_recall_dis,
                                 int64_t* d_recall_ids);
int gamma_hip_ivfpq_coarse_device(gamma_hip_index* h, const gamma_hip_search_params* p, int nq,
                                  const float* d_x, float* d_coarse_dis, int32_t* d_probe);
int gamma_hip_ivfpq_search_shard_preassigned(gamma_hip_index* h, const gamma_hip_search_params* p,
                                             int nq, const float* d_x, const float* d_coarse_dis,
                                             const int32_t* d_probe, int k, float* d_recall_dis,
                                             int64_t* d_recall_ids);
typedef int (*gamma_hip_bound_reduce_fn)(void* user, float* d_bound, int nq, int take_max, void* stream);
int gamma_hip_ivfpq_search_shard_bounded(gamma_hip_index* h, const gamma_hip_search_params* p,
                                         int nq, const float* d_x, const float* d_coarse_dis,
                                         const int32_t* d_probe, int k, float* d_recall_dis,
                                         int64_t* d_recall_ids, float* d_bound,
                                         gamma_hip_bound_reduce_fn reduce, void* user);
int gamma_hip_bound_combine(void* stream, float* d_acc, const float* d_in, int n, int take_max);
int gamma_hip_ivfpq_shard_exact(gamma_hip_index* h, const gamma_hip_search_params* p, int nq, const float* d_x,
                                const int64_t* d_ids, int R, float* d_exact);
int gamma_hip_ivfpq_merge_rerank_exact(gamma_hip_index* h, const gamma_hip_search_params* p, int nshards, int nq,
                                       const float* d_x, int k, const float* d_all_dis, const int64_t* d_all_ids,
                                       const float* d_all_exact, int q0, int nq_local, float* d_distances, int64_t* d_labels);
int gamma_hip_ivfpq_shard_export_exact(gamma_hip_index* h, const gamma_hip_search_params* p, int nf, const float* d_xf,
                                       const float* d_vals, const int64_t* d_ids, const int32_t* d_off, int64_t stride,
                                       const float* d_bound_f, float* d_ex);
int gamma_hip_ivfpq_merge_replay_exact(gamma_hip_index* h, const gamma_hip_search_params* p, int nshards, int nf,
                                       const float* d_x_slice, int64_t stride, const float* d_vals_all, const int64_t* d_ids_all,
                                       const int32_t* d_off_all, const float* d_ex_all, int k, const int32_t* d_list,
                                       float* d_distances, int64_t* d_labels);
int gamma_hip_ivfpq_merge_rerank(gamma_hip_index* h, const gamma_hip_search_params* p,
                                 int nshards, int nq, const float* d_x, int k,
                                 const float* d_all_dis, const int64_t* d_all_ids, int q0,
                                 int nq_local, float* d_distances, int64_t* d_labels);

int gamma_hip_flat_search(gamma_hip_index* h, const gamma_hip_search_params* p, int nq,
                          const float* x, int k, float* distances, int64_t* labels);
int gamma_hip_flat_search_device(gamma_hip_index* h, const gamma_hip_search_params* p, int nq,
                                 const float* d_x, int k, float* d_distances, int64_t* d_labels);

int gamma_hip_debug_heap_stream(gamma_hip_index* h, int op, int k, int n, const float* vals, float* arr_vals, int32_t* arr_ids,
                                float* sorted_vals, int32_t* sorted_ids);
int gamma_hip_ivfpq_shard_cut_flags(gamma_hip_index* h, int nq, uint8_t* d_flags);
// ... 61 lines not shown
```

Before: 11.23 million.

## Add split-bf16 MFMA coarse filter with exact fp32 rescoring and adaptive backoff

Adds a precomputed split-bf16 (hi/lo) image of the coarse centroids and a new MFMA kernel that computes coarse L2 bounds with three bf16 MFMAs per k-step. Candidates within a safety margin of the per-query threshold are kept, and the final selection re-scores boundary candidates in exact fp32 so results stay correct. The kernel is meant to cut the cost of the coarse distance GEMM. Overflow and give-up counts are copied back asynchronously, and the path backs off to fp32 when too many queries fall through. This adds extra rescoring work, an image build at train time, and host-side bookkeeping.

```diff
diff --git a/gamma_amd/_lib.py b/gamma_amd/_lib.py
--- a/gamma_amd/_lib.py
+++ b/gamma_amd/_lib.py
@@ -62,6 +62,7 @@
     "gamma_hip_ivfpq_set_repack_threshold": (C.c_int, [C.c_void_p, C.c_int64]),
     "gamma_hip_set_small_path": (C.c_int, [C.c_void_p, C.c_int]),
     "gamma_hip_set_coarse_fused": (C.c_int, [C.c_void_p, C.c_int, C.c_int]),
+    "gamma_hip_coarse_filter_stats": (C.c_int, [C.c_void_p, i64p]),
     "gamma_hip_tie_stats": (C.c_int, [C.c_void_p, i64p, C.c_int]),
     "gamma_hip_ties_not_honoured": (C.c_int, [C.c_void_p, i64p, C.c_int]),
     "gamma_hip_blas_form_not_restated": (C.c_int, [C.c_void_p, i64p, C.c_int]),
diff --git a/gamma_amd/api.py b/gamma_amd/api.py
--- a/gamma_amd/api.py
+++ b/gamma_amd/api.py
@@ -537,7 +537,12 @@
         self._ck(self.L.gamma_hip_set_workspace_budget(self.h, int(nbytes)), "set_workspace_budget")
 
     def set_coarse_fused(self, on=True, list_cap=128):
-        self._ck(self.L.gamma_hip_set_coarse_fused(self.h, 1 if on else 0, list_cap), "set_coarse_fused")
+        self._ck(self.L.gamma_hip_set_coarse_fused(self.h, int(on), list_cap), "set_coarse_fused")
+
+    def coarse_filter_stats(self):
+        out = np.zeros(4, np.int64)
+        self._ck(self.L.gamma_hip_coarse_filter_stats(self.h, _p(out, _lib.i64p)), "coarse_filter_stats")
+        return dict(zip(["given_up", "queries", "backoffs", "fp32_calls_left"], [int(v) for v in out]))
 
     def set_small_path(self, on=True):
         self._ck(self.L.gamma_hip_set_small_path(self.h, int(on)), "set_small_path")
diff --git a/gamma_amd/csrc/bf16_split.h b/gamma_amd/csrc/bf16_split.h
--- /dev/null
+++ b/gamma_amd/csrc/bf16_split.h
@@ -0,0 +1,26 @@
+#pragma once
+#include <hip/hip_runtime.h>
+#include <stdint.h>
+
+namespace gh {
+
+typedef __attribute__((__vector_size__(8 * sizeof(__bf16)))) __bf16 bf16x8;
+
+__device__ __forceinline__ uint32_t cvt_pk_bf16(float lo, float hi) {
+    uint32_t r;
+    asm("v_cvt_pk_bf16_f32 %0, %1, %2" : "=v"(r) : "v"(lo), "v"(hi));
+    return r;
+}
+__device__ __forceinline__ void split_bf16x8(const float* f, uint4& hi, uint4& lo) {
+    uint32_t h[4], l[4];
+#pragma unroll
+    for (int i = 0; i < 4; i++) {
+        h[i] = cvt_pk_bf16(f[2 * i], f[2 * i + 1]);
+        const float h0 = __uint_as_float(h[i] << 16), h1 = __uint_as_float(h[i] & 0xffff0000u);
+        l[i] = cvt_pk_bf16(f[2 * i] - h0, f[2 * i + 1] - h1);
+    }
+    hi = make_uint4(h[0], h[1], h[2], h[3]);
+    lo = make_uint4(l[0], l[1], l[2], l[3]);
+}
+
+}
diff --git a/gamma_amd/csrc/coarse.hip b/gamma_amd/csrc/coarse.hip
--- a/gamma_amd/csrc/coarse.hip
+++ b/gamma_amd/csrc/coarse.hip
@@ -6,6 +6,7 @@
 #include <algorithm>
 #include <type_traits>
 
+#include "bf16_split.h"
 #include "device_math.h"
 #include "heap_dev.h"
 #include "kernels.h"
@@ -196,6 +197,148 @@
 }
 
 
+__global__ __launch_bounds__(256) void k_coarse_image(const float* __restrict__ y, const float* __restrict__ yn, int ny,
+                                                      int ny_pad, int D, char* __restrict__ img, float* __restrict__ hc) {
+    const int KK = D / 16;
+    const int idx = blockIdx.x * 256 + threadIdx.x;
+    if (idx >= ny_pad * (D / 8)) return;
+    const int c = idx / (D / 8), kg = idx % (D / 8);
+    float f[8];
+#pragma unroll
+    for (int t = 0; t < 8; t++) f[t] = c < ny ? y[(int64_t)c * D + kg * 8 + t] : 0.f;
+    uint4 hi, lo;
+    split_bf16x8(f, hi, lo);
+    const int kh = kg / KK, kk = kg % KK, j = c & 31;
+    char* base = img + (int64_t)(c >> 5) * (D * 128);
+    *reinterpret_cast<uint4*>(base + ((((0 * KK + kk) * 2 + kh) * 32 + j) * 16)) = hi;
+    *reinterpret_cast<uint4*>(base + ((((1 * KK + kk) * 2 + kh) * 32 + j) * 16)) = lo;
+    if (kg == 0) hc[c] = c < ny ? (1.f - kCoarseBfMargin) * yn[c] : __uint_as_float(0x7fc00000u);
+}
+
+template <int NCH>
+__global__ __launch_bounds__(256, 2) void k_coarse_filter_bf16(const float* __restrict__ x, int nq,
+                                                               const char* __restrict__ img, const float* __restrict__ hc,
+                                                               int ny, int col0, const float* __restrict__ tau,
+                                                               int tiles_per_strip, int cap, int cap_stride,
+                                                               unsigned long long* __restrict__ cand,
+                                                               int* __restrict__ cand_cnt, int nseg) {
+    constexpr int D = 16 * NCH, KK = NCH, BLK = D * 128, TILE = 2 * BLK;
+    constexpr int LPT = TILE / (256 * 16);
+    static_assert(TILE % (256 * 16) == 0, "tile staged by whole rounds of the workgroup");
+    extern __shared__ __attribute__((aligned(16))) char s_cimg[];
+    const int tid = threadIdx.x, lane = tid & 63, w = tid >> 6, kh = lane >> 5, j = lane & 31;
+    const int seg = blockIdx.x, q_base = blockIdx.y * 128;
+    const int ntiles = (ny - col0 + 63) >> 6;
+    const int t0 = seg * tiles_per_strip, t1 = min(ntiles, t0 + tiles_per_strip);
+    auto stage = [&](int t, int b) {
+        const char* src = img + (int64_t)((col0 >> 6) + t) * TILE + (w * LPT) * 1024 + lane * 16;
+        char* dst = s_cimg + b * TILE + (w * LPT) * 1024;
+#pragma unroll
+        for (int u = 0; u < LPT; u++)
+            __builtin_amdgcn_global_load_lds((const __attribute__((address_space(1))) void*)(src + u * 1024),
+                                             (__attribute__((address_space(3))) void*)(dst + u * 1024), 16, 0, 0);
+    };
+    if (t0 < t1) stage(t0, 0);
+    bf16x8 ah[KK], al[KK];
+    float a_row, t_row;
+    int ok_row;
+    {
+        const int row = q_base + w * 32 + j;
+        const float* xp = x + (int64_t)min(row, nq - 1) * D + (D / 2) * kh;
+        float ss = 0.f;
+#pragma unroll
+        for (int kk = 0; kk < KK; kk++) {
+            const float4 v0 = *reinterpret_cast<const float4*>(xp + 8 * kk);
+            const float4 v1 = *reinterpret_cast<const float4*>(xp + 8 * kk + 4);
+            const float f[8] = {v0.x, v0.y, v0.z, v0.w, v1.x, v1.y, v1.z, v1.w};
+#pragma unroll
+            for (int t = 0; t < 8; t++) ss = __builtin_fmaf(f[t], f[t], ss);
+            uint4 hi, lo;
+            split_bf16x8(f, hi, lo);
+            ah[kk] = __builtin_bit_cast(bf16x8, hi);
+            al[kk] = __builtin_bit_cast(bf16x8, lo);
+        }
+        const float xn = ss + __shfl_xor(ss, 32, 64);
+        ok_row = (xn >= kCoarseBfXnMin && xn <= kCoarseBfNormMax) ? 1 : 0;
+        a_row = (1.f - kCoarseBfMargin) * xn;
+        t_row = (row < nq && ok_row) ? tau[row] : -INFINITY;
+        if (row >= nq) ok_row = 1;
+    }
+    float ar[16], tr[16];
+    int bad = 0;
+#pragma unroll
+    for (int r = 0; r < 16; r++) {
+        const int i = (r & 3) + 8 * (r >> 2) + 4 * kh;
+        ar[r] = __shfl(a_row, i, 64);
+        tr[r] = __shfl(t_row, i, 64);
+        bad |= __shfl(ok_row, i, 64) ? 0 : (1 << r);
+    }
+    int cnt[16];
+#pragma unroll
+    for (int r = 0; r < 16; r++) cnt[r] = 0;
+    const uint32_t lt_mask = (1u << j) - 1u;
+    const unsigned row_stride = (unsigned)nseg * (unsigned)cap_stride;
+    const unsigned lane_row = ((unsigned)((q_base + w * 32 + 4 * kh) * nseg + seg)) * (unsigned)cap_stride;
+    const __amdgpu_buffer_rsrc_t rsrc = __builtin_amdgcn_make_buffer_rsrc(
+        cand, 0, (int)min((int64_t)nq * nseg * cap_stride * 8, (int64_t)0x7fffffff), 0x00020000);
+    constexpr unsigned OOB = 0x80000000u;
+    const int sh = lane & 32;
+    int rs[16];
+#pragma unroll
+    for (int r = 0; r < 16; r++) rs[r] = ((r & 3) + 8 * (r >> 2)) * (int)row_stride * 8;
+    __syncthreads();
+    for (int t = t0; t < t1; t++) {
+        const int b = (t - t0) & 1;
+        const int colb = col0 + t * 64;
+        float hcv[2];
+        hcv[0] = hc[colb + j];
+        hcv[1] = hc[colb + 32 + j];
+        if (t + 1 < t1) stage(t + 1, b ^ 1);
+        f32x16 acc[2];
+#pragma unroll
+        for (int nt = 0; nt < 2; nt++)
+#pragma unroll
+            for (int r = 0; r < 16; r++) acc[nt][r] = 0.f;
+        const char* tb = s_cimg + b * TILE + (kh * 32 + j) * 16;
+#pragma unroll
+        for (int kk = 0; kk < KK; kk++) {
+#pragma unroll
+            for (int nt = 0; nt < 2; nt++) {
+                const bf16x8 bh = *reinterpret_cast<const bf16x8*>(tb + nt * BLK + ((0 * KK + kk) * 2) * 512);
+                const bf16x8 bl = *reinterpret_cast<const bf16x8*>(tb + nt * BLK + ((1 * KK + kk) * 2) * 512);
+                acc[nt] = __builtin_amdgcn_mfma_f32_32x32x16_bf16(al[kk], bh, acc[nt], 0, 0, 0);
+                acc[nt] = __builtin_amdgcn_mfma_f32_32x32x16_bf16(ah[kk], bl, acc[nt], 0, 0, 0);
+                acc[nt] = __builtin_amdgcn_mfma_f32_32x32x16_bf16(ah[kk], bh, acc[nt], 0, 0, 0);
+            }
+        }
+#pragma unroll
+        for (int nt = 0; nt < 2; nt++) {
+            const unsigned colv = (unsigned)(colb + nt * 32 + j);
+#pragma unroll
+            for (int r = 0; r < 16; r++) {
+                const float L = __builtin_fmaf(-2.f, acc[nt][r], ar[r] + hcv[nt]);
+                const bool pass = L <= tr[r];
+                const unsigned long long mask = __ballot(pass);
+                const uint32_t mh = (uint32_t)(mask >> sh);
+                const unsigned slot = min((unsigned)cnt[r] + (unsigned)__popc(mh & lt_mask), (unsigned)cap);
+                u32x2 item;
+                item.x = colv;
+                item.y = __float_as_uint(L);
+                __builtin_amdgcn_raw_buffer_store_b64(item, rsrc, pass ? (lane_row + slot) * 8u : OOB, rs[r], 0);
+                cnt[r] += __popc(mh);
+            }
+        }
+        __syncthreads();
+    }
+    if (j == 0) {
+#pragma unroll
+        for (int r = 0; r < 16; r++) {
+            const int row = q_base + w * 32 + (r & 3) + 8 * (r >> 2) + 4 * kh;
+            if (row < nq) cand_cnt[row * nseg + seg] = ((bad >> r) & 1) ? cap + 1 : cnt[r];
+        }
+    }
+}
+
 __device__ __forceinline__ uint32_t wave_kth_smallest(uint32_t m, int K) {
     int lt = 0, le = 0;
 #pragma unroll
@@ -243,22 +386,42 @@
 }
 
 constexpr int CF_BUF = 256;
-template <int SNPL, int MAXSEG>
+template <int SNPL, int MAXSEG, bool BF = false>
 __global__ __launch_bounds__(256) void k_coarse_final(const float* __restrict__ mat, const float* __restrict__ tau,
                                                       const unsigned long long* __restrict__ cand,
                                                       const int* __restrict__ cand_cnt, int nseg, int cap,
                                                       int cap_stride, int nq, int P, float* __restrict__ out_dis,
-                                                      int* __restrict__ out_idx, int* __restrict__ ovf, int flag_ties) {
+                                                      int* __restrict__ out_idx, int* __restrict__ ovf, int flag_ties,
+                                                      const float* __restrict__ x, const float* __restrict__ y,
+                                                      const float* __restrict__ yn, int d, float yn_max,
+                                                      unsigned long long* __restrict__ stat) {
     constexpr int NPL = SNPL + 2 * MAXSEG;
     __shared__ unsigned long long s_buf[4][CF_BUF];
+    __shared__ __attribute__((aligned(16))) float s_xq[BF ? 4 : 1][BF ? 128 : 1];
     const int lane = threadIdx.x & 63, w = threadIdx.x >> 6;
     const int q = blockIdx.x * 4 + w;
+    if (BF && blockIdx.x == 0 && threadIdx.x == 0) atomicAdd(stat + 1, (unsigned long long)nq);
     if (q >= nq) return;
     unsigned long long* buf = s_buf[w];
     const int cnt = lane < nseg ? cand_cnt[q * nseg + lane] : 0;
     if (__ballot(cnt > cap)) {
-        if (lane == 0) ovf[1 + atomicAdd(ovf, 1)] = q;
+        if (lane == 0) {
+            ovf[1 + atomicAdd(ovf, 1)] = q;
+            if (BF) atomicAdd(stat, 1ull);
+        }
         return;
+    }
+    float margin = 0.f;
+    if constexpr (BF) {
+        float ss = 0.f;
+        for (int k = lane; k < d; k += 64) {
+            const float xv = x[(int64_t)q * d + k];
+            s_xq[w][k] = xv;
+            ss = __builtin_fmaf(xv, xv, ss);
+        }
+#pragma unroll
+        for (int o = 32; o > 0; o >>= 1) ss += __shfl_xor(ss, o, 64);
+        margin = 2.f * kCoarseBfMargin * 1.0009765625f * (ss + yn_max);
     }
     unsigned long long it[NPL];
     {
@@ -277,6 +440,13 @@
         const int e0 = (lane - 4 * sg) & 63;
         it[SNPL + 2 * sg] = e0 < c ? p[e0] : ~0ull;
         it[SNPL + 2 * sg + 1] = e0 + 64 < c ? p[e0 + 64] : ~0ull;
+        if constexpr (BF) {
+#pragma unroll
+            for (int h2 = 0; h2 < 2; h2++) {
+                unsigned long long& v = it[SNPL + 2 * sg + h2];
+                if (v != ~0ull) v = ((unsigned long long)f2key(__uint_as_float((uint32_t)(v >> 32))) << 32) | (uint32_t)v;
+            }
+        }
     }
     uint32_t m0 = 0xffffffffu, m1 = 0xffffffffu;
 #pragma unroll
@@ -286,14 +456,20 @@
         if (g1) m1 = k < m1 ? k : m1;
         else m0 = k < m0 ? k : m0;
     }
-    const uint32_t kb = P <= 32 ? wave_kth_smallest(m0 < m1 ? m0 : m1, P) : wave_kth_smallest2(m0, m1, P);
+    uint32_t kb = P <= 32 ? wave_kth_smallest(m0 < m1 ? m0 : m1, P) : wave_kth_smallest2(m0, m1, P);
+    if constexpr (BF) {
+        if (kb != 0xffffffffu) kb = f2key(key2f(kb) + margin);
+    }
     int c = 0;
 #pragma unroll
     for (int j = 0; j < NPL; j++) c += ((uint32_t)(it[j] >> 32) <= kb && it[j] != ~0ull) ? 1 : 0;
     const int incl = wave_incl_scan_i(c);
     const int tot = __shfl(incl, 63, 64);
     if (tot > CF_BUF) {
-        if (lane == 0) ovf[1 + atomicAdd(ovf, 1)] = q;
+        if (lane == 0) {
+            ovf[1 + atomicAdd(ovf, 1)] = q;
+            if (BF) atomicAdd(stat, 1ull);
+        }
         return;
     }
     int off = incl - c;
@@ -301,6 +477,37 @@
     for (int j = 0; j < NPL; j++)
         if ((uint32_t)(it[j] >> 32) <= kb && it[j] != ~0ull) buf[off++] = it[j];
     __builtin_amdgcn_wave_barrier();
+    if constexpr (BF) {
+        const float* sx = s_xq[w];
+        const int l4 = lane & 3;
+        float nacc = 0.f;
+        for (int i = 0; i < d; i += 4) {
+            const float xv = sx[i + l4];
+            nacc = __builtin_fmaf(xv, xv, nacc);
+        }
+        const float t01 = nacc + __shfl_down(nacc, 1, 4);
+        const float xn = __shfl(t01 + __shfl_down(t01, 2, 4), 0, 64);
+        for (int e = lane; e < tot; e += 64) {
+            const uint32_t col = (uint32_t)buf[e];
+            if (col >= (uint32_t)(64 * SNPL)) {
+                const float4* yr = reinterpret_cast<const float4*>(y + (int64_t)col * d);
+                float ip = 0.f;
+#pragma unroll 4
+                for (int k4 = 0; k4 < (d >> 2); k4++) {
+                    const float4 yv = yr[k4];
+                    const float4 xv = *reinterpret_cast<const float4*>(sx + 4 * k4);
+                    ip = __builtin_fmaf(xv.x, yv.x, ip);
+                    ip = __builtin_fmaf(xv.y, yv.y, ip);
+                    ip = __builtin_fmaf(xv.z, yv.z, ip);
+                    ip = __builtin_fmaf(xv.w, yv.w, ip);
+                }
+                float dis = __builtin_fmaf(-2.f, ip, xn + yn[col]);
+                if (dis < 0.f) dis = 0.f;
+                buf[e] = ((unsigned long long)f2key(dis) << 32) | col;
+            }
+        }
+        __builtin_amdgcn_wave_barrier();
+    }
     unsigned long long mine[CF_BUF / 64];
     int rr[CF_BUF / 64];
 #pragma unroll
@@ -462,9 +669,23 @@
     return pl;
 }
 
+size_t coarse_image_bytes(int d, int nlist) {
+    const size_t ny_pad = ((size_t)nlist + 63) / 64 * 64;
+    return ny_pad * d * 4 + ny_pad * sizeof(float);
+}
+bool coarse_image_supported(int d, int nlist) { return (d == 32 || d == 64 || d == 96 || d == 128) && nlist >= 2048; }
+void launch_coarse_image(hipStream_t s, const float* y, const float* yn, int nlist, int d, void* image) {
+    const int ny_pad = (nlist + 63) / 64 * 64;
+    const int n = ny_pad * (d / 8);
+    char* img = static_cast<char*>(image);
+    hipLaunchKernelGGL(k_coarse_image, dim3((n + 255) / 256), dim3(256), 0, s, y, yn, nlist, ny_pad, d, img,
+                       reinterpret_cast<float*>(img + (size_t)ny_pad * d * 4));
+}
+
 void launch_coarse_fused(hipStream_t s, const CoarseFusedPlan& pl, void* ws, const float* x, int nq, int d,
                          const float* y, int nlist, const float* yn, int P, float* out_dis, int* out_idx, bool exact_ties,
-                         unsigned long long* tie_stats, hipStream_t side, hipEvent_t fork, hipEvent_t join) {
+                         unsigned long long* tie_stats, hipStream_t side, hipEvent_t fork, hipEvent_t join,
+                         const CoarseBf16* bf) {
     char* b = static_cast<char*>(ws);
     float* mat = reinterpret_cast<float*>(b + pl.off_mat);
     float* tau = reinterpret_cast<float*>(b + pl.off_tau);
@@ -498,6 +719,17 @@
     else if (pl.sample == 1024) hipLaunchKernelGGL(k_coarse_bound<16>, dim3((nq + 3) / 4), dim3(256), 0, s, mat, nq, P, tau, ovf);
     else hipLaunchKernelGGL(k_coarse_bound<32>, dim3((nq + 3) / 4), dim3(256), 0, s, mat, nq, P, tau, ovf);
     dim3 grid((unsigned)pl.nseg, (unsigned)((nq + 127) / 128));
+#define GH_CB(NCH)                                                                                                      \
+    do {                                                                                                                \
+        static std::atomic<uint64_t> attr{0};                                                           \
+        if (first_call_on_device(attr)) {                                                                               \
+            (void)hipFuncSetAttribute(reinterpret_cast<const void*>(k_coarse_filter_bf16<NCH>),                         \
+                                      hipFuncAttributeMaxDynamicSharedMemorySize, 2 * 2 * (16 * NCH) * 128);            \
+        }                                                                                                               \
+        hipLaunchKernelGGL((k_coarse_filter_bf16<NCH>), grid, dim3(256), (size_t)2 * 2 * (16 * NCH) * 128, s, x, nq,    \
+                           static_cast<const char*>(bf->img), bf->hc, nlist, pl.sample, tau, pl.tiles_per_strip, pl.cap, \
+                           pl.cap_stride, cand, cnt, pl.nseg);                                                          \
+    } while (0)
 #define GH_CF(NCH)                                                                                                      \
     do {                                                                                                                \
         static std::atomic<uint64_t> attr{0};                                                           \
@@ -508,16 +740,32 @@
         hipLaunchKernelGGL((k_coarse_fused<NCH>), grid, dim3(256), lds, s, x, nq, y, nlist, pl.sample, yn, tau,         \
                            pl.tiles_per_strip, pl.cap, pl.cap_stride, cand, cnt, pl.nseg, nullptr);                          \
     } while (0)
-    switch (d) {
-        case 32: GH_CF(2); break;
-        case 64: GH_CF(4); break;
-        case 96: GH_CF(6); break;
-        default: GH_CF(8); break;
+    if (bf) {
+        switch (d) {
+            case 32: GH_CB(2); break;
+            case 64: GH_CB(4); break;
+            case 96: GH_CB(6); break;
+            default: GH_CB(8); break;
+        }
+    } else {
+        switch (d) {
+            case 32: GH_CF(2); break;
+            case 64: GH_CF(4); break;
+            case 96: GH_CF(6); break;
+            default: GH_CF(8); break;
+        }
     }
 #undef GH_CF
+#undef GH_CB
+#define GH_FIN1(SN, MS, BFV)                                                                                            \
+    hipLaunchKernelGGL((k_coarse_final<SN, MS, BFV>), dim3((nq + 3) / 4), dim3(256), 0, s, mat, tau, cand, cnt, pl.nseg, \
+                       pl.cap, pl.cap_stride, nq, P, out_dis, out_idx, ovf, exact_ties ? 1 : 0, x, y, yn, d,            \
+                       bf ? bf->yn_max : 0.f, bf ? bf->stat : nullptr)
 #define GH_FIN(SN, MS)                                                                                                  \
-    hipLaunchKernelGGL((k_coarse_final<SN, MS>), dim3((nq + 3) / 4), dim3(256), 0, s, mat, tau, cand, cnt, pl.nseg, pl.cap, \
-                       pl.cap_stride, nq, P, out_dis, out_idx, ovf, exact_ties ? 1 : 0)
+    do {                                                                                                                \
+        if (bf) GH_FIN1(SN, MS, true);                                                                                  \
+        else GH_FIN1(SN, MS, false);                                                                                    \
+    } while (0)
     if (pl.sample == 512) {
         if (pl.nseg <= 4) GH_FIN(8, 4);
         else if (pl.nseg <= 8) GH_FIN(8, 8);
@@ -530,6 +778,7 @@
         else GH_FIN(32, 16);
     }
 #undef GH_FIN
+#undef GH_FIN1
     if (!exact_ties) {
         hipLaunchKernelGGL(k_coarse_repair, dim3(kCoarseRepairGrid), dim3(256), (size_t)d * sizeof(float), s, x, d, y, nlist, yn,
                            ovf, scratch, P, out_dis, out_idx);
diff --git a/gamma_amd/csrc/flat_mfma.hip b/gamma_amd/csrc/flat_mfma.hip
--- a/gamma_amd/csrc/flat_mfma.hip
+++ b/gamma_amd/csrc/flat_mfma.hip
@@ -7,36 +7,19 @@
 
 #include "device_math.h"
 #include "filter_dev.h"
+#include "bf16_split.h"
 #include "block_utils.h"
 #include "kernels.h"
 #include "rerank_dev.h"
 
 namespace gh {
 
-typedef __attribute__((__vector_size__(8 * sizeof(__bf16)))) __bf16 bf16x8;
 typedef float ff32x16 __attribute__((ext_vector_type(16)));
 
 constexpr float FM_C = 1.220703125e-4f;
 constexpr int FM_QT = 64;
 constexpr int FM_ROWS = 128;
 constexpr int FM_NT = 256;
-
-__device__ __forceinline__ uint32_t cvt_pk_bf16(float lo, float hi) {
-    uint32_t r;
-    asm("v_cvt_pk_bf16_f32 %0, %1, %2" : "=v"(r) : "v"(lo), "v"(hi));
-    return r;
-}
-__device__ __forceinline__ void split_bf16x8(const float* f, uint4& hi, uint4& lo) {
-    uint32_t h[4], l[4];
-#pragma unroll
-    for (int i = 0; i < 4; i++) {
-        h[i] = cvt_pk_bf16(f[2 * i], f[2 * i + 1]);
-        const float h0 = __uint_as_float(h[i] << 16), h1 = __uint_as_float(h[i] & 0xffff0000u);
-        l[i] = cvt_pk_bf16(f[2 * i] - h0, f[2 * i + 1] - h1);
-    }
-    hi = make_uint4(h[0], h[1], h[2], h[3]);
-    lo = make_uint4(l[0], l[1], l[2], l[3]);
-}
 
 __host__ __device__ constexpr int fm_mt_bytes(int D) { return 2 * (D / 16) * 2 * 32 * 16; }
 
diff --git a/gamma_amd/csrc/gamma_hip.cpp b/gamma_amd/csrc/gamma_hip.cpp
--- a/gamma_amd/csrc/gamma_hip.cpp
+++ b/gamma_amd/csrc/gamma_hip.cpp
@@ -123,7 +123,7 @@
     if (h->d_raw_slot) (void)hipFree(h->d_raw_slot);
     void* ptrs[] = {h->d_list_rank, h->d_raw, h->d_bitmap, h->d_cc, h->d_cc_norms, h->d_pqc, h->d_T2, h->d_codes,
                     h->d_ids, h->d_list_mask, h->d_scan_codes, h->d_tie_stats, h->d_v2d, h->d_sums, h->d_t2max, h->d_bound_stat,
-                    h->d_bin_cc, h->d_bin_stats};
+                    h->d_bin_cc, h->d_bin_stats, h->d_cc_img, h->d_cbf_stat};
     for (void* p : ptrs)
         if (p) (void)hipFree(p);
     for (auto& kv : h->fields)
@@ -138,6 +138,8 @@
     if (h->dir_pin) (void)hipHostFree(h->dir_pin);
     if (h->bound_copy_ev) (void)hipEventDestroy(h->bound_copy_ev);
     if (h->pin_bound_stat) (void)hipHostFree(h->pin_bound_stat);
+    if (h->cbf_copy_ev) (void)hipEventDestroy(h->cbf_copy_ev);
+    if (h->pin_cbf_stat) (void)hipHostFree(h->pin_cbf_stat);
     if (h->pin_flat_over) (void)hipHostFree(h->pin_flat_over);
     DevBuf* bufs[] = {&h->w_mat, &h->w_coarse_dis, &h->w_probe, &h->w_xn, &h->w_st2, &h->w_pair_off,
                       &h->w_qtotal, &h->w_dist, &h->w_cand_dis, &h->w_cand_pos, &h->w_cand_ids,
@@ -208,8 +210,25 @@
 int gamma_hip_set_coarse_fused(gamma_hip_index* h, int on, int list_cap) {
     if (!h || list_cap < 1 || list_cap > gh::kCoarseCap) return GAMMA_HIP_EINVAL;
     SearchLock lk(h);
-    h->coarse_fused = on != 0;
+    h->coarse_fused = on == 0 ? 0 : (on == 2 ? 2 : 1);
     h->coarse_cap = list_cap;
+    h->cbf_off_calls = 0;
+    return GAMMA_HIP_OK;
+}
+
+int gamma_hip_coarse_filter_stats(gamma_hip_index* h, int64_t* out4) {
+    if (!h || !out4) return GAMMA_HIP_EINVAL;
+    SearchLock lk(h);
+    unsigned long long v[2] = {0, 0};
+    if (h->d_cbf_stat) {
+        GH_CHECK(h, hipSetDevice(h->device));
+        GH_CHECK(h, hipStreamSynchronize(h->stream));
+        GH_CHECK(h, hipMemcpy(v, h->d_cbf_stat, sizeof(v), hipMemcpyDeviceToHost));
+    }
+    out4[0] = (int64_t)v[0];
+    out4[1] = (int64_t)v[1];
+    out4[2] = h->cbf_backoffs;
+    out4[3] = h->cbf_off_calls;
     return GAMMA_HIP_OK;
 }
 
@@ -291,6 +310,7 @@
         b += h->arena_cap * (h->code_size + (int64_t)sizeof(int64_t));
         if (h->d_sums) b += h->arena_cap * (int64_t)sizeof(float) + (int64_t)h->nlist * 4;
         b += (int64_t)h->nlist * 12;
+        b += (int64_t)h->cc_img_bytes;
         b += (int64_t)(h->w_cmp_codes.cap + h->w_cmp_ids.cap + h->w_cmp_len.cap);
     }
     return b;
diff --git a/gamma_amd/csrc/gamma_hip_internal.h b/gamma_amd/csrc/gamma_hip_internal.h
--- a/gamma_amd/csrc/gamma_hip_internal.h
+++ b/gamma_amd/csrc/gamma_hip_internal.h
@@ -239,7 +239,19 @@
     std::atomic<int64_t> ties_unhonoured{0};
     int scan_dbg_now = 0;
     std::atomic<int64_t> blas_unrestated{0};
-    bool coarse_fused = true;
+    int coarse_fused = 1;
+    void* d_cc_img = nullptr;
+    size_t cc_img_bytes = 0;
+    bool cc_img_ok = false;
+    float cc_norm_max = 0.f;
+    unsigned long long* d_cbf_stat = nullptr;
+    unsigned long long* pin_cbf_stat = nullptr;
+    unsigned long long cbf_seen[2] = {0, 0};
+    hipEvent_t cbf_copy_ev = nullptr;
+    bool cbf_copy_pending = false;
+    uint64_t cbf_sig = 0;
+    int cbf_off_calls = 0;
+    int64_t cbf_backoffs = 0, cbf_calls = 0;
     bool small_path = true;
     int small_presel = 0;
     std::vector<int32_t> h_v2d;
diff --git a/gamma_amd/csrc/gamma_hip_search.cpp b/gamma_amd/csrc/gamma_hip_search.cpp
--- a/gamma_amd/csrc/gamma_hip_search.cpp
+++ b/gamma_amd/csrc/gamma_hip_search.cpp
@@ -146,7 +146,41 @@
     hipStream_t s = h->stream;
     int mode = p->coarse_mode;
     if (mode < 0) mode = nq < 20 ? 0 : 1;
-    const bool fused = mode == 1 && h->coarse_fused && gh::coarse_fused_supported(nq, d, nlist, P, tie_on(p));
+    const bool fused = mode == 1 && h->coarse_fused != 0 && gh::coarse_fused_supported(nq, d, nlist, P, tie_on(p));
+    bool bf16 = fused && h->coarse_fused == 1 && h->d_cc_img && h->cc_img_ok;
+    if (bf16) {
+        const uint64_t sig = ((uint64_t)nlist << 32) ^ ((uint64_t)P << 16) ^ (uint64_t)d ^ (1ull << 63);
+        auto landed = [&]() {
+            if (h->cbf_copy_pending && hipEventQuery(h->cbf_copy_ev) == hipSuccess) h->cbf_copy_pending = false;
+            else if (h->cbf_copy_pending) (void)hipGetLastError();
+            return !h->cbf_copy_pending;
+        };
+        if (sig != h->cbf_sig) {
+            h->cbf_sig = sig;
+            h->cbf_off_calls = 0;
+            if (h->cbf_copy_pending) {
+                (void)hipEventSynchronize(h->cbf_copy_ev);
+                h->cbf_copy_pending = false;
+            }
+            h->cbf_seen[0] = h->pin_cbf_stat[0];
+            h->cbf_seen[1] = h->pin_cbf_stat[1];
+        }
+        if (h->cbf_off_calls > 0) {
+            if (--h->cbf_off_calls > 0) bf16 = false;
+        } else if (landed()) {
+            const unsigned long long u = h->pin_cbf_stat[0], n = h->pin_cbf_stat[1];
+            const unsigned long long dn = n - h->cbf_seen[1], du = std::min(u - h->cbf_seen[0], dn);
+            if (dn >= 2048) {
+                h->cbf_seen[0] = u;
+                h->cbf_seen[1] = n;
+                if (8 * du > dn) {
+                    h->cbf_off_calls = 256;
+                    h->cbf_backoffs++;
+                    bf16 = false;
+                }
+            }
+        }
+    }
     gh::CoarseFusedPlan plan;
     if (fused) {
         plan = gh::coarse_fused_plan(nq, nlist, P, h->coarse_cap, tie_on(p));
@@ -164,9 +198,26 @@
     if (fused) {
         static const bool no_side = getenv("GAMMA_HIP_NO_SIDE_STREAM") != nullptr;
         const bool side = tie_on(p) && defer_join && !no_side;
+        gh::CoarseBf16 bf;
+        if (bf16) {
+            const size_t ny_pad = ((size_t)nlist + 63) / 64 * 64;
+            bf.img = h->d_cc_img;
+            bf.hc = reinterpret_cast<const float*>(static_cast<const char*>(h->d_cc_img) + ny_pad * d * 4);
+            bf.yn_max = h->cc_norm_max;
+            bf.stat = h->d_cbf_stat;
+        }
         gh::launch_coarse_fused(s, plan, h->w_mat.p, d_x, nq, d, h->d_cc, nlist, h->d_cc_norms, P, out_dis, out_probe,
-                                tie_on(p), h->d_tie_stats, side ? h->side : nullptr, h->ev_fork, h->ev_join);
+                                tie_on(p), h->d_tie_stats, side ? h->side : nullptr, h->ev_fork, h->ev_join,
+                                bf16 ? &bf : nullptr);
         h->coarse_join_pending = side;
+        if (bf16) {
+            h->cbf_calls++;
+            if (!h->cbf_copy_pending) {
+                GH_CHECK(h, hipMemcpyAsync(h->pin_cbf_stat, h->d_cbf_stat, 2 * sizeof(unsigned long long), hipMemcpyDeviceToHost, s));
+                GH_CHECK(h, hipEventRecord(h->cbf_copy_ev, s));
+                h->cbf_copy_pending = true;
+            }
+        }
         static const bool dbg = getenv("GAMMA_HIP_COARSE_DBG") != nullptr;
         if (dbg) {
             int n_ovf = 0;
diff --git a/gamma_amd/csrc/gamma_hip_store.cpp b/gamma_amd/csrc/gamma_hip_store.cpp
--- a/gamma_amd/csrc/gamma_hip_store.cpp
+++ b/gamma_amd/csrc/gamma_hip_store.cpp
@@ -1116,6 +1116,37 @@
     return ivf_init_locked(h, d, nlist, 1, metric, bucket_init_size, bucket_max_size, true);
 }
 
+static int build_coarse_image(H* h) {
+    h->cc_img_ok = false;
+    if (!gh::coarse_image_supported(h->d, h->nlist)) return GAMMA_HIP_OK;
+    const size_t bytes = gh::coarse_image_bytes(h->d, h->nlist);
+    if (!h->d_cc_img) {
+        GH_CHECK(h, hipMalloc(&h->d_cc_img, bytes));
+        h->cc_img_bytes = bytes;
+    }
+    if (!h->d_cbf_stat) {
+        GH_CHECK(h, hipMalloc((void**)&h->d_cbf_stat, 2 * sizeof(unsigned long long)));
+        GH_CHECK(h, hipMemset(h->d_cbf_stat, 0, 2 * sizeof(unsigned long long)));
+        GH_CHECK(h, hipHostMalloc((void**)&h->pin_cbf_stat, 2 * sizeof(unsigned long long), hipHostMallocDefault));
+        h->pin_cbf_stat[0] = h->pin_cbf_stat[1] = 0;
+        GH_CHECK(h, hipEventCreateWithFlags(&h->cbf_copy_ev, hipEventDisableTiming));
+    }
+    gh::launch_coarse_image(h->wstream, h->d_cc, h->d_cc_norms, h->nlist, h->d, h->d_cc_img);
+    GH_CHECK(h, hipGetLastError());
+    std::vector<float> nn((size_t)h->nlist);
+    GH_CHECK(h, hipMemcpyAsync(nn.data(), h->d_cc_norms, nn.size() * sizeof(float), hipMemcpyDeviceToHost, h->wstream));
+    GH_CHECK(h, hipStreamSynchronize(h->wstream));
+    float mx = 0.f;
+    bool ok = true;
+    for (float v : nn) {
+        if (!(v <= gh::kCoarseBfNormMax)) ok = false;
+        else mx = std::max(mx, v);
+    }
+    h->cc_norm_max = mx;
+    h->cc_img_ok = ok;
+    return GAMMA_HIP_OK;
+}
+
 int gamma_hip_ivfflat_set_trained(gamma_hip_index* h, const float* cc) {
     if (!h || !cc) return GAMMA_HIP_EINVAL;
     WriteLock lk(h);
@@ -1124,6 +1155,7 @@
     GH_CHECK(h, hipMemcpyAsync(h->d_cc, cc, (size_t)h->nlist * h->d * sizeof(float), hipMemcpyHostToDevice, h->wstream));
     gh::launch_row_norms(h->wstream, h->d_cc, h->nlist, h->d, h->d_cc_norms);
     GH_CHECK(h, hipGetLastError());
+    GH_TRY(build_coarse_image(h));
     GH_CHECK(h, hipStreamSynchronize(h->wstream));
     h->trained = true;
     return GAMMA_HIP_OK;
@@ -1165,6 +1197,7 @@
     GH_CHECK(h, hipMemcpyAsync(h->d_cc, cc, ncc * sizeof(float), hipMemcpyHostToDevice, h->wstream));
     GH_CHECK(h, hipMemcpyAsync(h->d_pqc, pqc, npq * sizeof(float), hipMemcpyHostToDevice, h->wstream));
     gh::launch_row_norms(h->wstream, h->d_cc, h->nlist, h->d, h->d_cc_norms);
+    GH_TRY(build_coarse_image(h));
     if (h->table_mode == 0) {
     } else if (table)
         GH_CHECK(h, hipMemcpyAsync(h->d_T2, table, nt * sizeof(float), hipMemcpyHostToDevice, h->wstream));
diff --git a/gamma_amd/csrc/kernels.h b/gamma_amd/csrc/kernels.h
--- a/gamma_amd/csrc/kernels.h
+++ b/gamma_amd/csrc/kernels.h
@@ -212,6 +212,18 @@
     int sample, nseg, tiles_per_strip, cap, cap_stride;
     size_t off_mat, off_tau, off_cand, off_cnt, off_ovf, off_scratch, off_full, bytes;
 };
+constexpr float kCoarseBfMargin = 1.220703125e-4f;
+constexpr float kCoarseBfXnMin = 5.421010862427522e-20f;
+constexpr float kCoarseBfNormMax = 1.329227995784916e+36f;
+struct CoarseBf16 {
+    const void* img;
+    const float* hc;
+    float yn_max;
+    unsigned long long* stat;
+};
+size_t coarse_image_bytes(int d, int nlist);
+bool coarse_image_supported(int d, int nlist);
+void launch_coarse_image(hipStream_t s, const float* y, const float* yn, int nlist, int d, void* image);
 bool coarse_fused_supported(int nq, int d, int nlist, int P, bool exact_ties = false);
 CoarseFusedPlan coarse_fused_plan(int nq, int nlist, int P, int cap, bool exact_ties = false);
 void launch_coarse_heap_rows(hipStream_t s, const float* mat, int nlist, int nq, int K, const int* rows, float* out_vals,
@@ -219,7 +231,8 @@
 void launch_coarse_fused(hipStream_t s, const CoarseFusedPlan& pl, void* ws, const float* x, int nq, int d,
                          const float* y, int nlist, const float* yn, int P, float* out_dis, int* out_idx,
                          bool exact_ties = false, unsigned long long* tie_stats = nullptr,
-                         hipStream_t side = nullptr, hipEvent_t fork = nullptr, hipEvent_t join = nullptr);
+                         hipStream_t side = nullptr, hipEvent_t fork = nullptr, hipEvent_t join = nullptr,
+                         const CoarseBf16* bf = nullptr);
 bool launch_small_coarse_ip(hipStream_t s, const float* x, int nq, int d, const float* cc, int nlist, float* mat, int M,
                             const float* pqc, float* st2, int* zero_me = nullptr);
 void launch_small_coarse_select(hipStream_t s, const float* mat, int nlist, int nq, int P, float* out_vals, int* out_pos,
diff --git a/include/gamma_hip.h b/include/gamma_hip.h
--- a/include/gamma_hip.h
+++ b/include/gamma_hip.h
@@ -83,6 +83,7 @@
 int gamma_hip_set_workspace_budget(gamma_hip_index* h, int64_t bytes);
 int gamma_hip_set_exact_ties(gamma_hip_index* h, int on);
 int gamma_hip_set_coarse_fused(gamma_hip_index* h, int on, int list_cap);
+int gamma_hip_coarse_filter_stats(gamma_hip_index* h, int64_t* out4);
 int gamma_hip_set_small_path(gamma_hip_index* h, int on);
 int gamma_hip_tie_stats(gamma_hip_index* h, int64_t* out3, int reset);
 int gamma_hip_ties_not_honoured(gamma_hip_index* h, int64_t* out_calls, int reset);
```

Result: faster. 11.56 million, median of 6 (+3.0%).
